# csukuangfj/kaldi-hmm-gmm

Measured on AMD Instinct MI355X. Metric: frames/sec (whole node) per EM iter (align+acc-stats), 5k-pdf x 64-Gauss, higher is better.
Workload: dtype f32 via f16x2s

## Files before the change

include/khg_hip.h:

```cpp
#ifndef KHG_HIP_H_
#define KHG_HIP_H_
#include <stdint.h>

#ifdef __cplusplus
extern "C" {
#endif

#define KHG_OK 0
#define KHG_E_ARG (-1)
#define KHG_E_HIP (-2)
#define KHG_E_RUNTIME (-3)
#define KHG_E_UNSUPPORTED (-4)
#define KHG_MAX_DIM 512

typedef struct khg_ctx khg_ctx;
typedef struct khg_model khg_model;
typedef struct khg_tm khg_tm;
typedef struct khg_utts khg_utts;
typedef struct khg_accs khg_accs;

const char *khg_last_error(void);
int khg_version(void);

int khg_ctx_create(int device, void *stream, khg_ctx **out);
int khg_ctx_destroy(khg_ctx *ctx);
int khg_ctx_sync(khg_ctx *ctx);
int khg_ctx_set_timing(khg_ctx *ctx, int on);
int khg_ctx_get_timings(khg_ctx *ctx, char *names, int64_t names_cap, float *ms, int32_t cap,
                        int32_t *n_out);

#define KHG_K1_AUTO 0
#define KHG_K1_FP32_PDF 2
#define KHG_K1_FP32_UTT 3
#define KHG_K1_F16X2 4
#define KHG_K1_F16X2S 5
int khg_ctx_set_k1_form(khg_ctx *ctx, int form);

#define KHG_OPT_K1_FORM 0
#define KHG_OPT_K1_ORDER 1
#define KHG_OPT_K1_NF 2
#define KHG_OPT_K1P_TS 3
#define KHG_OPT_K1_INTERLEAVE 4
#define KHG_OPT_K1_DBG 5
#define KHG_OPT_K2_INORDER 6
#define KHG_OPT_K2_KS 7
#define KHG_OPT_K2_SERIAL 8
#define KHG_OPT_K2_PROF 9
#define KHG_OPT_K3_BUCKET 10
#define KHG_OPT_K3_FORM 11
#define KHG_OPT_K3_PHASE_B 12
#define KHG_OPT_K3_NY 13
#define KHG_OPT_DEBUG 14
#define KHG_OPT_K3_PHASE_A 15
#define KHG_OPT_K2_SPLIT 16
#define KHG_OPT_K2S_HUB 17
#define KHG_OPT_LAT_OPS_LDS 18
#define KHG_OPT_K1_LAUNCH 19
#define KHG_OPT_K1_PGRID 20
#define KHG_OPT_K1_PROF 21
#define KHG_OPT_K2_LADDER 22
#define KHG_OPT_COUNT 23
#define KHG_INFO_SCRATCH_BYTES 100
#define KHG_INFO_SCRATCH_BLOCKS 101
int khg_ctx_set_option(khg_ctx *ctx, int option, int value);
int khg_ctx_get_option(const khg_ctx *ctx, int option, int *value);
int khg_option_check(int option, int value);
int khg_option_from_env(const char *name, const char *text, int *option, int *value);

int khg_model_create(khg_ctx *ctx, int32_t num_pdfs, int32_t dim, const int32_t *gauss_off_h,
                     const float *gconsts_h, const float *means_invvars_h,
                     const float *inv_vars_h, khg_model **out);
int khg_model_destroy(khg_model *m);
int khg_model_invalidate(khg_model *m);

int khg_tm_create(khg_ctx *ctx, int32_t num_tids, const int32_t *id2pdf_h, khg_tm **out);
int khg_tm_set_trans_cost(khg_tm *tm, const float *trans_cost_h);
int khg_tm_destroy(khg_tm *tm);

int khg_utts_create(khg_ctx *ctx, const khg_tm *tm, int32_t n_utt, int32_t dim,
                    const int64_t *frame_off_h, const float *feats_h, const float *feats_d,
                    const int64_t *state_off_h, const int32_t *start_h, const int64_t *arc_off_h,
                    const int32_t *ilabel_h, const int32_t *olabel_h, const float *weight_h,
                    const int32_t *nextstate_h, const float *final_h, khg_utts **out);
int khg_utts_destroy(khg_utts *u);
typedef struct khg_graph khg_graph;
int khg_graph_create(khg_ctx *ctx, const khg_tm *tm, int32_t num_states, int32_t start, const int64_t *arc_off_h,
                     const int32_t *ilabel_h, const int32_t *olabel_h, const float *weight_h,
                     const int32_t *nextstate_h, const float *final_h, khg_graph **out);
int khg_graph_destroy(khg_graph *g);
int khg_graph_info(const khg_graph *g, int64_t *num_states, int64_t *num_arcs, int32_t *num_pdfs,
                   int32_t *max_in_degree, int64_t *device_bytes);
int khg_utts_create_on_graph(khg_ctx *ctx, const khg_tm *tm, khg_graph *g, int32_t n_utt, int32_t dim,
                             const int64_t *frame_off_h, const float *feats_h, const float *feats_d, khg_utts **out);
int khg_utts_graph_bytes(const khg_utts *u, int64_t *bytes);
int khg_utts_num_pdfs(const khg_utts *u, int64_t *pdf_off_h );
int khg_utts_pdfs(const khg_utts *u, int32_t *pdfs_h );
int khg_utts_k2_plan(khg_ctx *ctx, const khg_utts *u, int32_t out[8]);
int khg_utts_k2_ladder(khg_ctx *ctx, const khg_utts *u, int32_t *out);
int khg_utts_pdf_first(const khg_utts *u, int32_t *first_h );

int khg_loglikes(khg_ctx *ctx, const khg_model *m, khg_utts *u);
int khg_loglikes_reachable(khg_ctx *ctx, const khg_model *m, khg_utts *u);
int khg_loglikes_band(khg_ctx *ctx, const khg_model *m, khg_utts *u);
int khg_utts_pdf_last(const khg_utts *u, int32_t *last_h );
int khg_loglikes_layout(const khg_utts *u, int64_t *ll_off_h, int64_t *total);
int khg_loglikes_download(khg_ctx *ctx, const khg_utts *u, float *ll_h);
int khg_loglikes_upload(khg_ctx *ctx, khg_utts *u, const float *ll_h);
int khg_utts_set_pdf_list(khg_utts *u, int32_t n, const int32_t *pdfs_h);
int khg_utts_features_changed(khg_utts *u);

typedef struct {
  float beam;
  float retry_beam;
  int32_t careful;
  float acoustic_scale;
  int32_t max_active;
  int32_t min_active;
  float beam_delta;
  float hash_ratio;
  float like_scale;
} khg_align_config;
void khg_align_config_default(khg_align_config *c);

#define KHG_ALIGN_DONE 0
#define KHG_ALIGN_ERROR 1
#define KHG_ALIGN_RETRIED 2
#define KHG_ALIGN_EXACT_DP 4
#define KHG_ALIGN_FALLBACK 8

int khg_careful_graph(int32_t num_states, int32_t start, const int64_t *arc_off_h, const int32_t *ilabel_h,
                      const int32_t *olabel_h, const float *weight_h, const int32_t *nextstate_h, const float *final_h,
                      int32_t *out_num_states, int32_t *out_start, int64_t *out_arc_off_h, int32_t *out_ilabel_h,
                      int32_t *out_olabel_h, float *out_weight_h, int32_t *out_nextstate_h, float *out_final_h);

int khg_align(khg_ctx *ctx, const khg_tm *tm, khg_utts *u, const khg_align_config *cfg,
              int32_t *ali_h, int32_t *words_h, int64_t *words_off_h, int64_t words_cap,
              float *like_h, int32_t *status_h);
int khg_ali_upload(khg_ctx *ctx, khg_utts *u, const int32_t *ali_h);
int khg_ali_download(khg_ctx *ctx, khg_utts *u, int32_t *ali_h);

typedef struct {
  float beam;
  int32_t max_active;
  int32_t min_active;
  float lattice_beam;
  int32_t prune_interval;
  float beam_delta;
  float hash_ratio;
  float prune_scale;
  float acoustic_scale;
  int32_t allow_partial;
  int32_t scratch_per_frame;
} khg_lattice_faster_config;
void khg_lattice_faster_config_default(khg_lattice_faster_config *c);

#define KHG_LAT_SUCCEEDED 1
#define KHG_LAT_PARTIAL 2
#define KHG_LAT_SCRATCH 4
#define KHG_LAT_NO_PATH 8
#define KHG_LAT_EPS_LOOP 16
#define KHG_LAT_WORDS 32
#define KHG_LAT_NO_TRACEBACK 64

int khg_decode_lattice_faster(khg_ctx *ctx, const khg_tm *tm, khg_utts *u, const khg_lattice_faster_config *cfg,
                              int32_t *ali_h, int32_t *words_h, int64_t *words_off_h, int64_t words_cap,
                              double *like_h, int32_t *status_h);

typedef struct {
  float beam;
  float lattice_beam;
  int32_t prune_interval;
  float prune_scale;
  float acoustic_scale;
  int32_t allow_partial;
  int32_t scratch_per_frame;
} khg_lattice_simple_config;
void khg_lattice_simple_config_default(khg_lattice_simple_config *c);

#define KHG_LAT_NO_EPS_TOKEN 128
#define KHG_LAT_NAN 256

// ... 381 lines not shown
```

kaldi_hmm_gmm_amd/_lib.py:

```python
import ctypes as C
import os

import numpy as np

_HERE = os.path.dirname(os.path.abspath(__file__))
LIB_PATH = os.environ.get("KHG_LIBRARY") or os.path.join(_HERE, "libkhg_hip.so")


class KhgError(RuntimeError):
    """Mirror of the reference's std::runtime_error -> Python RuntimeError (csrc/log.h:46-53)."""


def _load():
    if not os.path.exists(LIB_PATH):
        raise ImportError(
            f"{LIB_PATH} not found: build it with `python -c 'import __graft_entry__ as g; g.build()'` "
            "(hipcc --offload-arch=gfx950). kaldi_hmm_gmm_amd has no CPU fallback."
        )
    try:
        import torch
    except ImportError:
        pass
    return C.CDLL(LIB_PATH)

# ... 54 lines not shown
    _fields_ = [
        ("min_gaussian_weight", C.c_float),
        ("min_gaussian_occupancy", C.c_float),
        ("min_variance", C.c_double),
        ("remove_low_count_gaussians", C.c_int32),
        ("variance_floor_vector", C.POINTER(C.c_double)),
    ]


class EbwOptionsC(C.Structure):
    _fields_ = [("E", C.c_double), ("tau", C.c_double)]


class EbwWeightOptionsC(C.Structure):
    _fields_ = [("min_num_count_weight_update", C.c_double), ("min_gaussian_weight", C.c_double), ("tau", C.c_double)]


class EbwResultsC(C.Structure):
    _fields_ = [("auxf_impr_gauss", C.c_double), ("count", C.c_double), ("auxf_impr_weights", C.c_double), ("floored", C.c_int32),
                ("failed", C.c_int32), ("skipped", C.c_int32), ("weights_skipped", C.c_int32)]


class FmllrOptionsC(C.Structure):
    _fields_ = [("min_count", C.c_double), ("num_iters", C.c_int32)]


class MlltOptionsC(C.Structure):
    _fields_ = [("num_iters", C.c_int32)]


class LdaOptionsC(C.Structure):
    _fields_ = [("target_dim", C.c_int32), ("remove_offset", C.c_int32), ("within_class_factor", C.c_double)]


class FrontendOptsC(C.Structure):
    _fields_ = [("kind", C.c_int32), ("samp_freq", C.c_float), ("frame_length_ms", C.c_float), ("frame_shift_ms", C.c_float), ("preemph_coeff", C.c_float),
                ("remove_dc_offset", C.c_int32), ("window_type", C.c_int32), ("blackman_coeff", C.c_float), ("snip_edges", C.c_int32),
                ("round_to_power_of_two", C.c_int32), ("dither", C.c_float), ("num_mel_bins", C.c_int32), ("low_freq", C.c_float), ("high_freq", C.c_float),
                ("vtln_warp", C.c_float), ("htk_compat", C.c_int32), ("num_ceps", C.c_int32), ("cepstral_lifter", C.c_float), ("use_energy", C.c_int32),
                ("raw_energy", C.c_int32), ("energy_floor", C.c_float), ("use_log_fbank", C.c_int32), ("use_power", C.c_int32)]


class RescoreStatsC(C.Structure):
    _fields_ = [("arcs", C.c_int64), ("emitting_arcs", C.c_int64), ("cells", C.c_int64)]


class LmRescoreStatsC(C.Structure):
    _fields_ = [("in_states", C.c_int64), ("in_arcs", C.c_int64), ("out_states", C.c_int64), ("out_arcs", C.c_int64), ("max_hist", C.c_int64)]


SIGNATURES = {
    "khg_last_error": (C.c_char_p, []),
    "khg_version": (C.c_int, []),
    "khg_ctx_create": (C.c_int, [C.c_int, vp, C.POINTER(vp)]),
    "khg_ctx_destroy": (C.c_int, [vp]),
    "khg_ctx_sync": (C.c_int, [vp]),
    "khg_ctx_set_timing": (C.c_int, [vp, C.c_int]),
    "khg_ctx_set_k1_form": (C.c_int, [vp, C.c_int]),
    "khg_ctx_set_option": (C.c_int, [vp, C.c_int, C.c_int]),
    "khg_ctx_get_option": (C.c_int, [vp, C.c_int, C.POINTER(C.c_int)]),
    "khg_option_check": (C.c_int, [C.c_int, C.c_int]),
    "khg_option_from_env": (C.c_int, [C.c_char_p, C.c_char_p, C.POINTER(C.c_int), C.POINTER(C.c_int)]),
    "khg_ctx_get_timings": (C.c_int, [vp, C.c_char_p, C.c_int64, c_f32p, C.c_int32, c_i32p]),
    "khg_model_create": (C.c_int, [vp, C.c_int32, C.c_int32, c_i32p, c_f32p, c_f32p, c_f32p, C.POINTER(vp)]),
    "khg_model_destroy": (C.c_int, [vp]),
    "khg_tm_create": (C.c_int, [vp, C.c_int32, c_i32p, C.POINTER(vp)]),
    "khg_tm_set_trans_cost": (C.c_int, [vp, c_f32p]),
    "khg_tm_destroy": (C.c_int, [vp]),
    "khg_utts_create": (
        C.c_int,
        [vp, vp, C.c_int32, C.c_int32, c_i64p, c_f32p, vp, c_i64p, c_i32p, c_i64p, c_i32p, c_i32p, c_f32p, c_i32p,
         c_f32p, C.POINTER(vp)],
    ),
    "khg_utts_destroy": (C.c_int, [vp]),
    "khg_graph_create": (C.c_int, [vp, vp, C.c_int32, C.c_int32, c_i64p, c_i32p, c_i32p, c_f32p, c_i32p, c_f32p, C.POINTER(vp)]),
    "khg_graph_destroy": (C.c_int, [vp]),
    "khg_graph_info": (C.c_int, [vp, c_i64p, c_i64p, c_i32p, c_i32p, c_i64p]),
    "khg_utts_create_on_graph": (C.c_int, [vp, vp, vp, C.c_int32, C.c_int32, c_i64p, c_f32p, vp, C.POINTER(vp)]),
    "khg_utts_graph_bytes": (C.c_int, [vp, c_i64p]),
    "khg_utts_num_pdfs": (C.c_int, [vp, c_i64p]),
    "khg_utts_pdfs": (C.c_int, [vp, c_i32p]),
    "khg_utts_k2_plan": (C.c_int, [vp, vp, c_i32p]),
    "khg_utts_k2_ladder": (C.c_int, [vp, vp, c_i32p]),
    "khg_utts_pdf_first": (C.c_int, [vp, c_i32p]),
    "khg_loglikes": (C.c_int, [vp, vp, vp]),
    "khg_loglikes_reachable": (C.c_int, [vp, vp, vp]),
    "khg_loglikes_band": (C.c_int, [vp, vp, vp]),
    "khg_utts_pdf_last": (C.c_int, [vp, c_i32p]),
    "khg_loglikes_layout": (C.c_int, [vp, c_i64p, c_i64p]),
    "khg_loglikes_download": (C.c_int, [vp, vp, c_f32p]),
    "khg_loglikes_upload": (C.c_int, [vp, vp, c_f32p]),
    "khg_utts_set_pdf_list": (C.c_int, [vp, C.c_int32, c_i32p]),
    "khg_utts_features_changed": (C.c_int, [vp]),
    "khg_comm_info": (C.c_int, [vp, c_i32p, c_i32p, c_i32p]),
    "khg_align_config_default": (None, [C.POINTER(AlignConfigC)]),
    "khg_align": (C.c_int, [vp, vp, vp, C.POINTER(AlignConfigC), c_i32p, c_i32p, c_i64p, C.c_int64, c_f32p, c_i32p]),
    "khg_ali_upload": (C.c_int, [vp, vp, c_i32p]),
    "khg_lattice_faster_config_default": (None, [C.POINTER(LatticeFasterConfigC)]),
    "khg_decode_lattice_faster": (C.c_int, [vp, vp, vp, C.POINTER(LatticeFasterConfigC), c_i32p, c_i32p, c_i64p, C.c_int64, c_f64p,
                                            c_i32p]),
    "khg_lattice_simple_config_default": (None, [C.POINTER(LatticeSimpleConfigC)]),
    "khg_decode_lattice_simple": (C.c_int, [vp, vp, vp, C.POINTER(LatticeSimpleConfigC), c_i32p, c_i32p, c_i64p, C.c_int64, c_f64p,
                                            c_i32p, c_i32p]),
    "khg_decode_lattice_simple_raw": (C.c_int, [vp, vp, vp, C.POINTER(LatticeSimpleConfigC), c_i32p, c_i32p, c_i64p, C.c_int64, c_f64p,
                                                c_i32p, c_i32p, C.POINTER(vp)]),
    "khg_decode_lattice_faster_raw": (C.c_int, [vp, vp, vp, C.POINTER(LatticeFasterConfigC), c_i32p, c_i32p, c_i64p, C.c_int64, c_f64p,
                                                c_i32p, C.POINTER(vp)]),
    "khg_lattices_sizes": (C.c_int, [vp, c_i64p, c_i64p]),
    "khg_lattices_download": (C.c_int, [vp, vp, c_i32p, c_i32p, c_f32p, c_f32p, c_f32p, c_i32p, c_i32p, c_i32p, c_f32p, c_f32p, c_i32p,
                                        c_i32p]),
    "khg_lattices_device_bytes": (C.c_int, [vp, c_i64p]),
    "khg_lattices_destroy": (C.c_int, [vp]),
    "khg_lattices_validate": (C.c_int, [C.c_int32, c_i64p, c_i64p, c_i32p, c_i32p, c_f32p, c_f32p, c_f32p, c_i32p, c_i32p, c_i32p, c_f32p,
                                        c_f32p, c_i32p, c_i32p]),
    "khg_lattices_upload": (C.c_int, [vp, C.c_int32, c_i64p, c_i64p, c_i32p, c_i32p, c_f32p, c_f32p, c_f32p, c_i32p, c_i32p, c_i32p, c_f32p,
                                      c_f32p, c_i32p, c_i32p, C.POINTER(vp)]),
    "khg_lattices_num_utts": (C.c_int, [vp, c_i32p]),
    "khg_lattices_ali_layout": (C.c_int, [vp, vp, c_i64p]),
    "khg_lattices_num_chunks": (C.c_int, [vp, c_i32p]),
    "khg_lattices_chunk_utts": (C.c_int, [vp, c_i32p]),
    "khg_lattices_best_path": (C.c_int, [vp, vp, C.c_int32, c_f32p, c_f32p, c_i32p, c_i32p, c_i64p, C.c_int64, c_f32p, c_i32p]),
    "khg_lattices_prune": (C.c_int, [vp, vp, C.c_float, C.c_float, C.c_float, c_i32p, C.POINTER(vp)]),
    "khg_lattices_posteriors": (C.c_int, [vp, vp, C.c_float, C.c_float, c_i32p, c_f64p, C.POINTER(vp)]),
    "khg_lattices_rescore": (C.c_int, [vp, vp, vp, vp, vp, C.c_float, C.c_int, C.POINTER(RescoreStatsC), C.POINTER(vp)]),
    "khg_lattices_op_status": (C.c_int, [vp, c_i32p]),
    "khg_lattices_boost": (C.c_int, [vp, vp, C.c_int32, c_i32p, C.c_int32, c_i32p, c_i64p, c_i32p, vp, C.c_float, C.c_float, c_i32p,
                                     C.POINTER(vp)]),
    "khg_lm_validate": (C.c_int, [C.c_int32, c_i32p, c_f32p, c_i32p, c_i32p, c_f32p, c_i32p, c_f32p, C.c_int32]),
    "khg_lm_create": (C.c_int, [vp, C.c_int32, c_i32p, c_f32p, c_i32p, c_i32p, c_f32p, c_i32p, c_f32p, C.c_int32, C.POINTER(vp)]),
    "khg_lm_destroy": (C.c_int, [vp]),
    "khg_lm_num_states": (C.c_int, [vp, c_i32p]),
    "khg_lm_device_bytes": (C.c_int, [vp, c_i64p]),
    "khg_lm_score": (C.c_int, [C.c_int32, c_i32p, c_f32p, c_i32p, c_i32p, c_f32p, c_i32p, c_f32p, C.c_int32, C.c_int32, c_i32p, c_f32p]),
    "khg_lattices_lm_rescore": (C.c_int, [vp, vp, vp, C.c_float, C.c_int32, c_i32p, C.POINTER(LmRescoreStatsC), C.POINTER(vp)]),
    "khg_lattices_mpe_posteriors": (C.c_int, [vp, vp, C.c_int32, c_i32p, c_i32p, C.c_int32, c_i32p, c_i64p, c_i32p, vp, C.c_int32, C.c_int32,
                                              C.c_float, C.c_float, c_i32p, c_f64p, c_f64p, C.POINTER(vp)]),
    "khg_posteriors_sizes": (C.c_int, [vp, c_i64p, c_i64p]),
    "khg_posteriors_download": (C.c_int, [vp, vp, c_i64p, c_i32p, c_f64p, c_f64p]),
    "khg_posteriors_device_bytes": (C.c_int, [vp, c_i64p]),
    "khg_posteriors_destroy": (C.c_int, [vp]),
    "khg_posteriors_validate": (C.c_int, [C.c_int32, c_i64p, c_i64p, C.c_int64, c_i32p, c_f64p]),
    "khg_posteriors_upload": (C.c_int, [vp, C.c_int32, c_i64p, c_i64p, c_i32p, c_f64p, C.POINTER(vp)]),
    "khg_ali_download": (C.c_int, [vp, vp, c_i32p]),
    "khg_accs_create": (C.c_int, [vp, vp, vp, C.POINTER(vp)]),
    "khg_accs_destroy": (C.c_int, [vp]),
    "khg_accs_zero": (C.c_int, [vp, vp]),
    "khg_accs_size": (C.c_int, [vp, c_i64p]),
    "khg_accs_device_ptr": (C.c_int, [vp, C.POINTER(vp)]),
    "khg_accs_download": (C.c_int, [vp, vp, c_f64p]),
    "khg_accs_upload": (C.c_int, [vp, vp, c_f64p]),
    "khg_acc_stats": (C.c_int, [vp, vp, vp, vp, C.c_float, vp]),
    "khg_acc_stats_post": (C.c_int, [vp, vp, vp, vp, vp, C.c_float, vp]),
    "khg_acc_stats_post2": (C.c_int, [vp, vp, vp, vp, vp, C.c_float, vp, vp]),
    "khg_accs_add": (C.c_int, [vp, vp, C.c_float, vp]),
    "khg_accs_scale": (C.c_int, [vp, vp, C.c_float]),
    "khg_accs_smooth_with_accum": (C.c_int, [vp, vp, C.c_float, vp, vp, c_i32p]),
    "khg_accs_allreduce": (C.c_int, [vp, vp, vp]),
    "khg_accs_allreduce_range": (C.c_int, [vp, vp, vp, C.c_int32, C.c_int32, vp]),
    "khg_acc_stats_reduce": (C.c_int, [vp, vp, vp, vp, C.c_float, vp, vp, C.c_int32]),
    "khg_accs_allreduce_f32": (C.c_int, [vp, vp, vp]),
    "khg_comm_unique_id": (C.c_int, [vp]),
    "khg_comm_create": (C.c_int, [vp, C.c_int32, C.c_int32, vp, C.POINTER(vp)]),
    "khg_comm_destroy": (C.c_int, [vp]),
    "khg_compute_gconsts": (C.c_int, [C.c_int32, C.c_int32, c_i32p, c_f32p, c_f32p, c_f32p, c_f32p, c_i32p]),
    "khg_mle_options_default": (None, [C.POINTER(MleOptionsC)]),
    "khg_mle_am_diag_gmm_update": (
# ... 131 lines not shown
```

kaldi_hmm_gmm_amd/csrc/khg_ctx_model.hip:

```cpp
#include "khg_internal.hpp"

#include <mutex>
#include "khg_k1_loglikes.hip.inc"

static thread_local std::string g_err;
extern "C" const char* khg_last_error(void) { return g_err.c_str(); }
int khg_set_error(int code, const std::string& msg) { g_err = msg; return code; }
extern "C" int khg_version(void) { return 100; }

static std::mutex g_ctx_mu;
static std::vector<khg_ctx*> g_ctxs;
static constexpr size_t KHG_ARENA_BYTES = size_t(24) << 20;
void* arena_alloc(khg_ctx* ctx, size_t bytes) {
  KhgArena& a = ctx->arena;
  if (!a.dev) {
    if (a.cap == SIZE_MAX) return nullptr;
    void *d = nullptr, *h = nullptr;
    if (hipMalloc(&d, KHG_ARENA_BYTES) != hipSuccess || hipHostMalloc(&h, KHG_ARENA_BYTES, hipHostMallocDefault) != hipSuccess) {
      if (d) (void)hipFree(d);
      (void)hipGetLastError();
      a.cap = SIZE_MAX;
      return nullptr;
    }
    a.dev = static_cast<char*>(d); a.host = static_cast<char*>(h); a.cap = KHG_ARENA_BYTES; a.top = a.base = 256;
// ... 51 lines not shown
  return false;
}
void khg_dev_free(void* p) {
  if (p && !khg_arena_release(p)) (void)hipFree(p);
}

static void ctx_defaults_from_env(khg_ctx* c);
extern "C" int khg_ctx_create(int device, void* stream, khg_ctx** out) {
  if (!out) return khg_set_error(KHG_E_ARG, "khg_ctx_create: out is NULL");
  int n = 0;
  hipError_t e = hipGetDeviceCount(&n);
  if (e != hipSuccess || n <= 0)
    return khg_set_error(KHG_E_HIP, "khg_ctx_create: no HIP device available (this library has no CPU fallback)");
  if (device < 0 || device >= n) return khg_set_error(KHG_E_ARG, "khg_ctx_create: bad device index");
  HIPCHK(hipSetDevice(device));
  hipDeviceProp_t prop;
  HIPCHK(hipGetDeviceProperties(&prop, device));
  if (std::string(prop.gcnArchName).rfind("gfx950", 0) != 0)
    return khg_set_error(KHG_E_UNSUPPORTED, std::string("khg_ctx_create: built for gfx950, device is ") + prop.gcnArchName);
  khg_ctx* c = new khg_ctx();
  c->device = device;
  if (stream) { c->stream = (hipStream_t)stream; c->own_stream = false; }
  else { HIPCHK(hipStreamCreateWithFlags(&c->stream, hipStreamNonBlocking)); c->own_stream = true; }
  for (auto& s : c->sides) HIPCHK(hipStreamCreateWithFlags(&s, hipStreamNonBlocking));
  ctx_defaults_from_env(c);
  int rc = dev_alloc(&c->err_flag_d, 1);
  if (!rc) rc = dev_alloc(&c->dump_d, 256);
  if (!rc && hipHostMalloc(reinterpret_cast<void**>(&c->err_host), 256, hipHostMallocDefault) != hipSuccess) rc = khg_set_error(KHG_E_HIP, "khg_ctx_create: hipHostMalloc failed");
  if (rc) { delete c; return rc; }
  HIPCHK(hipMemsetAsync(c->err_flag_d, 0, sizeof(int32_t), c->stream));
  { std::lock_guard<std::mutex> lk(g_ctx_mu); g_ctxs.push_back(c); }
  *out = c;
  return KHG_OK;
}
extern "C" int khg_ctx_destroy(khg_ctx* c) {
  if (!c) return KHG_OK;
  (void)hipStreamSynchronize(c->stream);
  for (auto& s : c->sides) (void)hipStreamSynchronize(s);
  {
    std::lock_guard<std::mutex> lk(g_ctx_mu);
    g_ctxs.erase(std::remove(g_ctxs.begin(), g_ctxs.end(), c), g_ctxs.end());
    if (c->arena.dev && !c->arena.blocks.empty()) {
      c->arena.dirty.clear();
      g_orphans.push_back(std::move(c->arena));
      c->arena = KhgArena();
    }
  }
  DEVFREE(c->err_flag_d); DEVFREE(c->dump_d); DEVFREE(c->k1_next_d);
  if (c->err_host) (void)hipHostFree(c->err_host);
  if (c->arena.dev) (void)hipFree(c->arena.dev);
  if (c->arena.host) (void)hipHostFree(c->arena.host);
  if (c->own_stream) (void)hipStreamDestroy(c->stream);
  for (auto& s : c->sides) (void)hipStreamDestroy(s);
  if (c->comm_stream) { (void)hipStreamSynchronize(c->comm_stream); (void)hipStreamDestroy(c->comm_stream); }
  if (c->ev_k3) (void)hipEventDestroy(c->ev_k3);
  if (c->ev_c1) (void)hipEventDestroy(c->ev_c1);
  delete c;
  return KHG_OK;
}
extern "C" int khg_ctx_set_timing(khg_ctx* c, int on) {
  if (!c) return khg_set_error(KHG_E_ARG, "ctx is NULL");
  c->timing = on != 0;
  return KHG_OK;
}
extern "C" int khg_ctx_get_timings(khg_ctx* c, char* names, int64_t names_cap, float* ms, int32_t cap, int32_t* n_out) {
  if (!c || !n_out) return khg_set_error(KHG_E_ARG, "bad arguments");
  HIPCHK(hipStreamSynchronize(c->stream));
  for (auto& s : c->sides) HIPCHK(hipStreamSynchronize(s));
  int n = 0; std::string all;
  for (auto& t : c->timings) {
    float v = 0.0f;
    (void)hipEventElapsedTime(&v, t.e0, t.e1);
    if (n < cap && ms) ms[n] = v;
    all += t.name; all += '\n';
    (void)hipEventDestroy(t.e0); (void)hipEventDestroy(t.e1);
    ++n;
  }
  c->timings.clear();
  if (names && names_cap > 0) { size_t k = std::min<size_t>(all.size(), (size_t)names_cap - 1); memcpy(names, all.data(), k); names[k] = 0; }
  *n_out = n;
  return KHG_OK;
}
static const struct { int lo, hi; } k_opt_range[KHG_OPT_COUNT] = {
  {KHG_K1_AUTO, KHG_K1_F16X2S}, {0, 4}, {0, 6}, {0, 1 << 20}, {-1, 1}, {0, 255}, {0, 1}, {0, 4}, {0, 3}, {0, 1}, {0, 2}, {0, 2}, {0, 2}, {0, 64}, {0, 1}, {0, 1}, {0, 1}, {0, 1 << 20}, {0, 1}, {0, 2}, {0, 1 << 16}, {0, 1}, {0, 1}};
extern "C" int khg_option_check(int opt, int value) {
  if (opt < 0 || opt >= KHG_OPT_COUNT) return khg_set_error(KHG_E_ARG, "khg_option_check: no such option");
  if (value < k_opt_range[opt].lo || value > k_opt_range[opt].hi || (opt == KHG_OPT_K1_FORM && value == 1))
    return khg_set_error(KHG_E_ARG, "khg_ctx_set_option: option " + std::to_string(opt) + " takes values " + std::to_string(k_opt_range[opt].lo) + " .. " + std::to_string(k_opt_range[opt].hi));
  return KHG_OK;
}
extern "C" int khg_ctx_set_option(khg_ctx* c, int opt, int value) {
  if (!c || opt < 0 || opt >= KHG_OPT_COUNT) return khg_set_error(KHG_E_ARG, "khg_ctx_set_option: bad arguments");
  int rc = khg_option_check(opt, value);
  if (rc) return rc;
  c->opt[opt] = value;
  return KHG_OK;
}
extern "C" int khg_ctx_get_option(const khg_ctx* c, int opt, int* value) {
  if (c && value && (opt == KHG_INFO_SCRATCH_BYTES || opt == KHG_INFO_SCRATCH_BLOCKS)) {
    *value = opt == KHG_INFO_SCRATCH_BYTES ? (c->arena.dev ? (int)c->arena.top : 0) : (int)c->arena.blocks.size();
    return KHG_OK;
  }
  if (!c || !value || opt < 0 || opt >= KHG_OPT_COUNT) return khg_set_error(KHG_E_ARG, "khg_ctx_get_option: bad arguments");
  *value = c->opt[opt];
  return KHG_OK;
}
extern "C" int khg_ctx_set_k1_form(khg_ctx* c, int form) { return khg_ctx_set_option(c, KHG_OPT_K1_FORM, form); }
static const struct { const char* name; int opt; const char* words; } k_env_tab[] = {
  {"KHG_K1", KHG_OPT_K1_FORM, "auto=0,pdf=2,fp32=2,utt=3,f16x2=4,f16x2s=5"},
  {"KHG_K1_ORDER", KHG_OPT_K1_ORDER, "desc=0,none=1,asc=2,tiles=3,xcd=4"},
  {"KHG_K1_NF", KHG_OPT_K1_NF, ""}, {"KHG_K1P_TS", KHG_OPT_K1P_TS, ""}, {"KHG_K1_INTERLEAVE", KHG_OPT_K1_INTERLEAVE, ""},
  {"KHG_K1B_DBG", KHG_OPT_K1_DBG, ""}, {"KHG_K2_INORDER", KHG_OPT_K2_INORDER, ""}, {"KHG_K2_KS", KHG_OPT_K2_KS, ""},
  {"KHG_K2_SERIAL", KHG_OPT_K2_SERIAL, ""}, {"KHG_K2_PROF", KHG_OPT_K2_PROF, ""},
  {"KHG_K3_BUCKET", KHG_OPT_K3_BUCKET, "sort=0,atomic=1,count=2"}, {"KHG_K3_FORM", KHG_OPT_K3_FORM, "auto=0,block=1,valu=2"},
  {"KHG_K3_VALU", KHG_OPT_K3_FORM, "1=2"}, {"KHG_K3_PHASEB", KHG_OPT_K3_PHASE_B, "f64=0,f32=1,f16=2"},
  {"KHG_K3_NY", KHG_OPT_K3_NY, ""}, {"KHG_DEBUG", KHG_OPT_DEBUG, ""}, {"KHG_K3_PHASEA", KHG_OPT_K3_PHASE_A, "auto=0,f16=0,f32=1"},
  {"KHG_K2_SPLIT", KHG_OPT_K2_SPLIT, "on=0,off=1"}, {"KHG_K2S_HUB", KHG_OPT_K2S_HUB, ""},
  {"KHG_LAT_OPS_LDS", KHG_OPT_LAT_OPS_LDS, "on=0,off=1"},
  {"KHG_K1_LAUNCH", KHG_OPT_K1_LAUNCH, "auto=0,chunk=1,persistent=2"}, {"KHG_K1_PGRID", KHG_OPT_K1_PGRID, ""},
  {"KHG_K1_PROF", KHG_OPT_K1_PROF, ""}, {"KHG_K2_LADDER", KHG_OPT_K2_LADDER, "on=0,off=1"}};
extern "C" int khg_option_from_env(const char* name, const char* text, int* option, int* value) {
  if (!name || !text || !*text || !option || !value) return khg_set_error(KHG_E_ARG, "khg_option_from_env: bad arguments");
  for (const auto& t : k_env_tab) {
    if (strcmp(t.name, name) != 0) continue;
    const char* e = text;
    int v = atoi(e);
    bool word = false;
    for (const char* w = t.words; *w;) {
      const char* eq = strchr(w, '=');
      const size_t n = (size_t)(eq - w);
      if (strlen(e) == n && strncmp(e, w, n) == 0) { v = atoi(eq + 1); word = true; break; }
      const char* comma = strchr(eq, ',');
      if (!comma) break;
      w = comma + 1;
    }
    if (!word && *t.words && !(e[0] >= '0' && e[0] <= '9') && e[0] != '-')
      return khg_set_error(KHG_E_ARG, std::string(name) + ": unknown word '" + text + "'");
    if (v < k_opt_range[t.opt].lo || v > k_opt_range[t.opt].hi)
      return khg_set_error(KHG_E_ARG, std::string(name) + " takes values " + std::to_string(k_opt_range[t.opt].lo) + " .. " + std::to_string(k_opt_range[t.opt].hi));
    *option = t.opt; *value = v;
    return KHG_OK;
  }
  return khg_set_error(KHG_E_ARG, std::string("khg_option_from_env: no such variable: ") + name);
}
static void ctx_defaults_from_env(khg_ctx* c) {
  c->opt[KHG_OPT_K1_INTERLEAVE] = -1;
  c->opt[KHG_OPT_K1P_TS] = 1024;
  c->opt[KHG_OPT_K2S_HUB] = 32;
  c->opt[KHG_OPT_K3_PHASE_B] = 2;
  for (const auto& t : k_env_tab) {
    const char* e = getenv(t.name);
    if (!e || !*e) continue;
    int opt = 0, v = 0;
    if (khg_option_from_env(t.name, e, &opt, &v) == KHG_OK) c->opt[opt] = v;
  }
}
extern "C" int khg_ctx_sync(khg_ctx* c) {
  if (!c) return khg_set_error(KHG_E_ARG, "ctx is NULL");
  return check_err_flag(c, "khg_ctx_sync");
}
int check_err_flag(khg_ctx* c, const char* where) {
  { int rf = arena_flush(c); if (rf) return rf; }
  for (int i = 0; i < khg_ctx::NSIDE; ++i)
    if (c->side_dirty[i]) { HIPCHK(hipStreamSynchronize(c->sides[i])); c->side_dirty[i] = false; }
  HIPCHK(hipMemcpyAsync(c->err_host, c->err_flag_d, sizeof(int32_t), hipMemcpyDeviceToHost, c->stream));
  HIPCHK(hipStreamSynchronize(c->stream));
  c->pageable_pending = false;
  const int32_t f = *c->err_host;
  if (f) {
    HIPCHK(hipMemsetAsync(c->err_flag_d, 0, sizeof(int32_t), c->stream));
    if (f & 1) return khg_set_error(KHG_E_RUNTIME, std::string(where) + ": Invalid answer (overflow or invalid variances/features?)");
    if (f & 2) return khg_set_error(KHG_E_RUNTIME, std::string(where) + ": internal queue overflow in the faithful decoder");
    if (f & 8) return khg_set_error(KHG_E_RUNTIME, std::string(where) + ": internal error: K3 work items exceed their bound");
    return khg_set_error(KHG_E_RUNTIME, std::string(where) + ": pdf-id out of range (graph/model mismatch)");
  }
  return KHG_OK;
}

template <int KQ>
__global__ __launch_bounds__(256) void k0_pack_tiles(const float* __restrict__ gconsts, const float* __restrict__ miv,
                                                      const float* __restrict__ iv, const int32_t* __restrict__ gauss_off,
                                                      const int32_t* __restrict__ pdf_tile_off, const int32_t* __restrict__ tile_pdf,
                                                      int D, float* __restrict__ wimg, float* __restrict__ nhiv) {
  constexpr int ROW = khg_row_floats(KQ), TILE = khg_tile_floats(KQ);
  const int t = blockIdx.x, p = tile_pdf[t];
  const int g_first = gauss_off[p] + 32 * (t - pdf_tile_off[p]);
  const int nrow = min(32, gauss_off[p + 1] - g_first);
  float* img = wimg + (size_t)t * TILE;
  for (int i = threadIdx.x; i < TILE; i += 256) {
    float v = 0.0f;
    if (i < 4 * 32 * ROW) {
      const int q = i / (32 * ROW), r = (i / ROW) & 31, s = i % ROW;
      const int d = 2 * s + (q & 1);
      if (r < nrow && d < D) {
        const size_t src = (size_t)(g_first + r) * D + d;
        v = (q & 2) ? -0.5f * iv[src] : miv[src];
      }
    } else if (i < 4 * 32 * ROW + 32) {
      const int r = i - 4 * 32 * ROW;
      v = r < nrow ? gconsts[g_first + r] : -INFINITY;
    }
    img[i] = v;
  }
// ... 271 lines not shown
```

kaldi_hmm_gmm_amd/csrc/khg_internal.hpp:

```cpp
#pragma once
#include <hip/hip_runtime.h>

#include <algorithm>
#include <climits>
#include <cmath>
#include <cstdint>
#include <cstdio>
#include <cstdlib>
#include <cstring>
#include <deque>
#include <limits>
#include <string>
#include <type_traits>
#include <utility>
#include <vector>

#include "../../include/khg_hip.h"
#include "khg_dev_types.hip.inc"

int khg_set_error(int code, const std::string& msg);

#define HIPCHK(expr)                                                                         \
  do {                                                                                       \
    hipError_t e_ = (expr);                                                                  \
// ... 159 lines not shown
  float* trans_cost_d = nullptr;
  bool has_trans_cost = false;
};

struct khg_graph {
  khg_ctx* ctx = nullptr;
  int32_t refs = 1;
  int64_t S = 0, A = 0, nwords = 0, device_bytes = 0;
  int32_t start = -1, max_indeg = 0, max_outdeg = 0;
  bool same_col = true, has_eps = false, ladder = true;
  std::vector<int32_t> pdfs, pdf_first, pdf_dfin;
  int64_t *state_off_d = nullptr, *in_off_d = nullptr, *out_off_d = nullptr;
  int32_t *start_d = nullptr, *in_src_d = nullptr, *in_col_d = nullptr, *in_tid_d = nullptr, *in_olabel_d = nullptr, *out_inidx_d = nullptr;
  float *in_w_d = nullptr, *final_d = nullptr;
};
void khg_graph_release(khg_graph* g);

struct khg_utts {
  khg_ctx* ctx = nullptr;
  khg_graph* graph = nullptr;
  int32_t* gidx_d = nullptr;
  int64_t graph_bytes = 0;
  bool small = false;
  int32_t n_utt = 0, D = 0;
  int64_t N = 0;
  bool has_graphs = false;
  std::vector<int64_t> frame_off, state_off, pdf_off, ll_off, bp_off, path_off, words_off;
  std::vector<int32_t> pdfs;
  int32_t max_states = 0, max_inarcs = 0, max_indeg = 0, max_outdeg = 0;
  bool same_col = true;
  bool ladder = true;
  int32_t pdfs_checked_P = -1;
  bool has_eps = false;
  const float* feats_d = nullptr; bool own_feats = false;
  int64_t *frame_off_d = nullptr, *state_off_d = nullptr, *pdf_off_d = nullptr, *ll_off_d = nullptr;
  int32_t *pdfs_d = nullptr, *start_d = nullptr;
  KwChunk* wchunks_d = nullptr;
  int32_t n_wchunks = 0;
  int64_t *in_off_d = nullptr, *out_off_d = nullptr;
  int32_t *in_src_d = nullptr, *in_col_d = nullptr, *in_tid_d = nullptr, *in_olabel_d = nullptr, *out_inidx_d = nullptr;
  float *in_w_d = nullptr, *final_d = nullptr;
  K1Chunk* chunks_d = nullptr; int32_t n_chunks = 0; int32_t chunk_kq = 0;
  int64_t* tile_off_d = nullptr; int32_t* tiles_d = nullptr;
  std::vector<int32_t> pdf_first;
  std::vector<int32_t> pdf_last;
  int ll_mode = 0;
  void* band_args = nullptr;
  khg_model* band_model = nullptr; int band_ks = 0; size_t band_lds = 0; uint64_t band_serial = 0, band_version = 0; std::vector<int32_t> band_key;
  int tiles_reach = -1;
  std::vector<int32_t> tiles_pto;
  float* ll_d = nullptr; int64_t ll_total = 0; bool ll_valid = false;
  float* xpl_d = nullptr; int64_t* utt_xtile_off_d = nullptr; int32_t xpl_kq = 0;
  K1pEntry* p_ents_d = nullptr; K1pSlice* p_slices_d = nullptr; int32_t p_nslices = 0; int p_reach = -1; int32_t p_P = -1;
  int32_t p_grp[10] = {0, 0, 0, 0, 0, 0, 0, 0, 0, 0};
  std::vector<int32_t> p_goff;
  int64_t* utt_x32_off_d = nullptr;
  K1bChunk* bchunks_d = nullptr; int32_t n_bchunks = 0, bchunk_nt = 0;
  int32_t* x32_utt_d = nullptr; int64_t n_x32 = 0;
  k1b_u32x4* xh_d = nullptr; int32_t xh_ks = 0; std::vector<int32_t> xh_ex; int32_t* xh_ex_d = nullptr;
  std::vector<float> xmax;
  k1b_u32x4* xs_d = nullptr; int32_t xs_ks = 0; std::vector<int32_t> xs_ex; int32_t* xs_ex_d = nullptr;
  K1sChunk* schunks_d = nullptr; int32_t n_schunks = 0, schunk_nmax = 0;
  K1sUnit* sunits_d = nullptr; std::vector<int32_t> sunits_pto; int sunits_reach = -1;
  uint8_t* bp_d = nullptr; int64_t *bp_off_d = nullptr, *path_off_d = nullptr, *words_off_d = nullptr;
  double* layer_best_d = nullptr; int32_t* layer_cnt_d = nullptr; int32_t* path_d = nullptr;
  unsigned char* k2_gscratch_d = nullptr; size_t k2_gscratch_bytes = 0;
  int32_t* k2_order_d = nullptr;
  int32_t *ali_d = nullptr, *words_d = nullptr, *num_words_d = nullptr, *status_d = nullptr;
  float* like_d = nullptr;
  bool ali_valid = false;
  char* out_blk_d = nullptr; size_t out_blk_bytes = 0;
  hipEvent_t ev_dp = nullptr, ev_ali = nullptr;
  bool ali_pending = false;
  int32_t *ali2_d = nullptr, *unc_d = nullptr, *unc_cnt_h = nullptr, *unc_cnt_dev = nullptr;
  int64_t* sub_off_d = nullptr;
  bool ali_split = false;
  int32_t *pdf_count_d = nullptr, *pdf_cursor_d = nullptr, *frame_ids_d = nullptr;
  uint32_t *sort_keys_d = nullptr, *sort_keys_out_d = nullptr, *sort_vals_d = nullptr; void* sort_tmp_d = nullptr; size_t sort_tmp_bytes = 0;
  int32_t* cs_hist_d = nullptr; size_t cs_hist_n = 0; int64_t* cs_tot_d = nullptr; size_t cs_tot_n = 0;
  double *k3_part_d = nullptr, *k3_llpart_d = nullptr; size_t k3_part_n = 0, k3_llpart_n = 0;
  void* k3_items_d = nullptr; int32_t* k3_item_off_d = nullptr; size_t k3_items_n = 0, k3_item_off_n = 0;
  int64_t* pdf_start_d = nullptr; unsigned long long* tid_count_d = nullptr;
  int32_t k3_P = 0, k3_tids = 0;
  int32_t *pe_row_d = nullptr, *pe_tid_d = nullptr, *pe_ids_d = nullptr; float* pe_w_d = nullptr; size_t pe_cap = 0;
  uint32_t *pe_keys_d = nullptr, *pe_keys_out_d = nullptr, *pe_vals_d = nullptr; void* pe_tmp_d = nullptr; size_t pe_tmp_bytes = 0;
  int64_t* pe_start_d = nullptr; int32_t pe_P = 0;
  uint64_t *rc_keys_d = nullptr, *rc_keys_out_d = nullptr; uint32_t *rc_vals_d = nullptr, *rc_vals_out_d = nullptr;
  int32_t *rc_flag_d = nullptr, *rc_inc_d = nullptr, *rc_row_d = nullptr; float* rc_cell_d = nullptr; size_t rc_cap = 0;
  void* rc_tmp_d = nullptr; size_t rc_tmp_bytes = 0;
  int32_t *rc_cell_start_d = nullptr, *rc_item_off_d = nullptr; int64_t* rc_stats_d = nullptr; int32_t rc_P = -1;
};

static inline int64_t utt_states(const khg_utts* u, int i) { return u->graph ? u->state_off[1] : u->state_off[(size_t)i + 1] - u->state_off[(size_t)i]; }

struct khg_accs {
  khg_ctx* ctx = nullptr;
  int64_t sumG = 0; int32_t D = 0, num_tids = 0;
  int64_t n = 0, cap = 0;
  double* buf_d = nullptr;
  float* wire_d = nullptr; int64_t wire_cap = 0;
  double* occ() const { return buf_d; }
  double* mean() const { return buf_d + sumG; }
  double* var() const { return buf_d + sumG + sumG * D; }
  double* trans() const { return buf_d + sumG + 2 * sumG * D; }
  double* scalars() const { return trans() + num_tids + 1; }
};

constexpr size_t KHG_ARENA_MAX_REQ = size_t(4) << 20;
template <class T>
inline int u_alloc(khg_utts* u, T** p, size_t n) {
  if (n == 0) n = 1;
  if (u->small && n * sizeof(T) <= KHG_ARENA_MAX_REQ) {
    *p = static_cast<T*>(arena_alloc(u->ctx, n * sizeof(T)));
    if (*p) return KHG_OK;
  }
  return dev_alloc(p, n);
}
template <class T>
inline int u_upload(khg_ctx* ctx, khg_utts* u, T** p, const std::vector<T>& v) {
  if (u->small && v.size() * sizeof(T) <= KHG_ARENA_MAX_REQ) {
    *p = static_cast<T*>(arena_alloc(u->ctx, std::max<size_t>(v.size(), 1) * sizeof(T)));
    if (*p) {
      if (!v.empty()) { memcpy(u->ctx->arena.mirror(*p), v.data(), v.size() * sizeof(T)); arena_mark_dirty(u->ctx, *p, v.size() * sizeof(T)); }
      return KHG_OK;
    }
  }
  return dev_upload(ctx, p, v);
}

int check_err_flag(khg_ctx* c, const char* where);
int model_pack(khg_ctx* ctx, khg_model* m);
int model_stats(khg_ctx* ctx, khg_model* m);
int wait_ali(khg_ctx* ctx, khg_utts* u);
void k1_free_band(khg_utts* u);
int k1_maxima(khg_ctx* ctx, khg_model* m, khg_utts* u, std::vector<float>* xk);
khg_model* khg_model_lookup(uint64_t serial);
int k1_band_check(khg_ctx* ctx, khg_utts* u);
int k1_band_repair(khg_ctx* ctx, khg_utts* u, int32_t* status_d, int repair_bit, hipStream_t side);
int accs_allreduce_pieces(khg_ctx* ctx, khg_accs* a, const khg_model* m, int first_pdf, int n_pdf, void* comm, hipStream_t st);
int ctx_comm_stream(khg_ctx* ctx);
int k3_post_check(khg_ctx* ctx, const khg_model* m, const std::string& who);
__attribute__((visibility("hidden"))) int k3_acc_stats_post_one_block(khg_ctx* ctx, const khg_model* m, const khg_tm* tm, khg_utts* u, const khg_posteriors* p, float scale, khg_accs* acc);
struct PostInfo { const khg_ctx* ctx; int32_t U, max_tid; const int64_t *frame_off, *entry_off; };
void posteriors_info(const khg_posteriors* p, PostInfo* out);
int posteriors_flatten(khg_ctx* ctx, const khg_posteriors* p, const int64_t* set_frame_off_d, double scale, int32_t num_tids,
                       int32_t* e_row, int32_t* e_tid, float* e_w, int sign = 0);
int posteriors_make_unit(khg_ctx* ctx, int32_t n_utt, const int64_t* frame_off_h, int64_t** entry_begin_d, double** weight_d, int32_t** tid_d,
                         const int64_t** frame_off_d, khg_posteriors** out);
inline int utts_grow_pe(khg_utts* u, size_t E) {
  if (E <= u->pe_cap) return KHG_OK;
  DEVFREE(u->pe_row_d); DEVFREE(u->pe_tid_d); DEVFREE(u->pe_ids_d); DEVFREE(u->pe_w_d); DEVFREE(u->pe_keys_d); DEVFREE(u->pe_keys_out_d); DEVFREE(u->pe_vals_d);
  u->pe_cap = 0;
  int rc = u_alloc(u, &u->pe_row_d, E);
  if (!rc) rc = u_alloc(u, &u->pe_tid_d, E);
  if (!rc) rc = u_alloc(u, &u->pe_ids_d, E);
  if (!rc) rc = u_alloc(u, &u->pe_w_d, E);
  if (!rc) rc = u_alloc(u, &u->pe_keys_d, E);
  if (!rc) rc = u_alloc(u, &u->pe_keys_out_d, E);
  if (!rc) rc = u_alloc(u, &u->pe_vals_d, E);
  if (rc) return rc;
  u->pe_cap = E;
  return KHG_OK;
}
```

kaldi_hmm_gmm_amd/csrc/khg_k3.hip:

```cpp
#include "khg_internal.hpp"

#include <hipcub/hipcub.hpp>

#include "khg_k3_accstats.hip.inc"
#include "khg_k3_post.hip.inc"
#include "khg_k3_accops.hip.inc"

extern "C" int khg_accs_create(khg_ctx* ctx, const khg_model* m, const khg_tm* tm, khg_accs** out) {
  if (ctx_dead(ctx) || !m || !tm || !out) return khg_set_error(KHG_E_ARG, "khg_accs_create: bad arguments");
  khg_accs* a = new khg_accs();
  a->ctx = ctx; a->sumG = m->sumG; a->D = m->D; a->num_tids = tm->num_tids;
  a->n = a->sumG * (1 + 2 * (int64_t)a->D) + a->num_tids + 1 + 8;
  int rc = dev_alloc(&a->buf_d, (size_t)a->n);
  if (rc) { delete a; return rc; }
  a->cap = a->n;
  *out = a;
  return khg_accs_zero(ctx, a);
}
extern "C" int khg_accs_destroy(khg_accs* a) { if (a) { DEVFREE(a->buf_d); DEVFREE(a->wire_d); delete a; } return KHG_OK; }
extern "C" int khg_accs_zero(khg_ctx* ctx, khg_accs* a) {
  if (ctx_dead(ctx) || !a) return khg_set_error(KHG_E_ARG, "bad arguments");
  HIPCHK(hipMemsetAsync(a->buf_d, 0, sizeof(double) * (size_t)a->n, ctx->stream));
  return KHG_OK;
}
// ... 54 lines not shown
  if (dst->sumG > 0) {
    KernelTimer kt(ctx, "k3_accs_smooth");
    KHG_LAUNCH(ctx, k3_accs_smooth, dim3((unsigned)((dst->sumG + 3) / 4)), dim3(256), 0, ctx->stream, dst->occ(), dst->mean(), dst->var(), src->occ(),
               src->mean(), src->var(), (double)tau, dst->sumG, (int)dst->D, cnt_d);
    e = hipGetLastError();
  }
  if (untouched_out) {
    int32_t cnt = 0;
    if (e == hipSuccess) e = hipMemcpyAsync(&cnt, cnt_d, sizeof(int32_t), hipMemcpyDeviceToHost, ctx->stream);
    if (e == hipSuccess) e = hipStreamSynchronize(ctx->stream);
    DEVFREE(cnt_d);
    if (e == hipSuccess) *untouched_out = cnt;
  }
  if (e != hipSuccess) return khg_set_error(KHG_E_HIP, hipGetErrorString(e));
  return KHG_OK;
}

static int k3_phase_a_scales(khg_ctx* ctx, khg_model* m, khg_utts* u, bool* use) {
  *use = false;
  const int D = m->D, K = 8 * m->KQ;
  if (m->KQ == 0) return KHG_OK;
  std::vector<float> xk;
  int rc = k1_maxima(ctx, m, u, &xk);
  if (rc) return rc;
  if (m->k3_xb.empty()) {
    if (m->wmax.empty() || (int)m->k3_xb_raw.size() != D) { m->wmax.clear(); rc = model_stats(ctx, m); if (rc) return rc; }
    m->k3_xb = m->k3_xb_raw;
    m->k3_ex.assign((size_t)K, 0);
    bool ok = true;
    for (int d = 0; d < D; ++d) {
      const float xb = m->k3_xb[(size_t)d];
      if (!(xb > 0.0f) || !(xb < 1.0e18f)) { ok = false; break; }
      m->k3_ex[(size_t)2 * d] = 12 - std::ilogb(xb);
      m->k3_ex[(size_t)2 * d + 1] = 9 - std::ilogb(xb * xb);
    }
    int S = INT_MAX;
    if (ok) {
      for (int k = 0; k < 2 * D; ++k) if (m->wmax[(size_t)k] > 0.0f) S = std::min(S, 14 - std::ilogb(m->wmax[(size_t)k]) + m->k3_ex[(size_t)k]);
      if (S == INT_MAX) S = 0;
      if (S < -40 || S > 40) ok = false;
    }
    if (ok) {
      double floor_sum = 0.0, bound = (double)m->gcmax;
      for (int k = 0; k < 2 * D; ++k) {
        const double xbk = (k & 1) ? (double)m->k3_xb[(size_t)(k >> 1)] * (double)m->k3_xb[(size_t)(k >> 1)] : (double)m->k3_xb[(size_t)(k >> 1)];
        floor_sum += std::ldexp((double)m->wmax[(size_t)k], S - m->k3_ex[(size_t)k]) + std::ldexp(xbk, m->k3_ex[(size_t)k]);
        bound += (double)m->wmax[(size_t)k] * xbk * ((k & 1) ? 128.0 : 16.0);
      }
      if (!(std::ldexp(floor_sum, -25 - S) <= 4.0e-6) || !(bound <= 268435456.0)) ok = false;
      if (ctx->opt[KHG_OPT_DEBUG]) fprintf(stderr, "[khg] K3 fp16 phase A: S %d, floor %.3g, bound %.3g -> %s\n", S, std::ldexp(floor_sum, -25 - S), bound, ok ? "on" : "off");
    }
    m->k3_S = ok ? S : 0;
    m->k3_f16_ok = ok;
    if (ok) {
      if (!m->k3_ex_d) { rc = dev_alloc(&m->k3_ex_d, (size_t)K); if (rc) return rc; }
      HIPCHK(hipMemcpyAsync(m->k3_ex_d, m->k3_ex.data(), sizeof(int32_t) * (size_t)K, hipMemcpyHostToDevice, ctx->stream));
      HIPCHK(hipStreamSynchronize(ctx->stream));
    }
  }
  if (!m->k3_f16_ok) return KHG_OK;
  for (int k = 0; k < 2 * D; ++k)
    if (!(std::ldexp((double)xk[(size_t)k], m->k3_ex[(size_t)k]) < 65504.0)) return KHG_OK;
  *use = true;
  return KHG_OK;
}

static size_t k3_valu_lds(const khg_model* m, int maxG, bool post) {
  return sizeof(float) * (size_t)K3_CHUNK * ((size_t)(m->KQ ? 4 * m->KQ : (m->D | 1)) + (maxG | 1) + (post ? 5 : 4));
}
#define K3_VALU_LDS_MAX (160 * 1024)
enum K3Form { K3F_WAVE, K3F_MFMA, K3F_VALU };
struct K3Run {
  int form = K3F_VALU;
  int cls_lo = 0, cls_hi = INT_MAX;
  int maxG = 0, n_cls = 0;
  bool second = false;
  int NB = 0, NB16 = 0, nwv16 = 4;
  int ny = 1;
  bool parked = false;
  size_t nsum1 = 0;
  int target = 0;
  int64_t extra_blocks = 0, max_items = 0, max_slots = 0;
  bool may_f16a = false, may_f16b = false;
  size_t lds[3] = {0, 0, 0};
  bool too_wide = false;
};
struct K3Plan { int nruns = 0; K3Run run[2]; };

static K3Plan k3_plan(const khg_ctx* ctx, const khg_model* m, bool post, int64_t Neff, bool one_block) {
  const int P = m->P, KQ = m->KQ;
  const int k3form = ctx->opt[KHG_OPT_K3_FORM];
  const int pha = ctx->opt[KHG_OPT_K3_PHASE_A], phb = ctx->opt[KHG_OPT_K3_PHASE_B], ny_opt = ctx->opt[KHG_OPT_K3_NY];
  const int64_t avg = Neff / std::max(1, P);
  auto items = [&](K3Run& r) {
    r.target = one_block ? INT_MAX : (int)std::min<int64_t>(1 << 30, std::max<int64_t>(512, 2 * avg / r.ny));
    const int64_t per_t = Neff / r.target;
    r.extra_blocks = std::min<int64_t>(per_t + P, 2 * per_t) + 1;
    r.max_items = (int64_t)P * r.ny + r.extra_blocks;
    r.max_slots = !r.parked ? INT_MAX : r.ny > 1 ? r.max_items : 2 * per_t + 1;
  };
  auto wave = [&](int cls_lo, int cls_hi, int maxG) {
    K3Run r;
    r.form = K3F_WAVE; r.cls_lo = cls_lo; r.cls_hi = cls_hi; r.maxG = maxG; r.n_cls = P;
    const size_t nb = (size_t)(r.NB = (maxG + 15) / 16);
    r.may_f16a = nb >= 3 && pha == 0 && phb != 1; r.may_f16b = phb == 2;
    const size_t fold = sizeof(double) * (nb * 16 * 80 + nb * 16);
    r.lds[0] = std::max<size_t>(sizeof(float) * (nb * 20 * 64 + 4 * 4 * 16 * 20), fold);
    r.lds[1] = std::max<size_t>(sizeof(float) * (4 * 4 * 16 * 20) + 2 * (size_t)(4 * 2 * 16 * K3_XH_ROW), fold);
    r.lds[2] = std::max<size_t>(2 * (size_t)4 * (2 * (2 * 16 * K3_XH_ROW) + 2 * 2 * 40 * 36) + nb * 3 * 2 * 64 * 16, fold);
    const int64_t avg_tiles = (avg + 15) / 16;
    r.ny = (int)std::max<int64_t>(1, std::min<int64_t>(std::min<int64_t>(32, (avg_tiles + 15) / 16), (4096 + P - 1) / P));
    if (ny_opt > 0) r.ny = ny_opt;
    r.parked = true; r.nsum1 = nb * 16 * 80 + nb * 16 + 1;
    items(r);
    return r;
  };
  auto block = [&](int form, int cls_lo, int cls_hi, int maxG, int n_cls, bool second) {
    K3Run r;
    r.form = form; r.cls_lo = cls_lo; r.cls_hi = cls_hi; r.maxG = maxG; r.n_cls = n_cls; r.second = second;
    const int64_t avg_chunks = (avg + K3_CHUNK - 1) / K3_CHUNK;
    if (form == K3F_MFMA) {
      r.NB = std::max(1, (maxG + 63) / 64);
      r.lds[0] = sizeof(float) * ((size_t)4 * K3_CHUNK * 2 * KQ + (post ? 6 : 5) * K3_CHUNK);
      r.ny = (int)std::max<int64_t>(1, std::min<int64_t>(std::min<int64_t>(32, avg_chunks), (4096 + n_cls - 1) / std::max(1, n_cls)));
      if (ny_opt > 0) r.ny = ny_opt;
      r.may_f16a = r.may_f16b = !post && pha == 0 && phb == 2 && ((KQ == 20 && maxG <= 128) || (KQ == 10 && maxG <= 192));
      r.NB16 = maxG <= 128 ? 1 : 3; r.nwv16 = maxG > 64 && maxG <= 128 ? 8 : 4;
      const size_t kpad = ((size_t)8 * KQ + 31) / 32 * 32, gp_b16 = maxG <= 64 ? 64 : (maxG <= 128 ? 128 : 192);
      r.lds[2] = std::max<size_t>(2 * (2 * (size_t)K3_CHUNK * (kpad + 8) + 2 * (size_t)8 * KQ * (K3_CHUNK + 8)) + sizeof(float) * 9 * K3_CHUNK,
                                  sizeof(float) * (2 * gp_b16 * (size_t)(m->D | 1) + 8 * (size_t)KQ));
    } else {
      r.lds[0] = k3_valu_lds(m, maxG, post); r.too_wide = r.lds[0] > K3_VALU_LDS_MAX;
      r.ny = (int)std::max<int64_t>(1, std::min<int64_t>(64, (avg_chunks + 3) / 4));
    }
    if (one_block) r.ny = 1;
    items(r);
    return r;
  };
  int maxG = 0, maxG_lo = 0, n_hi = 0;
  for (int p = 0; p < P; ++p) {
    const int Gp = m->gauss_off[(size_t)p + 1] - m->gauss_off[(size_t)p];
    maxG = std::max(maxG, Gp);
    if (Gp <= 64) maxG_lo = std::max(maxG_lo, Gp); else ++n_hi;
  }
  const bool mfma_ok = (maxG <= 128 || (maxG <= 256 && KQ == 10)) && k3form != 2 && KQ != 0;
  const bool wave_ok = !post && KQ == 10 && k3form == 0 && maxG_lo > 0;
  const int rest = mfma_ok ? K3F_MFMA : K3F_VALU;
  K3Plan pl;
  if (wave_ok && n_hi == 0) pl.run[pl.nruns++] = wave(0, INT_MAX, maxG);
  else if (wave_ok) {
    pl.run[pl.nruns++] = wave(0, 64, maxG_lo);
    pl.run[pl.nruns++] = block(rest, 64, INT_MAX, maxG, n_hi, true);
  } else pl.run[pl.nruns++] = block(rest, 0, INT_MAX, maxG, P, false);
  return pl;
}

int k3_post_check(khg_ctx* ctx, const khg_model* m, const std::string& who) {
  const K3Run r = k3_plan(ctx, m, true, 0, false).run[0];
  if (r.too_wide) return khg_set_error(KHG_E_UNSUPPORTED, who + "a pdf of " + std::to_string(r.maxG) + " Gaussians is too large for the LDS chunk buffers of the statistics pass");
  return KHG_OK;
}

typedef void (*K3Kernel)(K3Args);
enum K3Variant { K3V_WAVE, K3V_WAVE16, K3V_FINALIZE, K3V_MFMA, K3V_BLOCK16, K3V_VALU };
struct K3Inst { int variant, KQ, NB, nwv; bool post, f16a; K3Kernel fn; };
#define K3_WAVE_ROWS(NB)                                                                                                           \
  {K3V_WAVE, 10, NB, 4, false, false, k3_accumulate_wave<NB>}, {K3V_WAVE, 10, NB, 4, false, true, k3_accumulate_wave<NB, true>}, \
  {K3V_WAVE16, 10, NB, 4, false, true, k3_accumulate_wave16<NB>}, {K3V_FINALIZE, 10, NB, 4, false, false, k3_wave_finalize<NB>}
#define K3_MFMA_ROWS(KQ, NBW) {K3V_MFMA, KQ, NBW, 4, false, false, k3_accumulate_mfma<KQ, NBW>}, {K3V_MFMA, KQ, NBW, 4, true, false, k3_accumulate_mfma<KQ, NBW, true>}
#define K3_VALU_ROWS(KQ) {K3V_VALU, KQ, 0, 4, false, false, k3_accumulate<KQ>}, {K3V_VALU, KQ, 0, 4, true, false, k3_accumulate<KQ, true>}
static const K3Inst k3_insts[] = {
  K3_WAVE_ROWS(1), K3_WAVE_ROWS(2), K3_WAVE_ROWS(3), K3_WAVE_ROWS(4),
  K3_MFMA_ROWS(10, 1), K3_MFMA_ROWS(10, 2), K3_MFMA_ROWS(10, 3), K3_MFMA_ROWS(10, 4), K3_MFMA_ROWS(20, 1), K3_MFMA_ROWS(20, 2),
  {K3V_BLOCK16, 20, 1, 4, false, true, k3_accumulate_block16<20, 1, 4>}, {K3V_BLOCK16, 10, 1, 4, false, true, k3_accumulate_block16<10, 1, 4>},
  {K3V_BLOCK16, 20, 1, 8, false, true, k3_accumulate_block16<20, 1, 8>}, {K3V_BLOCK16, 10, 1, 8, false, true, k3_accumulate_block16<10, 1, 8>},
  {K3V_BLOCK16, 10, 3, 4, false, true, k3_accumulate_block16<10, 3, 4>},
  K3_VALU_ROWS(10), K3_VALU_ROWS(20), K3_VALU_ROWS(0),
};
static K3Kernel k3_kernel(int variant, int KQ, int NB, int nwv, bool post, bool f16a) {
  for (const K3Inst& i : k3_insts)
    if (i.variant == variant && i.KQ == KQ && i.NB == NB && i.nwv == nwv && i.post == post && i.f16a == f16a) return i.fn;
  return nullptr;
}
static int k3_launch(khg_ctx* ctx, K3Kernel fn, unsigned grid, int nthr, size_t lds, const K3Args& a) {
  if (lds > 48 * 1024) HIPCHK(hipFuncSetAttribute((const void*)fn, hipFuncAttributeMaxDynamicSharedMemorySize, (int)lds));
  KHG_LAUNCH(ctx, fn, dim3(grid), dim3(nthr), lds, ctx->stream, a);
  return KHG_OK;
}

template <class Launch>
static int k3_for_ranges(khg_ctx* ctx, const khg_model* m, khg_accs* acc, void* comm, int nparts, Launch&& launch) {
  const int n = comm ? nparts : 1;
  for (int part = 0; part < n; ++part) {
    const int p0 = (int)((int64_t)m->P * part / n), np = (int)((int64_t)m->P * (part + 1) / n) - p0;
    int rc = launch(p0, np);
    if (!rc && comm && n > 1) rc = accs_allreduce_pieces(ctx, acc, m, p0, np, comm, nullptr);
    if (rc) return rc;
  }
  return KHG_OK;
}

static K3Args k3_args(khg_ctx* ctx, const khg_model* m, const khg_tm* tm, const khg_utts* u, khg_accs* acc, float weight, bool post, int64_t Neff) {
  K3Args a;
  a.feats = u->feats_d; a.ali = post ? u->pe_tid_d : u->ali_d; a.id2pdf = tm->id2pdf_d; a.num_tids = tm->num_tids;
  a.N = Neff; a.P = m->P; a.D = m->D;
  a.gauss_off = m->gauss_off_d; a.gconsts = m->gconsts_d; a.means_invvars = m->miv_d; a.inv_vars = m->iv_d; a.nhalf_inv_vars = m->nhiv_d;
  a.pdf_count = u->pdf_count_d; a.pdf_start = post ? u->pe_start_d : u->pdf_start_d; a.pdf_cursor = u->pdf_cursor_d;
  a.frame_ids = post ? u->pe_ids_d : u->frame_ids_d; a.tid_count = u->tid_count_d;
  a.e_row = post ? u->pe_row_d : nullptr; a.e_w = post ? u->pe_w_d : nullptr;
  a.occ = acc->occ(); a.mean_acc = acc->mean(); a.var_acc = acc->var(); a.trans_acc = acc->trans(); a.scalars = acc->scalars();
  a.weight = weight; a.err_flag = ctx->err_flag_d; a.part = nullptr; a.ll_part = nullptr; a.pdf0 = 0; a.npdf = m->P; a.items = nullptr; a.item_off = nullptr;
  a.pa_ex = nullptr; a.pa_S = 0; a.pa_scale = 1.0f; a.pa_inv = 1.0f; a.pa_c1 = 1.44269504088896340736f; a.pb_gscale = 1.0f; a.pb_SG = 0;
  return a;
}
static bool k3_weight_ordinary(float weight) { return std::isfinite(weight) && std::fabs(weight) > 1.0e-30f && std::fabs(weight) < 1.0e30f; }
static void k3_set_scales(K3Args& a, const khg_model* m, bool f16a, bool f16b) {
  if (f16a) {
    a.pa_ex = m->k3_ex_d; a.pa_S = m->k3_S;
    a.pa_scale = std::ldexp(1.0f, m->k3_S); a.pa_inv = std::ldexp(1.0f, -m->k3_S); a.pa_c1 = std::ldexp(1.44269504088896340736f, -m->k3_S);
  }
  if (f16b) { a.pb_SG = 13 - std::ilogb(std::fabs(a.weight)); a.pb_gscale = std::ldexp(1.0f, a.pb_SG); }
}

template int u_alloc<uint32_t>(khg_utts*, uint32_t**, size_t);
static int k3_bucket(khg_ctx* ctx, const khg_model* m, const khg_tm* tm, khg_utts* u, const K3Args& a, bool post, int64_t nsub, int64_t Neff) {
  int rc = KHG_OK;
  uint32_t *&sort_keys = post ? u->pe_keys_d : u->sort_keys_d, *&sort_keys_out = post ? u->pe_keys_out_d : u->sort_keys_out_d;
  uint32_t*& sort_vals = post ? u->pe_vals_d : u->sort_vals_d;
  void*& sort_tmp = post ? u->pe_tmp_d : u->sort_tmp_d;
  size_t& sort_tmp_bytes = post ? u->pe_tmp_bytes : u->sort_tmp_bytes;
  const int gb = (int)std::min<int64_t>(4096, (Neff + 255) / 256);
  {
    KernelTimer kt(ctx, nsub < 0 ? "k3_bucket" : "k3_bucket_pass2");
    if (!post && nsub < 0 && (ctx->opt[KHG_OPT_K3_BUCKET] == 1 || u->N >= (int64_t)INT_MAX)) {
      KHG_LAUNCH(ctx, k3_count, dim3(gb), dim3(256), 0, ctx->stream, a);
      KHG_LAUNCH(ctx, k3_scan, dim3(1), dim3(1024), 0, ctx->stream, a);
      KHG_LAUNCH(ctx, k3_scatter, dim3(gb), dim3(256), 0, ctx->stream, a);
    } else if (!post && nsub < 0 && ctx->opt[KHG_OPT_K3_BUCKET] == 2 && m->P <= K3_CS_MAXP) {
      const int nw = m->P + 1 <= 7168 ? 4 : 2;
      int64_t CB = 32768;
      while (CB > 64 * nw * 4 && (u->N + CB - 1) / CB < 1024) CB /= 2;
      const int nblk = (int)((u->N + CB - 1) / CB);
      const size_t hist_n = (size_t)nblk * ((size_t)m->P + 1);
      if (u->cs_hist_n < hist_n) { DEVFREE(u->cs_hist_d); rc = u_alloc(u, &u->cs_hist_d, hist_n); if (rc) return rc; u->cs_hist_n = hist_n; }
      if (u->cs_tot_n < (size_t)m->P + 1) { DEVFREE(u->cs_tot_d); rc = u_alloc(u, &u->cs_tot_d, (size_t)m->P + 1); if (rc) return rc; u->cs_tot_n = (size_t)m->P + 1; }
      K3CsArgs c{u->cs_hist_d, u->cs_tot_d, (int32_t)CB, nblk};
      const bool ldst = tm->num_tids <= K3_LDS_TIDS;
      const size_t lds_h = sizeof(unsigned int) * ((size_t)m->P + 1 + (ldst ? (size_t)tm->num_tids + 1 : 0));
      const size_t lds_p = sizeof(unsigned int) * (size_t)nw * ((size_t)m->P + 1 + 1024);
      if (lds_h > 48 * 1024) {
        HIPCHK(hipFuncSetAttribute((const void*)k3_cs_hist<true>, hipFuncAttributeMaxDynamicSharedMemorySize, (int)lds_h));
        HIPCHK(hipFuncSetAttribute((const void*)k3_cs_hist<false>, hipFuncAttributeMaxDynamicSharedMemorySize, (int)lds_h));
      }
      if (lds_p > 48 * 1024) HIPCHK(hipFuncSetAttribute((const void*)k3_cs_place, hipFuncAttributeMaxDynamicSharedMemorySize, (int)lds_p));
      if (ldst) KHG_LAUNCH(ctx, k3_cs_hist<true>, dim3(nblk), dim3(256), lds_h, ctx->stream, a, c);
      else KHG_LAUNCH(ctx, k3_cs_hist<false>, dim3(nblk), dim3(256), lds_h, ctx->stream, a, c);
      KHG_LAUNCH(ctx, k3_cs_scan, dim3((m->P + 256) / 256), dim3(256), 0, ctx->stream, a, c);
      KHG_LAUNCH(ctx, k3_cs_starts, dim3(1), dim3(1024), 0, ctx->stream, a, c);
      KHG_LAUNCH(ctx, k3_cs_place, dim3(nblk), dim3(64 * nw), lds_p, ctx->stream, a, c);
    } else {
      int bits = 1;
      while ((1 << bits) <= m->P) ++bits;
      if (!sort_keys) {
        rc = u_alloc(u, &sort_keys, (size_t)u->N);
        if (!rc) rc = u_alloc(u, &sort_keys_out, (size_t)u->N);
        if (!rc) rc = u_alloc(u, &sort_vals, (size_t)u->N);
        if (rc) return rc;
      }
      size_t need = 0;
      HIPCHK(hipcub::DeviceRadixSort::SortPairs(nullptr, need, sort_keys, sort_keys_out, sort_vals,
                                                reinterpret_cast<uint32_t*>(a.frame_ids), (int)Neff, 0, bits, ctx->stream));
      if (need > sort_tmp_bytes) {
        DEVFREE(sort_tmp);
        { int rt = u_alloc(u, reinterpret_cast<char**>(&sort_tmp), need); if (rt) return rt; }
        sort_tmp_bytes = need;
      }
      if (post) {
        const bool ldst = tm->num_tids <= K3_LDS_TIDS;
        if (ldst) KHG_LAUNCH(ctx, k3_post_keys<true>, dim3(std::min(gb, 1024)), dim3(256), sizeof(double) * ((size_t)tm->num_tids + 1), ctx->stream, a, sort_keys, sort_vals);
        else KHG_LAUNCH(ctx, k3_post_keys<false>, dim3(std::min(gb, 1024)), dim3(256), 0, ctx->stream, a, sort_keys, sort_vals);
      } else if (nsub >= 0) {
        if (!u->sub_off_d) { rc = u_alloc(u, &u->sub_off_d, (size_t)u->n_utt + 1); if (rc) return rc; }
        KHG_LAUNCH(ctx, k3_sub_scan, dim3(1), dim3(1024), 0, ctx->stream, u->unc_d, u->frame_off_d, u->n_utt, u->sub_off_d);
        KHG_LAUNCH(ctx, k3_sub_keys, dim3((unsigned)std::min(u->n_utt, 8192)), dim3(64), 0, ctx->stream, a, u->unc_d, u->frame_off_d, u->sub_off_d, u->n_utt, sort_keys, sort_vals);
      } else if (tm->num_tids <= K3_LDS_TIDS) KHG_LAUNCH(ctx, k3_sort_keys<true>, dim3(std::min(gb, 1024)), dim3(256), 0, ctx->stream, a, sort_keys, sort_vals);
      else KHG_LAUNCH(ctx, k3_sort_keys<false>, dim3(std::min(gb, 1024)), dim3(256), 0, ctx->stream, a, sort_keys, sort_vals);
      HIPCHK(hipcub::DeviceRadixSort::SortPairs(sort_tmp, need, sort_keys, sort_keys_out, sort_vals,
                                                reinterpret_cast<uint32_t*>(a.frame_ids), (int)Neff, 0, bits, ctx->stream));
      if (post) {
        K3Args b = a;
        b.num_tids = -1;
        KHG_LAUNCH(ctx, k3_bounds, dim3((m->P + 256) / 256), dim3(256), 0, ctx->stream, b, sort_keys_out);
      } else KHG_LAUNCH(ctx, k3_bounds, dim3((m->P + 256) / 256), dim3(256), 0, ctx->stream, a, sort_keys_out);
    }
  }
  return KHG_OK;
}
static int k3_make_work_items(khg_ctx* ctx, const khg_model* m, khg_utts* u, const K3Args& a, const K3Run& r, K3Item** items, int32_t** item_off) {
  if (r.max_items >= INT_MAX / 2) return khg_set_error(KHG_E_UNSUPPORTED, "khg_acc_stats: too many work items");
  const size_t n_items = (size_t)r.max_items, n_off = (size_t)m->P + 1, n_part = r.parked ? (size_t)r.max_slots * r.nsum1 : 0;
  int rc = KHG_OK;
  if (u->k3_items_n < n_items) { DEVFREE(u->k3_items_d); rc = u_alloc(u, reinterpret_cast<K3Item**>(&u->k3_items_d), 2 * n_items); if (rc) return rc; u->k3_items_n = n_items; }
  if (u->k3_item_off_n < n_off) { DEVFREE(u->k3_item_off_d); rc = u_alloc(u, &u->k3_item_off_d, 2 * n_off); if (rc) return rc; u->k3_item_off_n = n_off; }
  if (u->k3_part_n < n_part) { DEVFREE(u->k3_part_d); rc = u_alloc(u, &u->k3_part_d, n_part); if (rc) return rc; u->k3_part_n = n_part; }
  *items = reinterpret_cast<K3Item*>(u->k3_items_d) + (r.second ? u->k3_items_n : 0);
  *item_off = u->k3_item_off_d + (r.second ? u->k3_item_off_n : 0);
  KHG_LAUNCH(ctx, k3_make_items, dim3(1), dim3(1024), 0, ctx->stream, a, r.ny, r.target, (int)r.max_items, (int)std::min<int64_t>(r.max_slots, INT_MAX),
             *items, *item_off, r.cls_lo, r.cls_hi);
  return KHG_OK;
}
static int k3_run(khg_ctx* ctx, const khg_model* m, khg_utts* u, khg_accs* acc, K3Args& a, const K3Run& r, bool post, const char* timer, void* comm, int nparts) {
  if (r.too_wide) return khg_set_error(KHG_E_UNSUPPORTED, "khg_acc_stats: pdf too large for the LDS chunk buffers");
  const bool wave = r.form == K3F_WAVE;
  const bool wt = k3_weight_ordinary(a.weight);
  bool f16a = false;
  if (r.may_f16a && (wave || wt)) { int rs = k3_phase_a_scales(ctx, const_cast<khg_model*>(m), u, &f16a); if (rs) return rs; }
  const bool f16b = f16a && r.may_f16b && wt;
  k3_set_scales(a, m, f16a, f16b);
  const int variant = wave ? (f16b ? K3V_WAVE16 : K3V_WAVE) : r.form == K3F_VALU ? K3V_VALU : f16b ? K3V_BLOCK16 : K3V_MFMA;
  const int nwv = variant == K3V_BLOCK16 ? r.nwv16 : 4;
  const K3Kernel fn = k3_kernel(variant, m->KQ, variant == K3V_BLOCK16 ? r.NB16 : r.NB, nwv, post, f16a);
  const K3Kernel fin = wave ? k3_kernel(K3V_FINALIZE, m->KQ, r.NB, 4, false, false) : nullptr;
  if (!fn || (wave && !fin)) return khg_set_error(KHG_E_RUNTIME, "khg_acc_stats: no kernel for the planned form");
  const size_t lds = r.lds[f16b ? 2 : f16a ? 1 : 0];
  int rc = KHG_OK;
  if (wave && u->k3_llpart_n < (size_t)m->P) { DEVFREE(u->k3_llpart_d); rc = u_alloc(u, &u->k3_llpart_d, (size_t)m->P); if (rc) return rc; u->k3_llpart_n = (size_t)m->P; }
  K3Item* items = nullptr; int32_t* item_off = nullptr;
  rc = k3_make_work_items(ctx, m, u, a, r, &items, &item_off); if (rc) return rc;
  a.items = items; a.item_off = item_off;
  if (wave) {
    HIPCHK(hipMemsetAsync(u->k3_llpart_d, 0, sizeof(double) * (size_t)m->P, ctx->stream));
    a.ll_part = u->k3_llpart_d; a.part = u->k3_part_d;
  }
  rc = k3_for_ranges(ctx, m, acc, comm, nparts, [&](int p0, int np) -> int {
    a.pdf0 = p0; a.npdf = np;
    const unsigned nblk = (unsigned)((int64_t)std::min(np, r.n_cls) * r.ny + r.extra_blocks);
    KernelTimer kt(ctx, timer);
    int rl = k3_launch(ctx, fn, nblk, 64 * nwv, lds, a);
    if (!rl && wave) rl = k3_launch(ctx, fin, (unsigned)np, 256, 0, a);
    return rl;
  });
  if (rc) return rc;
  a.pdf0 = 0; a.npdf = m->P;
  if (wave) KHG_LAUNCH(ctx, k3_wave_scalars, dim3(1), dim3(1024), 0, ctx->stream, a, r.cls_lo, r.cls_hi);
  return KHG_OK;
}
static int acc_stats_pass(khg_ctx* ctx, const khg_model* m, const khg_tm* tm, khg_utts* u, float weight, khg_accs* acc, void* comm, int nparts, int64_t nsub,
                          int64_t npost = -1, bool one_block = false) {
  int rc = KHG_OK;
  const bool post = npost >= 0;
  const int64_t Neff = post ? npost : nsub < 0 ? u->N : nsub;
  if (!post) {
    HIPCHK(hipMemsetAsync(u->pdf_count_d, 0, sizeof(int32_t) * (size_t)m->P, ctx->stream));
    HIPCHK(hipMemsetAsync(u->tid_count_d, 0, sizeof(unsigned long long) * ((size_t)tm->num_tids + 1), ctx->stream));
  }
  K3Args a = k3_args(ctx, m, tm, u, acc, weight, post, Neff);
  nparts = std::max(1, std::min(nparts, m->P));
  if (comm && nparts > 1) { rc = ctx_comm_stream(ctx); if (rc) return rc; }
  if (Neff > 0) {
    rc = k3_bucket(ctx, m, tm, u, a, post, nsub, Neff); if (rc) return rc;
    const K3Plan pl = k3_plan(ctx, m, post, Neff, one_block);
    for (int i = 0; i < pl.nruns && !rc; ++i)
      rc = k3_run(ctx, m, u, acc, a, pl.run[i], post, nsub < 0 ? "k3_accumulate" : "k3_accumulate_pass2", i + 1 == pl.nruns ? comm : nullptr, nparts);
    if (rc) return rc;
    HIPCHK(hipGetLastError());
  } else {
    rc = k3_for_ranges(ctx, m, acc, nparts > 1 ? comm : nullptr, nparts, [](int, int) { return (int)KHG_OK; }); if (rc) return rc;
  }
  if (comm) {
    if (nparts > 1) rc = accs_allreduce_pieces(ctx, acc, m, -1, 0, comm, nullptr);
    else rc = khg_accs_allreduce(ctx, acc, comm);
    if (rc) return rc;
  }
  return KHG_OK;
}
static int acc_stats_impl(khg_ctx* ctx, const khg_model* m, const khg_tm* tm, khg_utts* u, float weight, khg_accs* acc, void* comm, int nparts) {
  if (ctx_dead(ctx) || !m || !tm || !u || !acc) return khg_set_error(KHG_E_ARG, "khg_acc_stats: bad arguments");
  { int rf = utts_foreign_ctx(ctx, u, "khg_acc_stats"); if (rf) return rf; }
  if (!u->ali_valid) return khg_set_error(KHG_E_ARG, "khg_acc_stats: no resident alignment (khg_align or khg_ali_upload first)");
  if (m->D != u->D || acc->D != m->D || acc->sumG != m->sumG || acc->num_tids != tm->num_tids)
    return khg_set_error(KHG_E_RUNTIME, "khg_acc_stats: accumulator / model / feature dimensions do not match");
  if (tm->max_pdf >= m->P) return khg_set_error(KHG_E_RUNTIME, "khg_acc_stats: transition model refers to pdf-ids the model does not have");
  int64_t nsub = -1;
  if (u->ali_pending && u->ali_split && u->N > 0) {
    HIPCHK(hipEventSynchronize(u->ev_dp));
    if (u->unc_cnt_h[0] == 0) u->ali_split = false;
    else nsub = u->unc_cnt_h[1];
  }
  int rc = nsub < 0 ? wait_ali(ctx, u) : KHG_OK;
  if (!rc) rc = arena_flush(ctx);
  if (rc) return rc;
  if (!u->frame_ids_d || u->k3_P != m->P || u->k3_tids != tm->num_tids) {
    DEVFREE(u->pdf_count_d); DEVFREE(u->pdf_cursor_d); DEVFREE(u->pdf_start_d); DEVFREE(u->tid_count_d); DEVFREE(u->frame_ids_d);
    rc = u_alloc(u, &u->pdf_count_d, (size_t)m->P);
    if (!rc) rc = u_alloc(u, &u->pdf_cursor_d, (size_t)m->P);
    if (!rc) rc = u_alloc(u, &u->pdf_start_d, (size_t)m->P + 1);
    if (!rc) rc = u_alloc(u, &u->tid_count_d, (size_t)tm->num_tids + 1);
    if (!rc) rc = u_alloc(u, &u->frame_ids_d, (size_t)u->N);
    if (rc) return rc;
    u->k3_P = m->P; u->k3_tids = tm->num_tids;
  }
  if (nsub < 0) return acc_stats_pass(ctx, m, tm, u, weight, acc, comm, nparts, -1);
  rc = acc_stats_pass(ctx, m, tm, u, weight, acc, nullptr, 1, -1);
  if (!rc) rc = wait_ali(ctx, u);
  if (!rc) rc = acc_stats_pass(ctx, m, tm, u, weight, acc, comm, nparts, nsub);
  return rc;
}
extern "C" int khg_acc_stats(khg_ctx* ctx, const khg_model* m, const khg_tm* tm, khg_utts* u, float weight, khg_accs* acc) {
  return acc_stats_impl(ctx, m, tm, u, weight, acc, nullptr, 1);
}
extern "C" int khg_acc_stats_reduce(khg_ctx* ctx, const khg_model* m, const khg_tm* tm, khg_utts* u, float weight, khg_accs* acc, void* comm, int32_t nparts) {
  return acc_stats_impl(ctx, m, tm, u, weight, acc, comm, nparts <= 0 ? 4 : nparts);
}

static int acc_stats_post_impl(const std::string& name, khg_ctx* ctx, const khg_model* m, const khg_tm* tm, khg_utts* u, const khg_posteriors* p, float scale,
                               khg_accs* acc, khg_accs* acc2, bool two, bool one_block = false) {
  const std::string who = name + ": ";
  if (ctx_dead(ctx) || !m || !tm || !u || !p || !acc || (two && !acc2)) return khg_set_error(KHG_E_ARG, who + "bad arguments");
  if (two && acc == acc2) return khg_set_error(KHG_E_ARG, who + "num_accs and den_accs are the same block");
  { int rf = utts_foreign_ctx(ctx, u, name.c_str()); if (rf) return rf; }
  PostInfo pi;
  posteriors_info(p, &pi);
  if (pi.ctx != ctx || m->ctx != ctx || tm->ctx != ctx || acc->ctx != ctx || u->ctx != ctx || (two && acc2->ctx != ctx))
    return khg_set_error(KHG_E_ARG, who + "a handle of another context");
  if (pi.U != u->n_utt)
    return khg_set_error(KHG_E_ARG, who + "the posteriors hold " + std::to_string(pi.U) + " utterances, the set " + std::to_string(u->n_utt));
  for (int i = 0; i < pi.U; ++i) {
    const int64_t tp = pi.frame_off[i + 1] - pi.frame_off[i], ts = u->frame_off[(size_t)i + 1] - u->frame_off[(size_t)i];
    if (tp != 0 && tp != ts)
      return khg_set_error(KHG_E_ARG, who + "utterance " + std::to_string(i) + " has " + std::to_string(tp) + " frames of posteriors and " + std::to_string(ts) + " frames of features");
  }
  if (m->D != u->D || acc->D != m->D || acc->sumG != m->sumG || acc->num_tids != tm->num_tids ||
      (two && (acc2->D != m->D || acc2->sumG != m->sumG || acc2->num_tids != tm->num_tids)))
    return khg_set_error(KHG_E_ARG, who + "accumulator / model / feature dimensions do not match");
  if (tm->max_pdf >= m->P) return khg_set_error(KHG_E_ARG, who + "transition model refers to pdf-ids the model does not have");
  if (!std::isfinite(scale)) return khg_set_error(KHG_E_ARG, who + "scale must be finite");
  if (pi.max_tid > tm->num_tids)
    return khg_set_error(KHG_E_ARG, who + "the posteriors hold transition-id " + std::to_string(pi.max_tid) + ", the transition model has " + std::to_string(tm->num_tids));
  const int64_t E = pi.entry_off[pi.U];
// ... 30 lines not shown
```

kaldi_hmm_gmm_amd/csrc/khg_k3_accstats.hip.inc:

```

struct K3Args {
  const float* feats;
  const int32_t* ali;
  const int32_t* id2pdf;
  int32_t num_tids;
  int64_t N;
  int32_t P, D;
  const int32_t* gauss_off;
  const float* gconsts;
  const float* means_invvars;
  const float* inv_vars;
  const float* nhalf_inv_vars;
  int32_t* pdf_count;
  int64_t* pdf_start;
  int32_t* pdf_cursor;
  int32_t* frame_ids;
  unsigned long long* tid_count;
  double* occ; double* mean_acc; double* var_acc; double* trans_acc; double* scalars;
  float weight;
  int32_t* err_flag;
  double* part;
  double* ll_part;
  int32_t pdf0, npdf;
  const struct K3Item* items;
  const int32_t* item_off;
  const int32_t* pa_ex;
  int32_t pa_S;
  float pa_scale, pa_inv, pa_c1;
  float pb_gscale;
  int32_t pb_SG;
  const int32_t* e_row;
  const float* e_w;
};

struct K3Item { int32_t pdf, y, ny, slot; };

__device__ __forceinline__ bool k3_take_item(const K3Args& a, K3Item& it) {
  const int i = a.item_off[a.pdf0] + (int)blockIdx.x;
  if (i >= a.item_off[a.pdf0 + a.npdf]) return false;
  it = a.items[i];
  return true;
}

#define K3_NYCAP 4096
__global__ __launch_bounds__(1024) void k3_make_items(K3Args a, int ny_base, int target_frames, int max_items, int max_slots, K3Item* items, int32_t* item_off,
                                                      int cls_lo, int cls_hi) {
  __shared__ int s_n[1024], s_s[1024];
  __shared__ int s_run[2];
  const int tid = threadIdx.x;
  if (tid == 0) { s_run[0] = 0; s_run[1] = 0; }
  __syncthreads();
  for (int base = 0; base < a.P; base += 1024) {
    const int p = base + tid;
    int n = 0;
    if (p < a.P) {
      const int64_t nfr = a.pdf_start[p + 1] - a.pdf_start[p];
      const int64_t c = (nfr + target_frames - 1) / target_frames;
      n = (int)(c > ny_base ? (c > K3_NYCAP ? K3_NYCAP : c) : ny_base);
      const int Gp = a.gauss_off[p + 1] - a.gauss_off[p];
      if (Gp <= cls_lo || Gp > cls_hi || nfr == 0) n = 0;
    }
    const int sl = n > 1 ? n : 0;
    s_n[tid] = n; s_s[tid] = sl;
    __syncthreads();
    for (int o = 1; o < 1024; o <<= 1) {
      const int vn = tid >= o ? s_n[tid - o] : 0, vs = tid >= o ? s_s[tid - o] : 0;
      __syncthreads();
      s_n[tid] += vn; s_s[tid] += vs;
      __syncthreads();
    }
    const int i0 = s_run[0] + s_n[tid] - n, sl0 = s_run[1] + s_s[tid] - sl;
    if (p < a.P) {
      item_off[p] = i0 < max_items ? i0 : max_items;
      if (i0 + n > max_items || sl0 + sl > max_slots) atomicOr(a.err_flag, 8);
      else for (int y = 0; y < n; ++y) items[i0 + y] = K3Item{p, y, n, sl ? sl0 + y : -1};
    }
    __syncthreads();
    if (tid == 1023) { s_run[0] += s_n[1023]; s_run[1] += s_s[1023]; }
    __syncthreads();
  }
  if (tid == 0) item_off[a.P] = s_run[0] < max_items ? s_run[0] : max_items;
}

#define K3_SEG 8
__global__ void k3_count(K3Args a) {
  const int64_t nseg = (a.N + K3_SEG - 1) / K3_SEG;
  int64_t sgi = (int64_t)blockIdx.x * blockDim.x + threadIdx.x;
  const int64_t stride = (int64_t)gridDim.x * blockDim.x;
  for (; sgi < nseg; sgi += stride) {
    const int64_t i0 = sgi * K3_SEG;
    const int n = (int)min((int64_t)K3_SEG, a.N - i0);
    int ctid = -1, ntid = 0, cpdf = -1, npdf = 0;
    for (int k = 0; k < n; ++k) {
      const int tid = a.ali[i0 + k];
      if (tid < 1 || tid > a.num_tids) continue;
      const int pdf = a.id2pdf[tid];
      if (pdf < 0 || pdf >= a.P) { atomicOr(a.err_flag, 4); continue; }
      if (tid != ctid) {
        if (ntid) atomicAdd(&a.tid_count[ctid], (unsigned long long)ntid);
        ctid = tid; ntid = 0;
      }
      ++ntid;
      if (pdf != cpdf) {
        if (npdf) atomicAdd(&a.pdf_count[cpdf], npdf);
        cpdf = pdf; npdf = 0;
      }
      ++npdf;
    }
    if (ntid) atomicAdd(&a.tid_count[ctid], (unsigned long long)ntid);
    if (npdf) atomicAdd(&a.pdf_count[cpdf], npdf);
  }
}

// ... 688 lines not shown
          ll[k][ft][r] = e;
          s += e;
        }
        s = k3_row_sum(s);
        if (j16 == 0) red[wave * K3_CHUNK + 16 * ft + 4 * q + r] = s;
      }
    k3_block_sync();
    if (tid < K3_CHUNK)
      fin[tid] = (red[tid] + red[K3_CHUNK + tid]) + (red[2 * K3_CHUNK + tid] + red[3 * K3_CHUNK + tid]);
    k3_block_sync();
#pragma unroll
    for (int ft = 0; ft < 4; ++ft)
#pragma unroll
      for (int r = 0; r < 4; ++r) {
        const int f = 16 * ft + 4 * q + r;
        const float ssum = fin[f];
        float wf = a.weight;
        if constexpr (POST) wf = wts[f];
        if (wave == 0 && j16 == 0 && f < cf) {
          const float llf = __logf(ssum) + mx[ft][r];
          if (!(fabsf(llf) <= 3.0e38f)) atomicOr(a.err_flag, 1);
          tot_ll += (double)(llf * wf);
          if constexpr (POST) tot_w += (double)wf;
        }
        const float scale = f < cf ? wf / ssum : 0.0f;
#pragma unroll
        for (int k = 0; k < NBW; ++k) ll[k][ft][r] = ll[k][ft][r] * scale;
      }
#pragma unroll
    for (int ft = 0; ft < 4; ++ft) {
#pragma unroll
      for (int s = 0; s < 4; ++s) {
        const int fr = 16 * ft + 4 * q + s;
        double ga[NBW];
#pragma unroll
        for (int k = 0; k < NBW; ++k) { ga[k] = (double)ll[k][ft][s]; occ[k] += ga[k]; }
#pragma unroll
        for (int db = 0; db < NDB; ++db) {
          const int col = 16 * db + j16;
          const int d = col < XP ? col : col - XP;
          const double bv = (double)xq[(((col < XP ? 0 : 2) + (d & 1)) * K3_CHUNK + fr) * KH + (d >> 1)];
#pragma unroll
          for (int k = 0; k < NBW; ++k)
            acc[k][db] = __builtin_amdgcn_mfma_f64_16x16x4f64(ga[k], bv, acc[k][db], 0, 0, 0);
        }
      }
    }
  }
#pragma unroll
  for (int k = 0; k < NBW; ++k) {
    const int gb = 16 * (wave + 4 * k);
#pragma unroll
    for (int db = 0; db < NDB; ++db) {
      const int col = 16 * db + j16;
#pragma unroll
      for (int r = 0; r < 4; ++r) {
        const int g = gb + q + 4 * r;
        if (g < G) {
          if (col < D) atomicAdd(a.mean_acc + (int64_t)(g0 + g) * D + col, acc[k][db][r]);
          else if (col >= XP && col - XP < D) atomicAdd(a.var_acc + (int64_t)(g0 + g) * D + (col - XP), acc[k][db][r]);
        }
      }
    }
    double o = occ[k];
    o += __shfl_xor(o, 16);
    o += __shfl_xor(o, 32);
    if (q == 0 && gb + j16 < G) atomicAdd(a.occ + g0 + gb + j16, o);
  }
  if (wave == 0) {
    for (int o2 = 32; o2 > 0; o2 >>= 1) tot_ll += __shfl_xor(tot_ll, o2);
    if (lane == 0 && tot_ll != 0.0) atomicAdd(&a.scalars[1], tot_ll);
  }
  if constexpr (POST) {
    if (wave == 0) {
      for (int o2 = 32; o2 > 0; o2 >>= 1) tot_w += __shfl_xor(tot_w, o2);
      if (lane == 0 && tot_w != 0.0) atomicAdd(&a.scalars[0], tot_w);
    }
  } else {
    if (tid == 0 && it.y == 0) atomicAdd(&a.scalars[0], (double)nfr * (double)a.weight);
  }
}

typedef _Float16 k3_f16x8 __attribute__((ext_vector_type(8)));
#define K3_XH_ROW 104

template <int NB>
__device__ __forceinline__ void k3_wave_flush(const K3Args& a, const double* sum, int g0, int G, int D, int tid) {
  constexpr int XP = 40;
  for (int i = tid; i < NB * 16 * 2 * XP; i += 256) {
    const int g = i / (2 * XP), col = i - g * (2 * XP);
    if (g < G) {
      if (col < D) atomicAdd(a.mean_acc + (int64_t)(g0 + g) * D + col, sum[i]);
      else if (col >= XP && col - XP < D) atomicAdd(a.var_acc + (int64_t)(g0 + g) * D + (col - XP), sum[i]);
    }
  }
  if (tid < NB * 16 && tid < G) atomicAdd(a.occ + g0 + tid, sum[NB * 16 * 2 * XP + tid]);
}

__device__ __forceinline__ void k3_lds_sync() {
  asm volatile("s_waitcnt lgkmcnt(0)" ::: "memory");
  __builtin_amdgcn_wave_barrier();
}

template <int NB, bool F16A = false>
__global__ __launch_bounds__(256, NB <= 2 ? 2 : 1) void k3_accumulate_wave(K3Args a) {
  extern __shared__ __attribute__((aligned(16))) float k3s[];
  constexpr int KQ = 10, XP = 4 * KQ, KH = 2 * KQ, NDB = KQ / 2, TF = 16;
  K3Item it;
  if (!k3_take_item(a, it)) return;
  const int pdf = it.pdf;
  const int64_t beg = a.pdf_start[pdf];
  const int nfr = (int)(a.pdf_start[pdf + 1] - beg);
  if (nfr == 0) return;
  const int D = a.D;
  const int g0 = a.gauss_off[pdf], G = a.gauss_off[pdf + 1] - g0;
  const int tid = threadIdx.x, lane = tid & 63;
  const int wave = __builtin_amdgcn_readfirstlane(tid >> 6);
  const int j16 = lane & 15, q = lane >> 4;
  float* Wl = k3s;
  float* xw = (F16A ? k3s : Wl + NB * KH * 64) + wave * (4 * TF * KH);
  _Float16* xh = reinterpret_cast<_Float16*>(k3s + 4 * (4 * TF * KH)) + wave * (2 * TF * K3_XH_ROW);
  float gcv[NB];
#pragma unroll
  for (int k = 0; k < NB; ++k) gcv[k] = (16 * k + j16 < G) ? a.gconsts[g0 + 16 * k + j16] : -INFINITY;
  float wq[F16A ? 1 : NB][F16A ? 1 : KH];
  k3_f16x8 w1[F16A ? NB : 1][3], w2[F16A ? NB : 1][3];
  if constexpr (!F16A) {
    for (int idx = tid; idx < NB * KH * 64; idx += 256) {
      const int l = idx & 63, s = (idx >> 6) % KH, k = idx / (64 * KH);
      const int g = 16 * k + (l & 15), qq = l >> 4, d = 2 * s + (qq & 1);
      float v = 0.0f;
      if (g < G && d < D) v = (qq & 2) ? a.nhalf_inv_vars[(int64_t)(g0 + g) * D + d] : a.means_invvars[(int64_t)(g0 + g) * D + d];
      Wl[idx] = v;
    }
    __syncthreads();
#pragma unroll
    for (int k = 0; k < NB; ++k)
#pragma unroll
      for (int s = 0; s < KH; ++s) wq[k][s] = Wl[(k * KH + s) * 64 + lane];
  } else {
#pragma unroll
    for (int k = 0; k < NB; ++k)
#pragma unroll
      for (int st = 0; st < 3; ++st) {
        k3_f16x8 p1, p2;
#pragma unroll
        for (int e = 0; e < 8; ++e) {
          const int kp = 32 * st + 8 * q + e, var = kp >= XP, d = var ? kp - XP : kp, g = 16 * k + j16;
          float v = 0.0f;
          if (kp < 2 * XP && g < G && d < D) {
            const float w = var ? a.nhalf_inv_vars[(int64_t)(g0 + g) * D + d] : a.means_invvars[(int64_t)(g0 + g) * D + d];
            v = ldexpf(w, a.pa_S - a.pa_ex[2 * d + var]);
          }
          const _Float16 h1 = (_Float16)v;
          p1[e] = h1; p2[e] = (_Float16)(v - (float)h1);
        }
        w1[k][st] = p1; w2[k][st] = p2;
      }
#pragma unroll
    for (int k = 0; k < NB; ++k) gcv[k] = gcv[k] * a.pa_scale;
    for (int i = lane; i < 2 * TF * K3_XH_ROW; i += 64) xh[i] = (_Float16)0.0f;
    k3_lds_sync();
  }
  (void)Wl; (void)wq; (void)w1; (void)w2;

  f64x4 acc[NB][NDB];
// ... 90 lines not shown
      }
    }
#pragma unroll
    for (int r = 0; r < 4; ++r) {
      float m = ll[0][r];
#pragma unroll
      for (int k = 1; k < NB; ++k) m = fmaxf(m, ll[k][r]);
      m = k3_row_max(m);
      float ssum = 0.0f;
#pragma unroll
      for (int k = 0; k < NB; ++k) {
        const float e = __builtin_amdgcn_exp2f((ll[k][r] - m) * (F16A ? a.pa_c1 : 1.44269504088896340736f));
        ll[k][r] = e;
        ssum += e;
      }
      ssum = k3_row_sum(ssum);
      const int f = 4 * q + r;
      if (j16 == 0 && f < cf) {
        const float llf = __logf(ssum) + (F16A ? m * a.pa_inv : m);
        if (!(fabsf(llf) <= 3.0e38f)) atomicOr(a.err_flag, 1);
        tot_ll += (double)(llf * a.weight);
      }
      const float scale = f < cf ? a.weight / ssum : 0.0f;
#pragma unroll
      for (int k = 0; k < NB; ++k) ll[k][r] = ll[k][r] * scale;
    }
#pragma unroll
    for (int s = 0; s < 4; ++s) {
      const int fr = 4 * q + s;
      double ga[NB];
#pragma unroll
      for (int k = 0; k < NB; ++k) { ga[k] = (double)ll[k][s]; occ[k] += ga[k]; }
#pragma unroll
      for (int db = 0; db < NDB; ++db) {
        const int col = 16 * db + j16;
        const int d = col < XP ? col : col - XP;
        const double bv = (double)xw[(((col < XP ? 0 : 2) + (d & 1)) * TF + fr) * KH + (d >> 1)];
#pragma unroll
        for (int k = 0; k < NB; ++k)
          acc[k][db] = __builtin_amdgcn_mfma_f64_16x16x4f64(ga[k], bv, acc[k][db], 0, 0, 0);
      }
    }
    k3_lds_sync();
  }
  __syncthreads();
  double* sum = reinterpret_cast<double*>(k3s);
  constexpr int NSUM = NB * 16 * 2 * XP + NB * 16;
  for (int i = tid; i < NSUM; i += 256) sum[i] = 0.0;
  __syncthreads();
#pragma unroll 1
  for (int w = 0; w < 4; ++w) {
    if (wave == w) {
#pragma unroll
      for (int k = 0; k < NB; ++k) {
#pragma unroll
        for (int db = 0; db < NDB; ++db) {
          const int col = 16 * db + j16;
#pragma unroll
          for (int r = 0; r < 4; ++r) atomicAdd(&sum[(16 * k + q + 4 * r) * (2 * XP) + col], acc[k][db][r]);
        }
        double o = occ[k];
        o += __shfl_xor(o, 16);
        o += __shfl_xor(o, 32);
        if (q == 0) atomicAdd(&sum[NB * 16 * 2 * XP + 16 * k + j16], o);
      }
    }
    __syncthreads();
  }
  __shared__ double s_ll[4];
  for (int o2 = 32; o2 > 0; o2 >>= 1) tot_ll += __shfl_xor(tot_ll, o2);
  if (lane == 0) s_ll[wave] = tot_ll;
  __syncthreads();
  const double block_ll = ((s_ll[0] + s_ll[1]) + s_ll[2]) + s_ll[3];
  if (it.ny == 1) {
    k3_wave_flush<NB>(a, sum, g0, G, D, tid);
    if (tid == 0) a.ll_part[pdf] = block_ll;
  } else {
    double* dst = a.part + (int64_t)it.slot * (NSUM + 1);
    for (int i = tid; i < NSUM; i += 256) dst[i] = sum[i];
    if (tid == 0) dst[NSUM] = block_ll;
  }
}

template <int NB>
__global__ __launch_bounds__(256, 1) void k3_accumulate_wave16(K3Args a) {
  extern __shared__ __attribute__((aligned(16))) float k3s[];
  constexpr int KQ = 10, XP = 4 * KQ, NDB = KQ / 2, TF = 16;
  constexpr int XHH = 2 * TF * K3_XH_ROW;
  constexpr int XTR = 36, XTH = 2 * 2 * XP * XTR;
  K3Item it;
  if (!k3_take_item(a, it)) return;
  const int pdf = it.pdf;
  const int64_t beg = a.pdf_start[pdf];
  const int nfr = (int)(a.pdf_start[pdf + 1] - beg);
  if (nfr == 0) return;
  const int D = a.D;
  const int g0 = a.gauss_off[pdf], G = a.gauss_off[pdf + 1] - g0;
  const int tid = threadIdx.x, lane = tid & 63;
  const int wave = __builtin_amdgcn_readfirstlane(tid >> 6);
  const int j16 = lane & 15, q = lane >> 4;
  _Float16* xh = reinterpret_cast<_Float16*>(k3s) + wave * (2 * XHH + XTH);
  _Float16* xt = xh + 2 * XHH;
  float gcv[NB];
#pragma unroll
  for (int k = 0; k < NB; ++k) gcv[k] = ((16 * k + j16 < G) ? a.gconsts[g0 + 16 * k + j16] : -INFINITY) * a.pa_scale;
  char* wl16 = reinterpret_cast<char*>(reinterpret_cast<_Float16*>(k3s) + 4 * (2 * XHH + XTH));
  for (int e0 = tid; e0 < NB * 3 * 64; e0 += 256) {
    const int l = e0 & 63, st = (e0 >> 6) % 3, k = e0 / (3 * 64), jl = l & 15, ql = l >> 4;
    k3_f16x8 p1, p2;
#pragma unroll
    for (int e = 0; e < 8; ++e) {
      const int kp = 32 * st + 8 * ql + e, var = kp >= XP, d = var ? kp - XP : kp, g = 16 * k + jl;
      float v = 0.0f;
      if (kp < 2 * XP && g < G && d < D) {
        const float w = var ? a.nhalf_inv_vars[(int64_t)(g0 + g) * D + d] : a.means_invvars[(int64_t)(g0 + g) * D + d];
        v = ldexpf(w, a.pa_S - a.pa_ex[2 * d + var]);
      }
      const _Float16 h1 = (_Float16)v;
      p1[e] = h1; p2[e] = (_Float16)(v - (float)h1);
    }
    *reinterpret_cast<k3_f16x8*>(wl16 + (((k * 3 + st) * 2 + 0) * 64 + l) * 16) = p1;
    *reinterpret_cast<k3_f16x8*>(wl16 + (((k * 3 + st) * 2 + 1) * 64 + l) * 16) = p2;
  }
  {
    static_assert((2 * XHH + XTH) % 8 == 0, "the wave's planes are whole 16-byte words");
    const k3_f16x8 z = {0, 0, 0, 0, 0, 0, 0, 0};
    for (int i = lane; i < (2 * XHH + XTH) / 8; i += 64) reinterpret_cast<k3_f16x8*>(xh)[i] = z;
  }
  __syncthreads();

  f64x4 acc[NB][NDB];
  double occ[NB];
#pragma unroll
  for (int k = 0; k < NB; ++k) {
    occ[k] = 0.0;
#pragma unroll
    for (int db = 0; db < NDB; ++db) acc[k][db] = f64x4{0, 0, 0, 0};
  }
  double tot_ll = 0.0;
  unsigned bad = 0;
  const int ntile = (nfr + TF - 1) / TF, npair = (ntile + 1) / 2;
  constexpr int NM = 2 * TF * XP / (4 * 64);
  static_assert(NM * 4 * 64 == 2 * TF * XP, "micro-tiles cover the pair exactly");
  const int pstride = 4 * it.ny;
  float pre[NM][4];
  float sx[NM][2], sx2[NM][2];
  const bool even_d = (D & 1) == 0;
#pragma unroll
  for (int j = 0; j < NM; ++j)
#pragma unroll
    for (int c = 0; c < 2; ++c) {
      const int d = min(2 * ((lane + 64 * j) % 20) + c, D - 1);
      sx[j][c] = ldexpf(1.0f, a.pa_ex[2 * d]); sx2[j][c] = ldexpf(1.0f, a.pa_ex[2 * d + 1]);
    }
  const float gs = a.pb_gscale;
  const int rot = (int)(((unsigned)pdf * 2654435761u) % (unsigned)npair);
  auto pair_of = [&](int p) { const int x = p + rot; return x >= npair ? x - npair : x; };
  auto cf_of = [&](int pl, int tau) { if (pl >= npair) return 0; const int t = 2 * pair_of(pl) + tau; return t < ntile ? min(TF, nfr - t * TF) : 0; };
  auto fid_of = [&](int pl, int tau) -> int {
    const int n = cf_of(pl, tau);
    const int t = pl < npair ? 2 * pair_of(pl) + tau : 0;
    return lane < n ? a.frame_ids[beg + t * TF + lane] : 0;
  };
  auto request = [&](int fid0, int fid1) {
    int fa[NM], fb[NM];
#pragma unroll
    for (int j = 0; j < NM; ++j) {
      const int i = lane + 64 * j, tau = i / 160, fp = (i % 160) / 20;
      if (j < 2) { fa[j] = __shfl(fid0, 2 * fp); fb[j] = __shfl(fid0, 2 * fp + 1); }
      else if (j > 2) { fa[j] = __shfl(fid1, 2 * fp); fb[j] = __shfl(fid1, 2 * fp + 1); }
      else {
        const int a0 = __shfl(fid0, 2 * fp), a1 = __shfl(fid1, 2 * fp), b0 = __shfl(fid0, 2 * fp + 1), b1 = __shfl(fid1, 2 * fp + 1);
        fa[j] = tau ? a1 : a0; fb[j] = tau ? b1 : b0;
      }
    }
#pragma unroll
    for (int j = 0; j < NM; ++j) {
      const int d0 = 2 * ((lane + 64 * j) % 20);
      if (even_d) {
        typedef float f2 __attribute__((ext_vector_type(2)));
        const int dd = min(d0, D - 2);
        const f2 va = *reinterpret_cast<const f2*>(a.feats + (int64_t)fa[j] * D + dd), vb = *reinterpret_cast<const f2*>(a.feats + (int64_t)fb[j] * D + dd);
        pre[j][0] = va[0]; pre[j][1] = va[1]; pre[j][2] = vb[0]; pre[j][3] = vb[1];
      } else {
        const int da = min(d0, D - 1), db = min(d0 + 1, D - 1);
        pre[j][0] = a.feats[(int64_t)fa[j] * D + da]; pre[j][1] = a.feats[(int64_t)fa[j] * D + db];
        pre[j][2] = a.feats[(int64_t)fb[j] * D + da]; pre[j][3] = a.feats[(int64_t)fb[j] * D + db];
      }
    }
  };
  int p = it.y * 4 + wave;
  int fidn0 = 0, fidn1 = 0;
  if (p < npair) { request(fid_of(p, 0), fid_of(p, 1)); fidn0 = fid_of(p + pstride, 0); fidn1 = fid_of(p + pstride, 1); }
  for (; p < npair; p += pstride) {
    const int cf[2] = {cf_of(p, 0), cf_of(p, 1)};
#pragma unroll
    for (int j = 0; j < NM; ++j) {
      typedef _Float16 h2v __attribute__((ext_vector_type(2)));
      const int i = lane + 64 * j, tau = i / 160, r = i % 160, f0 = 2 * (r / 20), d0 = 2 * (r % 20);
      const int cft = tau ? cf[1] : cf[0];
      _Float16 h1[4], h2[4], g1[4], g2[4];
#pragma unroll
      for (int e = 0; e < 4; ++e) {
        const int f = f0 + (e >> 1), d = d0 + (e & 1);
        const float v = (f < cft && d < D) ? pre[j][e] : 0.0f;
        const float s1 = v * sx[j][e & 1], s2 = (v * v) * sx2[j][e & 1];
        h1[e] = (_Float16)s1; g1[e] = (_Float16)s2;
        h2[e] = (_Float16)(s1 - (float)h1[e]); g2[e] = (_Float16)(s2 - (float)g1[e]);
      }
#pragma unroll
      for (int ff = 0; ff < 2; ++ff) {
        _Float16* r1 = xh + tau * XHH + (f0 + ff) * K3_XH_ROW + d0;
        *reinterpret_cast<h2v*>(r1) = h2v{h1[2 * ff], h1[2 * ff + 1]};
        *reinterpret_cast<h2v*>(r1 + TF * K3_XH_ROW) = h2v{h2[2 * ff], h2[2 * ff + 1]};
        *reinterpret_cast<h2v*>(r1 + XP) = h2v{g1[2 * ff], g1[2 * ff + 1]};
        *reinterpret_cast<h2v*>(r1 + TF * K3_XH_ROW + XP) = h2v{g2[2 * ff], g2[2 * ff + 1]};
      }
#pragma unroll
      for (int dd = 0; dd < 2; ++dd) {
        _Float16* c1 = xt + (d0 + dd) * XTR + tau * TF + f0;
        *reinterpret_cast<h2v*>(c1) = h2v{h1[dd], h1[2 + dd]};
        *reinterpret_cast<h2v*>(c1 + 2 * XP * XTR) = h2v{h2[dd], h2[2 + dd]};
        *reinterpret_cast<h2v*>(c1 + XP * XTR) = h2v{g1[dd], g1[2 + dd]};
        *reinterpret_cast<h2v*>(c1 + 2 * XP * XTR + XP * XTR) = h2v{g2[dd], g2[2 + dd]};
      }
    }
    if (p + pstride < npair) { request(fidn0, fidn1); fidn0 = fid_of(p + 2 * pstride, 0); fidn1 = fid_of(p + 2 * pstride, 1); }
    k3_lds_sync();
    f32x4 ll[2][NB];
#pragma unroll
    for (int tau = 0; tau < 2; ++tau)
#pragma unroll
      for (int k = 0; k < NB; ++k) ll[tau][k] = f32x4{gcv[k], gcv[k], gcv[k], gcv[k]};
#pragma unroll
    for (int st = 0; st < 3; ++st) {
      k3_f16x8 x1[2], x2[2];
#pragma unroll
      for (int tau = 0; tau < 2; ++tau) {
        x1[tau] = *reinterpret_cast<const k3_f16x8*>(xh + tau * XHH + j16 * K3_XH_ROW + 32 * st + 8 * q);
        x2[tau] = *reinterpret_cast<const k3_f16x8*>(xh + tau * XHH + (TF + j16) * K3_XH_ROW + 32 * st + 8 * q);
      }
#pragma unroll
      for (int k = 0; k < NB; ++k) {
        const k3_f16x8 wa = *reinterpret_cast<const k3_f16x8*>(wl16 + (((k * 3 + st) * 2 + 0) * 64 + lane) * 16);
        const k3_f16x8 wb = *reinterpret_cast<const k3_f16x8*>(wl16 + (((k * 3 + st) * 2 + 1) * 64 + lane) * 16);
#pragma unroll
        for (int tau = 0; tau < 2; ++tau) {
          ll[tau][k] = __builtin_amdgcn_mfma_f32_16x16x32_f16(x2[tau], wa, ll[tau][k], 0, 0, 0);
          ll[tau][k] = __builtin_amdgcn_mfma_f32_16x16x32_f16(x1[tau], wb, ll[tau][k], 0, 0, 0);
          ll[tau][k] = __builtin_amdgcn_mfma_f32_16x16x32_f16(x1[tau], wa, ll[tau][k], 0, 0, 0);
        }
      }
    }
#pragma unroll
    for (int tau = 0; tau < 2; ++tau) {
#pragma unroll
      for (int r = 0; r < 4; ++r) {
        float m = ll[tau][0][r];
#pragma unroll
        for (int k = 1; k < NB; ++k) m = fmaxf(m, ll[tau][k][r]);
        m = k3_row_max(m);
        float ssum = 0.0f;
#pragma unroll
        for (int k = 0; k < NB; ++k) {
          const float e = __builtin_amdgcn_exp2f((ll[tau][k][r] - m) * a.pa_c1);
          ll[tau][k][r] = e;
          ssum += e;
        }
        ssum = k3_row_sum(ssum);
        const int f = 4 * q + r;
        const bool counts = (j16 == 0) & (f < cf[tau]);
        const float llf = __logf(ssum) + m * a.pa_inv;
        bad |= (counts & !(fabsf(llf) <= 3.0e38f)) ? 1u : 0u;
        tot_ll += counts ? (double)(llf * a.weight) : 0.0;
        const float scale = f < cf[tau] ? a.weight / ssum : 0.0f;
#pragma unroll
        for (int k = 0; k < NB; ++k) ll[tau][k][r] = ll[tau][k][r] * scale;
      }
    }
    k3_f16x8 ga1[NB], ga2[NB];
    f32x4 prev[NB];
#pragma unroll
    for (int k = 0; k < NB; ++k) {
#pragma unroll
      for (int e = 0; e < 8; ++e) {
        const float g = e < 4 ? ll[0][k][e] : ll[1][k][e - 4];
        occ[k] += (double)g;
        const float gsc = g * gs;
        const _Float16 h1 = (_Float16)gsc;
        ga1[k][e] = h1; ga2[k][e] = (_Float16)(gsc - (float)h1);
      }
    }
#pragma unroll
    for (int db = 0; db < NDB; ++db) {
      const _Float16* cb = xt + (16 * db + j16) * XTR + 4 * q;
      k3_f16x8 xb1, xb2;
      {
        typedef _Float16 h4 __attribute__((ext_vector_type(4)));
        const h4 a0 = *reinterpret_cast<const h4*>(cb), a1 = *reinterpret_cast<const h4*>(cb + TF);
        const h4 b0 = *reinterpret_cast<const h4*>(cb + 2 * XP * XTR), b1 = *reinterpret_cast<const h4*>(cb + 2 * XP * XTR + TF);
#pragma unroll
        for (int e = 0; e < 4; ++e) { xb1[e] = a0[e]; xb1[4 + e] = a1[e]; xb2[e] = b0[e]; xb2[4 + e] = b1[e]; }
      }
      f32x4 cur[NB];
#pragma unroll
      for (int k = 0; k < NB; ++k) {
        f32x4 c = f32x4{0, 0, 0, 0};
        c = __builtin_amdgcn_mfma_f32_16x16x32_f16(ga1[k], xb2, c, 0, 0, 0);
        c = __builtin_amdgcn_mfma_f32_16x16x32_f16(ga2[k], xb1, c, 0, 0, 0);
        c = __builtin_amdgcn_mfma_f32_16x16x32_f16(ga1[k], xb1, c, 0, 0, 0);
        cur[k] = c;
      }
      if (db > 0) {
#pragma unroll
        for (int k = 0; k < NB; ++k)
#pragma unroll
          for (int r = 0; r < 4; ++r) acc[k][db - 1][r] += (double)prev[k][r];
      }
#pragma unroll
      for (int k = 0; k < NB; ++k) prev[k] = cur[k];
    }
#pragma unroll
    for (int k = 0; k < NB; ++k)
#pragma unroll
      for (int r = 0; r < 4; ++r) acc[k][NDB - 1][r] += (double)prev[k][r];
    k3_lds_sync();
  }
  __syncthreads();
  double* sum = reinterpret_cast<double*>(k3s);
  constexpr int NSUM = NB * 16 * 2 * XP + NB * 16;
  for (int i = tid; i < NSUM; i += 256) sum[i] = 0.0;
  __syncthreads();
  int unscale[NDB];
#pragma unroll
  for (int db = 0; db < NDB; ++db) {
    const int col = 16 * db + j16, var = col >= XP, d = min(var ? col - XP : col, D - 1);
    unscale[db] = -(a.pb_SG + a.pa_ex[2 * d + var]);
  }
#pragma unroll 1
  for (int ph = 0; ph < 4; ++ph) {
    const int kk = (wave + ph) & 3;
#pragma unroll
    for (int k = 0; k < NB; ++k) {
      if (k != kk) continue;
#pragma unroll
      for (int db = 0; db < NDB; ++db) {
        const int col = 16 * db + j16;
#pragma unroll
        for (int r = 0; r < 4; ++r) atomicAdd(&sum[(16 * k + 4 * q + r) * (2 * XP) + col], ldexp(acc[k][db][r], unscale[db]));
      }
      double o = occ[k];
      o += __shfl_xor(o, 16);
      o += __shfl_xor(o, 32);
      if (q == 0) atomicAdd(&sum[NB * 16 * 2 * XP + 16 * k + j16], o);
    }
    __syncthreads();
  }
  if (bad) atomicOr(a.err_flag, 1);
  __shared__ double s_ll[4];
  for (int o2 = 32; o2 > 0; o2 >>= 1) tot_ll += __shfl_xor(tot_ll, o2);
  if (lane == 0) s_ll[wave] = tot_ll;
  __syncthreads();
  const double block_ll = ((s_ll[0] + s_ll[1]) + s_ll[2]) + s_ll[3];
  if (it.ny == 1) {
    k3_wave_flush<NB>(a, sum, g0, G, D, tid);
    if (tid == 0) a.ll_part[pdf] = block_ll;
  } else {
    double* dst = a.part + (int64_t)it.slot * (NSUM + 1);
    for (int i = tid; i < NSUM; i += 256) dst[i] = sum[i];
    if (tid == 0) dst[NSUM] = block_ll;
  }
}

#ifndef K3B16_KO
#define K3B16_KO 0
#endif
template <int KQ, int NBW, int NWV>
__global__ __launch_bounds__(64 * NWV, 1) void k3_accumulate_block16(K3Args a) {
  constexpr int NT = 64 * NWV;
  extern __shared__ __attribute__((aligned(16))) float k3s[];
  constexpr int XP = 4 * KQ;
  constexpr int K2 = 2 * XP;
  constexpr int KPAD = (K2 + 31) / 32 * 32, KST = KPAD / 32;
// ... 358 lines not shown
```

kaldi_hmm_gmm_amd/csrc/khg_pybind.cpp:

```cpp
#include <chrono>

#include <pybind11/numpy.h>
#include <pybind11/pybind11.h>
#include <pybind11/stl.h>

#include <cstdint>
#include <cstring>
#include <limits>
#include <string>
#include <vector>

#include "../../include/khg_hip.h"
#include "khg_py_ebw.hpp"
#include "khg_py_lattices.hpp"

namespace py = pybind11;

namespace {

py::object g_khg_error;

void Check(int rc) {
  if (rc == KHG_OK) return;
  const char* msg = khg_last_error();
  if (g_khg_error && !g_khg_error.is_none()) {
    PyErr_SetString(g_khg_error.ptr(), msg ? msg : "khg error");
    throw py::error_already_set();
  }
  throw std::runtime_error(msg ? msg : "khg error");
}

template <class F>
int NoGil(F&& f) {
  py::gil_scoped_release release;
  return f();
}

template <class T>
using Arr = py::array_t<T, py::array::c_style | py::array::forcecast>;

template <class T>
Arr<T> Zeros(std::vector<py::ssize_t> shape) {
  Arr<T> a(shape);
  std::memset(a.mutable_data(), 0, sizeof(T) * (size_t)a.size());
  return a;
}

struct KContext {
  khg_ctx* h = nullptr;
  int device = 0;
  KContext(int dev, py::object stream) : device(dev) {
    void* st = stream.is_none() ? nullptr : reinterpret_cast<void*>(stream.cast<uintptr_t>());
    Check(khg_ctx_create(dev, st, &h));
  }
  ~KContext() { close(); }
  void close() { if (h) { khg_ctx_destroy(h); h = nullptr; } }
  void sync() { Check(NoGil([&] { return khg_ctx_sync(h); })); }
  void set_timing(bool on) { Check(khg_ctx_set_timing(h, on ? 1 : 0)); }
  void set_k1_form(const std::string& f) {
    int v = f == "auto" ? KHG_K1_AUTO : (f == "pdf" || f == "fp32") ? KHG_K1_FP32_PDF : f == "utt" ? KHG_K1_FP32_UTT : f == "f16x2" ? KHG_K1_F16X2 : f == "f16x2s" ? KHG_K1_F16X2S : -1;
    if (v < 0) throw py::key_error(f);
    Check(khg_ctx_set_k1_form(h, v));
  }
  static int opt_id(const py::object& o) {
    if (py::isinstance<py::int_>(o)) return o.cast<int>();
    static const char* names[KHG_OPT_COUNT] = {"k1_form", "k1_order", "k1_nf", "k1p_ts", "k1_interleave", "k1_dbg", "k2_inorder", "k2_ks", "k2_serial",
                                               "k2_prof", "k3_bucket", "k3_form", "k3_phase_b", "k3_ny", "debug", "k3_phase_a", "k2_split", "k2s_hub", "lat_ops_lds", "k1_launch", "k1_pgrid", "k1_prof", "k2_ladder"};
    const std::string n = o.cast<std::string>();
    for (int i = 0; i < KHG_OPT_COUNT; ++i) if (n == names[i]) return i;
    if (n == "scratch_bytes") return KHG_INFO_SCRATCH_BYTES;
    if (n == "scratch_blocks") return KHG_INFO_SCRATCH_BLOCKS;
    throw py::key_error(n);
  }
  int get_option(py::object name) { int v = 0; Check(khg_ctx_get_option(h, opt_id(name), &v)); return v; }
  int set_option(py::object name, int value) {
    const int id = opt_id(name);
    int old = 0;
    Check(khg_ctx_get_option(h, id, &old));
    Check(khg_ctx_set_option(h, id, value));
    return old;
  }
  py::list timings() {
    const int cap = 4096;
    std::vector<char> names(1 << 16);
    std::vector<float> ms(cap);
    int32_t n = 0;
    Check(khg_ctx_get_timings(h, names.data(), (int64_t)names.size(), ms.data(), cap, &n));
    py::list out;
    const char* p = names.data();
    for (int i = 0; i < n && i < cap; ++i) {
      const char* e = std::strchr(p, '\n');
      std::string nm = e ? std::string(p, e) : std::string(p);
      out.append(py::make_tuple(nm, ms[i]));
      if (!e) break;
      p = e + 1;
    }
    return out;
  }
};

struct KComm {
  void* h = nullptr;
  int nranks = 1, rank = 0;
  static py::bytes unique_id() {
    char id[KHG_COMM_ID_BYTES];
    Check(khg_comm_unique_id(id));
    return py::bytes(id, KHG_COMM_ID_BYTES);
  }
  KComm(KContext& ctx, int n, int r, py::bytes uid) : nranks(n), rank(r) {
    std::string s = uid;
    if (s.size() != KHG_COMM_ID_BYTES) throw py::value_error("Comm: the id is 128 bytes");
    Check(NoGil([&] { return khg_comm_create(ctx.h, n, r, s.data(), &h); }));
  }
  py::dict info() {
    int32_t n = 0, r = -1, v = 0;
    Check(khg_comm_info(h, &n, &r, &v));
    py::dict d;
    d["nranks"] = n; d["rank"] = r; d["version"] = v;
    return d;
  }
  ~KComm() { close(); }
  void close() { if (h) { khg_comm_destroy(h); h = nullptr; } }
};

struct KAccs;

struct KModel {
  khg_model* h = nullptr;
  py::object ctx_obj;
  KContext* ctx;
  int num_pdfs = 0, dim = 0;
  Arr<int32_t> gauss_off;
  KModel(py::object ctx_o, Arr<int32_t> go, Arr<float> gc, Arr<float> miv, Arr<float> iv, py::object weights)
      : ctx_obj(ctx_o), ctx(ctx_o.cast<KContext*>()), gauss_off(go) {
    num_pdfs = (int)go.shape(0) - 1;
    if (miv.ndim() != 2 || iv.ndim() != 2 || miv.shape(0) != iv.shape(0) || miv.shape(1) != iv.shape(1) || num_pdfs < 1 ||
        miv.shape(0) != go.at(num_pdfs) || gc.shape(0) != miv.shape(0))
      throw py::value_error("DeviceModel: inconsistent shapes");
    dim = (int)miv.shape(1);
    Check(khg_model_create(ctx->h, num_pdfs, dim, go.data(), gc.data(), miv.data(), iv.data(), &h));
    if (!weights.is_none()) set_weights(weights.cast<Arr<float>>());
  }
  ~KModel() { close(); }
  void close() { if (h) { khg_model_destroy(h); h = nullptr; } }
  int64_t sumG() const { return gauss_off.at(num_pdfs); }
  void set_weights(Arr<float> w) {
    if (w.shape(0) != sumG()) throw py::value_error("set_weights: one weight per Gaussian");
    Check(khg_model_set_weights(ctx->h, h, w.data()));
  }
  py::dict mle_update(KAccs& accs, py::object opts, int flags);
// ... 409 lines not shown
    Arr<int32_t> keys({K1, (py::ssize_t)N + 1});
    Arr<double> cnt({K1}), x({K1, (py::ssize_t)dim}), x2({K1, (py::ssize_t)dim});
    Check(NoGil([&] { return khg_tree_stats_download(ctx->h, h, keys.mutable_data(), cnt.mutable_data(), x.mutable_data(), x2.mutable_data()); }));
    py::dict d;
    const py::slice sl(0, K, 1);
    d["keys"] = py::array(keys)[sl]; d["count"] = py::array(cnt)[sl]; d["x"] = py::array(x)[sl]; d["x2"] = py::array(x2)[sl];
    return d;
  }
  void upload(Arr<int32_t> keys, Arr<double> cnt, Arr<double> x, Arr<double> x2) {
    const py::ssize_t K = cnt.size();
    if (keys.size() != K * (N + 1) || x.size() != K * dim || x2.size() != K * dim)
      throw py::value_error("DeviceTreeStats.upload: keys [num_keys, N + 1], count [num_keys], x and x2 [num_keys, dim]");
    Check(NoGil([&] { return khg_tree_stats_upload(ctx->h, h, (int64_t)K, keys.data(), cnt.data(), x.data(), x2.data()); }));
  }
  void add(float scale, KTreeStats& src) { Check(NoGil([&] { return khg_tree_stats_add(ctx->h, h, scale, src.h); })); }
};

struct KUtts {
  khg_utts* h = nullptr;
  py::object ctx_obj, keep, keep_model;
  KContext* ctx;
  Arr<int64_t> frame_off;
  int n_utt = 0, dim = 0;
  int64_t state_total = 0;
  KUtts(py::object ctx_o, py::object tm, Arr<int64_t> fo, py::object feats, py::object dim_o, py::object graphs, py::object graph)
      : ctx_obj(ctx_o), ctx(ctx_o.cast<KContext*>()), frame_off(fo) {
    if (!graphs.is_none() && !graph.is_none()) throw py::value_error("UtteranceSet: exactly one of graphs / graph");
    n_utt = (int)fo.shape(0) - 1;
    const float* feats_h = nullptr;
    const float* feats_d = nullptr;
    Arr<float> fh;
    if (py::isinstance<py::tuple>(feats)) {
      py::tuple t = feats;
      feats_d = reinterpret_cast<const float*>(t[0].cast<uintptr_t>());
      keep = t[1];
      if (dim_o.is_none()) throw py::value_error("UtteranceSet: dim is required with device features");
      dim = dim_o.cast<int>();
    } else {
      fh = feats.cast<Arr<float>>();
      if (fh.ndim() != 2 || fh.shape(0) != fo.at(n_utt)) throw py::value_error("UtteranceSet: feats must be [frames, dim]");
      dim = (int)fh.shape(1);
      feats_h = fh.data();
    }
    const khg_tm* tmh = tm.is_none() ? nullptr : tm.cast<KTransitions*>()->h;
    if (!graph.is_none()) {
      khg_graph* gh = reinterpret_cast<khg_graph*>(graph.attr("h").cast<uintptr_t>());
      if (!gh) throw py::value_error("UtteranceSet: the DecodingGraph is closed");
      Check(khg_utts_create_on_graph(ctx->h, tmh, gh, n_utt, dim, fo.data(), feats_h, feats_d, &h));
      state_total = graph.attr("num_states").cast<int64_t>() * n_utt;
    } else if (graphs.is_none()) {
      Check(khg_utts_create(ctx->h, tmh, n_utt, dim, fo.data(), feats_h, feats_d, nullptr, nullptr, nullptr, nullptr, nullptr, nullptr,
                            nullptr, nullptr, &h));
    } else {
      py::dict g = graphs;
      auto so = g["state_off"].cast<Arr<int64_t>>(); auto st = g["start"].cast<Arr<int32_t>>();
      auto ao = g["arc_off"].cast<Arr<int64_t>>(); auto il = g["ilabel"].cast<Arr<int32_t>>();
      auto ol = g["olabel"].cast<Arr<int32_t>>(); auto w = g["weight"].cast<Arr<float>>();
      auto ns = g["nextstate"].cast<Arr<int32_t>>(); auto fin = g["final"].cast<Arr<float>>();
      Check(khg_utts_create(ctx->h, tmh, n_utt, dim, fo.data(), feats_h, feats_d, so.data(), st.data(), ao.data(), il.data(), ol.data(),
                            w.data(), ns.data(), fin.data(), &h));
      state_total = so.at(n_utt);
    }
  }
  ~KUtts() { close(); }
  void close() { if (h) { khg_utts_destroy(h); h = nullptr; } }
  void set_pdf_list(Arr<int32_t> p) { Check(khg_utts_set_pdf_list(h, (int32_t)p.shape(0), p.data())); }
  void features_changed() { Check(khg_utts_features_changed(h)); }
  py::tuple pdf_lists() {
    Arr<int64_t> off({(py::ssize_t)n_utt + 1});
    Check(khg_utts_num_pdfs(h, off.mutable_data()));
    const py::ssize_t n = off.at(n_utt);
    Arr<int32_t> pdfs({n > 0 ? n : 1});
    Check(khg_utts_pdfs(h, pdfs.mutable_data()));
    return py::make_tuple(off, py::array(pdfs)[py::slice(0, n, 1)]);
  }
  py::dict k2_plan(py::object ctx_o) {
    int32_t o[8];
    Check(khg_utts_k2_plan(ctx_o.cast<KContext*>()->h, h, o));
    py::dict d;
    d["KS"] = o[0]; d["DEG"] = o[1]; d["FAST"] = o[2] != 0; d["GMEM"] = o[3] != 0; d["SC"] = o[4] != 0;
    d["nthr"] = o[5]; d["lds_bytes"] = o[6]; d["faithful_form"] = o[7];
    return d;
  }
  bool k2_ladder(py::object ctx_o) {
    int32_t o = 0;
    Check(khg_utts_k2_ladder(ctx_o.cast<KContext*>()->h, h, &o));
    return o != 0;
  }
  py::object pdf_first_frames() {
    Arr<int64_t> off({(py::ssize_t)n_utt + 1});
    Check(khg_utts_num_pdfs(h, off.mutable_data()));
    const py::ssize_t n = off.at(n_utt);
    Arr<int32_t> first({n > 0 ? n : 1});
    Check(khg_utts_pdf_first(h, first.mutable_data()));
    return py::array(first)[py::slice(0, n, 1)];
  }
  py::object pdf_last_frames() {
    Arr<int64_t> off({(py::ssize_t)n_utt + 1});
    Check(khg_utts_num_pdfs(h, off.mutable_data()));
    const py::ssize_t n = off.at(n_utt);
    Arr<int32_t> last({n > 0 ? n : 1});
    Check(khg_utts_pdf_last(h, last.mutable_data()));
    return py::array(last)[py::slice(0, n, 1)];
  }
  void loglikes(KModel& m, bool reachable_only, bool band) {
    keep_model = band ? py::cast(&m) : py::object();
    Check(NoGil([&] { return band ? khg_loglikes_band(ctx->h, m.h, h) : reachable_only ? khg_loglikes_reachable(ctx->h, m.h, h) : khg_loglikes(ctx->h, m.h, h); }));
  }
  py::tuple loglikes_layout() {
    Arr<int64_t> off({(py::ssize_t)n_utt + 1});
    int64_t tot = 0;
    Check(khg_loglikes_layout(h, off.mutable_data(), &tot));
    return py::make_tuple(off, tot);
  }
  py::list download_loglikes() {
    Arr<int64_t> off({(py::ssize_t)n_utt + 1}), poff({(py::ssize_t)n_utt + 1});
    int64_t tot = 0;
    Check(khg_loglikes_layout(h, off.mutable_data(), &tot));
    Check(khg_utts_num_pdfs(h, poff.mutable_data()));
    std::vector<float> buf((size_t)(tot > 0 ? tot : 1));
    Check(NoGil([&] { return khg_loglikes_download(ctx->h, h, buf.data()); }));
    py::list out;
    for (int u = 0; u < n_utt; ++u) {
      const int64_t T = frame_off.at(u + 1) - frame_off.at(u), tpad = (T + 31) / 32 * 32, n = poff.at(u + 1) - poff.at(u);
      Arr<float> m({(py::ssize_t)n, (py::ssize_t)T});
      for (int64_t j = 0; j < n; ++j) std::memcpy(m.mutable_data() + j * T, buf.data() + off.at(u) + j * tpad, sizeof(float) * (size_t)T);
      out.append(m);
    }
    return out;
  }
  void upload_loglikes(py::list mats) {
    Arr<int64_t> off({(py::ssize_t)n_utt + 1});
    int64_t tot = 0;
    Check(khg_loglikes_layout(h, off.mutable_data(), &tot));
    std::vector<float> buf((size_t)(tot > 0 ? tot : 1), 0.0f);
    for (int u = 0; u < n_utt && u < (int)mats.size(); ++u) {
      Arr<float> m = mats[u].cast<Arr<float>>();
      const int64_t T = frame_off.at(u + 1) - frame_off.at(u), tpad = (T + 31) / 32 * 32;
      for (py::ssize_t j = 0; j < m.shape(0); ++j) std::memcpy(buf.data() + off.at(u) + j * tpad, m.data() + j * m.shape(1), sizeof(float) * (size_t)T);
    }
    Check(NoGil([&] { return khg_loglikes_upload(ctx->h, h, buf.data()); }));
  }
  py::dict decode_lattice_faster(KTransitions& tm, float beam, int32_t max_active, int32_t min_active, float lattice_beam, int32_t prune_interval,
                                 float beam_delta, float hash_ratio, float prune_scale, float acoustic_scale, bool allow_partial, int32_t scratch_per_frame) {
    khg_lattice_faster_config c;
    khg_lattice_faster_config_default(&c);
    c.beam = beam; c.max_active = max_active; c.min_active = min_active; c.lattice_beam = lattice_beam; c.prune_interval = prune_interval;
    c.beam_delta = beam_delta; c.hash_ratio = hash_ratio; c.prune_scale = prune_scale; c.acoustic_scale = acoustic_scale;
    c.allow_partial = allow_partial ? 1 : 0; c.scratch_per_frame = scratch_per_frame;
    const int64_t N = frame_off.at(n_utt), wcap = 2 * N + 1024 * (int64_t)n_utt + 1024;
    Arr<int32_t> ali({(py::ssize_t)(N > 0 ? N : 1)}), words({(py::ssize_t)wcap}), status({(py::ssize_t)n_utt});
    Arr<int64_t> woff({(py::ssize_t)n_utt + 1});
    Arr<double> like({(py::ssize_t)n_utt});
    Check(NoGil([&] { return khg_decode_lattice_faster(ctx->h, tm.h, h, &c, ali.mutable_data(), words.mutable_data(), woff.mutable_data(), wcap,
                                                       like.mutable_data(), status.mutable_data()); }));
    py::dict d;
    d["ali"] = py::array(ali)[py::slice(0, N, 1)];
    d["like"] = like; d["status"] = status;
    d["words"] = py::array(words)[py::slice(0, woff.at(n_utt), 1)];
    d["words_off"] = woff;
    return d;
  }
  py::dict raw_lattice_faster_impl(KTransitions& tm, float beam, int32_t max_active, int32_t min_active, float lattice_beam, int32_t prune_interval,
                                   float beam_delta, float hash_ratio, float prune_scale, float acoustic_scale, bool allow_partial,
                                   int32_t scratch_per_frame, bool device) {
    khg_lattice_faster_config c;
// ... 264 lines not shown
    norm_args("add_deltas", na, ua, status, &st, &sp);
    Check(NoGil([&] { return khg_utts_add_deltas(ctx->h, h, order, window, (int32_t)na.shape(0), ua.data(), na.data(), sp, reinterpret_cast<float*>(out)); }));
  }
};

}

void BindHost(py::module_& m, py::object* error_class);

PYBIND11_MODULE(_kaldi_hmm_gmm_amd, m) {
  m.doc() = "pybind11 host surface of libkhg_hip.so (include/khg_hip.h): the accelerated EM hot path of kaldi-hmm-gmm on MI355X";
  m.def("_set_error_class", [](py::object cls) { g_khg_error = cls; });
  BindHost(m, &g_khg_error);
  m.def("version", [] { return khg_version(); });
  m.attr("ALIGN_DONE") = KHG_ALIGN_DONE; m.attr("ALIGN_ERROR") = KHG_ALIGN_ERROR; m.attr("ALIGN_RETRIED") = KHG_ALIGN_RETRIED;
  m.attr("ALIGN_EXACT_DP") = KHG_ALIGN_EXACT_DP; m.attr("ALIGN_FALLBACK") = KHG_ALIGN_FALLBACK;

  py::class_<KContext>(m, "Context")
      .def(py::init<int, py::object>(), py::arg("device") = 0, py::arg("stream") = py::none())
      .def_property_readonly("h", [](KContext& c) { return reinterpret_cast<uintptr_t>(c.h); })
      .def_readonly("device", &KContext::device)
      .def("sync", &KContext::sync).def("set_timing", &KContext::set_timing).def("timings", &KContext::timings)
      .def("set_k1_form", &KContext::set_k1_form).def("set_option", &KContext::set_option, py::arg("name"), py::arg("value"))
      .def("get_option", &KContext::get_option, py::arg("name")).def("close", &KContext::close);

  py::class_<KComm>(m, "Comm")
      .def_static("unique_id", &KComm::unique_id)
      .def(py::init<KContext&, int, int, py::bytes>(), py::arg("ctx"), py::arg("nranks"), py::arg("rank"), py::arg("uid"), py::keep_alive<1, 2>())
      .def_property_readonly("h", [](KComm& c) { return reinterpret_cast<uintptr_t>(c.h); })
      .def_readonly("nranks", &KComm::nranks).def_readonly("rank", &KComm::rank).def("close", &KComm::close).def("info", &KComm::info)
      .def_property_readonly_static("ID_BYTES", [](py::object) { return KHG_COMM_ID_BYTES; });

  py::class_<KModel>(m, "DeviceModel")
      .def(py::init<py::object, Arr<int32_t>, Arr<float>, Arr<float>, Arr<float>, py::object>(), py::arg("ctx"), py::arg("gauss_off"),
           py::arg("gconsts"), py::arg("means_invvars"), py::arg("inv_vars"), py::arg("weights") = py::none())
      .def_property_readonly("h", [](KModel& x) { return reinterpret_cast<uintptr_t>(x.h); })
      .def_readonly("ctx", &KModel::ctx_obj).def_readonly("num_pdfs", &KModel::num_pdfs).def_readonly("dim", &KModel::dim)
      .def_readonly("gauss_off", &KModel::gauss_off)
      .def("set_weights", &KModel::set_weights)
      .def("mle_update", &KModel::mle_update, py::arg("accs"), py::arg("opts") = py::none(), py::arg("flags") = 0x7)
      .def("mle_update_sharded", &KModel::mle_update_sharded, py::arg("accs"), py::arg("opts") = py::none(), py::arg("flags") = 0x7,
           py::arg("comm") = py::none())
      .def("mle_update_range", &KModel::mle_update_range, py::arg("accs"), py::arg("opts"), py::arg("flags"), py::arg("first_pdf"), py::arg("n_pdf"))
      .def("mle_rows_download", &KModel::mle_rows_download).def("mle_rows_upload", &KModel::mle_rows_upload)
      .def("mle_update_finish", &KModel::mle_update_finish)
      .def("ebw_update", &KModel::ebw_update, py::arg("num_accs"), py::arg("den_accs"), py::arg("opts") = py::none(),
           py::arg("weight_opts") = py::none(), py::arg("flags") = 0x7)
      .def("scale_weights", &KModel::scale_weights)
      .def("invalidate", &KModel::invalidate)
      .def("transform_means", &KModel::transform_means, py::arg("M"))
      .def("split", &KModel::split, py::arg("targets"), py::arg("perturb_factor"), py::arg("randn"))
      .def("merge", &KModel::merge, py::arg("targets"))
      .def("download", &KModel::download, py::arg("weights") = true)
      .def("close", &KModel::close);

  py::class_<KTransitions>(m, "DeviceTransitions")
      .def(py::init<py::object, Arr<int32_t>>(), py::arg("ctx"), py::arg("id2pdf"))
      .def_property_readonly("h", [](KTransitions& x) { return reinterpret_cast<uintptr_t>(x.h); })
      .def_readonly("ctx", &KTransitions::ctx_obj).def_readonly("id2pdf", &KTransitions::id2pdf).def_readonly("num_tids", &KTransitions::num_tids)
      .def("set_trans_cost", &KTransitions::set_trans_cost).def("close", &KTransitions::close);

  py::class_<KAccs>(m, "DeviceAccs")
      .def(py::init<py::object, KModel&, KTransitions&>(), py::arg("ctx"), py::arg("model"), py::arg("tm"))
      .def_property_readonly("h", [](KAccs& x) { return reinterpret_cast<uintptr_t>(x.h); })
      .def_readonly("ctx", &KAccs::ctx_obj).def_readonly("sumG", &KAccs::sumG).def_readonly("dim", &KAccs::dim)
      .def_readonly("num_tids", &KAccs::num_tids).def_readonly("size", &KAccs::size)
      .def("zero", &KAccs::zero).def("device_ptr", &KAccs::device_ptr)
      .def("allreduce", &KAccs::allreduce, py::arg("comm") = py::none(), py::arg("wire_fp32") = false)
      .def("allreduce_range", &KAccs::allreduce_range, py::arg("model"), py::arg("first_pdf"), py::arg("n_pdf"), py::arg("comm") = py::none())
      .def("split", &KAccs::split).def("relayout", &KAccs::relayout).def("download_range", &KAccs::download_range)
      .def("download_occ", [](KAccs& a) { return a.download_range(0, a.sumG); })
      .def("download_trans", &KAccs::download_trans).def("download", &KAccs::download).def("upload", &KAccs::upload)
      .def("add", &KAccs::add, py::arg("scale"), py::arg("src")).def("scale", &KAccs::scale, py::arg("f"))
      .def("smooth_with_accum", &KAccs::smooth_with_accum, py::arg("tau"), py::arg("src"), py::arg("model"), py::arg("count") = true)
      .def("close", &KAccs::close);

  py::class_<KUtts>(m, "UtteranceSet")
      .def(py::init<py::object, py::object, Arr<int64_t>, py::object, py::object, py::object, py::object>(), py::arg("ctx"), py::arg("tm"), py::arg("frame_off"),
           py::arg("feats"), py::arg("dim") = py::none(), py::arg("graphs") = py::none(), py::arg("graph") = py::none())
      .def_property_readonly("graph_bytes", [](KUtts& x) { int64_t b = 0; Check(khg_utts_graph_bytes(x.h, &b)); return b; })
      .def_property_readonly("h", [](KUtts& x) { return reinterpret_cast<uintptr_t>(x.h); })
      .def_readonly("ctx", &KUtts::ctx_obj).def_readonly("frame_off", &KUtts::frame_off).def_readonly("n_utt", &KUtts::n_utt)
      .def_readonly("dim", &KUtts::dim)
      .def("set_pdf_list", &KUtts::set_pdf_list).def("features_changed", &KUtts::features_changed).def("pdf_lists", &KUtts::pdf_lists).def("k2_plan", &KUtts::k2_plan, py::arg("ctx")).def("k2_ladder", &KUtts::k2_ladder, py::arg("ctx")).def("pdf_first_frames", &KUtts::pdf_first_frames)
      .def("pdf_last_frames", &KUtts::pdf_last_frames)
      .def("loglikes", &KUtts::loglikes, py::arg("model"), py::arg("reachable_only") = false, py::arg("band") = false)
      .def("loglikes_layout", &KUtts::loglikes_layout).def("download_loglikes", &KUtts::download_loglikes)
      .def("upload_loglikes", &KUtts::upload_loglikes)
      .def("align", &KUtts::align, py::arg("tm"), py::arg("beam") = 200.0f, py::arg("retry_beam") = 0.0f, py::arg("acoustic_scale") = 1.0f,
           py::arg("careful") = false, py::arg("max_active") = (int64_t)std::numeric_limits<int32_t>::max(), py::arg("min_active") = 20,
           py::arg("beam_delta") = 0.5f, py::arg("hash_ratio") = 2.0f, py::arg("download") = true)
      .def("decode_lattice_faster", &KUtts::decode_lattice_faster, py::arg("tm"), py::arg("beam") = 16.0f,
           py::arg("max_active") = std::numeric_limits<int32_t>::max(), py::arg("min_active") = 200, py::arg("lattice_beam") = 10.0f,
           py::arg("prune_interval") = 25, py::arg("beam_delta") = 0.5f, py::arg("hash_ratio") = 2.0f, py::arg("prune_scale") = 0.1f,
           py::arg("acoustic_scale") = 1.0f, py::arg("allow_partial") = true, py::arg("scratch_per_frame") = 0)
      .def("raw_lattice_faster", &KUtts::raw_lattice_faster, py::arg("tm"), py::arg("beam") = 16.0f,
           py::arg("max_active") = std::numeric_limits<int32_t>::max(), py::arg("min_active") = 200, py::arg("lattice_beam") = 10.0f,
           py::arg("prune_interval") = 25, py::arg("beam_delta") = 0.5f, py::arg("hash_ratio") = 2.0f, py::arg("prune_scale") = 0.1f,
           py::arg("acoustic_scale") = 1.0f, py::arg("allow_partial") = true, py::arg("scratch_per_frame") = 0)
      .def("raw_lattices_faster_device", &KUtts::raw_lattices_faster_device, py::arg("tm"), py::arg("beam") = 16.0f,
           py::arg("max_active") = std::numeric_limits<int32_t>::max(), py::arg("min_active") = 200, py::arg("lattice_beam") = 10.0f,
           py::arg("prune_interval") = 25, py::arg("beam_delta") = 0.5f, py::arg("hash_ratio") = 2.0f, py::arg("prune_scale") = 0.1f,
           py::arg("acoustic_scale") = 1.0f, py::arg("allow_partial") = true, py::arg("scratch_per_frame") = 0)
      .def("decode_lattice_simple", &KUtts::decode_lattice_simple, py::arg("tm"), py::arg("beam") = 16.0f, py::arg("lattice_beam") = 10.0f,
           py::arg("prune_interval") = 25, py::arg("prune_scale") = 0.1f, py::arg("acoustic_scale") = 1.0f, py::arg("allow_partial") = true,
           py::arg("scratch_per_frame") = 0)
      .def("raw_lattice_simple", &KUtts::raw_lattice_simple, py::arg("tm"), py::arg("beam") = 16.0f, py::arg("lattice_beam") = 10.0f,
           py::arg("prune_interval") = 25, py::arg("prune_scale") = 0.1f, py::arg("acoustic_scale") = 1.0f, py::arg("scratch_per_frame") = 0)
      .def("raw_lattices_simple_device", &KUtts::raw_lattices_simple_device, py::arg("tm"), py::arg("beam") = 16.0f, py::arg("lattice_beam") = 10.0f,
           py::arg("prune_interval") = 25, py::arg("prune_scale") = 0.1f, py::arg("acoustic_scale") = 1.0f, py::arg("scratch_per_frame") = 0)
      .def("upload_ali", &KUtts::upload_ali).def("download_ali", &KUtts::download_ali)
      .def("acc_stats", &KUtts::acc_stats, py::arg("model"), py::arg("tm"), py::arg("accs"), py::arg("weight") = 1.0f)
      .def("acc_stats_post", &KUtts::acc_stats_post, py::arg("model"), py::arg("tm"), py::arg("post"), py::arg("accs"), py::arg("scale") = 1.0f)
      .def("acc_stats_post2", &KUtts::acc_stats_post2, py::arg("model"), py::arg("tm"), py::arg("post"), py::arg("num_accs"), py::arg("den_accs"),
           py::arg("scale") = 1.0f)
      .def("acc_stats_reduce", &KUtts::acc_stats_reduce, py::arg("model"), py::arg("tm"), py::arg("accs"), py::arg("weight") = 1.0f,
           py::arg("comm") = py::none(), py::arg("nparts") = 4)
      .def("acc_fmllr_stats_post", &KUtts::acc_fmllr_stats_post, py::arg("model"), py::arg("tm"), py::arg("post"), py::arg("utt2spk"), py::arg("stats"),
           py::arg("scale") = 1.0f)
      .def("acc_mllt_stats_post", &KUtts::acc_mllt_stats_post, py::arg("model"), py::arg("tm"), py::arg("post"), py::arg("stats"), py::arg("scale") = 1.0f)
      .def("acc_lda_stats_post", &KUtts::acc_lda_stats_post, py::arg("tm"), py::arg("post"), py::arg("stats"), py::arg("scale") = 1.0f)
      .def("_acc_tree_stats", &KUtts::acc_tree_stats, py::arg("tid2phone"), py::arg("tid2pdf_class"), py::arg("tid_flags"), py::arg("ci_phones"), py::arg("stats"))
      .def("splice_transform_feats", &KUtts::splice_transform_feats, py::arg("left"), py::arg("right"), py::arg("M"), py::arg("out"))
      .def("transform_feats", &KUtts::transform_feats, py::arg("utt2spk"), py::arg("W"), py::arg("out") = py::none(), py::arg("n_spk") = 0)
      .def("acc_cmvn_stats", &KUtts::acc_cmvn_stats, py::arg("utt2spk"), py::arg("stats"))
      .def("apply_cmvn", &KUtts::apply_cmvn, py::arg("utt2spk"), py::arg("norm"), py::arg("status") = py::none(), py::arg("out") = py::none())
      .def("add_deltas", &KUtts::add_deltas, py::arg("order"), py::arg("window"), py::arg("out"), py::arg("norm") = py::none(), py::arg("utt2spk") = py::none(),
           py::arg("status") = py::none())
      .def("close", &KUtts::close);

  py::class_<KFmllrStats>(m, "DeviceFmllrStats")
      .def(py::init<py::object, int, int>(), py::arg("ctx"), py::arg("n_spk"), py::arg("dim"))
      .def_property_readonly("h", [](KFmllrStats& x) { return reinterpret_cast<uintptr_t>(x.h); })
      .def_readonly("ctx", &KFmllrStats::ctx_obj).def_readonly("n_spk", &KFmllrStats::n_spk).def_readonly("dim", &KFmllrStats::dim)
      .def("zero", &KFmllrStats::zero).def("download", &KFmllrStats::download)
      .def("upload", &KFmllrStats::upload, py::arg("beta"), py::arg("K"), py::arg("G"))
      .def("add", &KFmllrStats::add, py::arg("scale"), py::arg("src"))
      .def("estimate", &KFmllrStats::estimate, py::arg("min_count") = 500.0, py::arg("num_iters") = 40, py::arg("W_d") = py::none())
      .def("set_chunk_frames", &KFmllrStats::set_chunk_frames, py::arg("frames")).def("num_chunks", &KFmllrStats::num_chunks)
      .def("close", &KFmllrStats::close);

  py::class_<KMlltStats>(m, "DeviceMlltStats")
      .def(py::init<py::object, int>(), py::arg("ctx"), py::arg("dim"))
      .def_property_readonly("h", [](KMlltStats& x) { return reinterpret_cast<uintptr_t>(x.h); })
      .def_readonly("ctx", &KMlltStats::ctx_obj).def_readonly("dim", &KMlltStats::dim)
      .def("zero", &KMlltStats::zero).def("download", &KMlltStats::download)
      .def("upload", &KMlltStats::upload, py::arg("beta"), py::arg("G"))
      .def("add", &KMlltStats::add, py::arg("scale"), py::arg("src"))
      .def("set_chunk_frames", &KMlltStats::set_chunk_frames, py::arg("frames")).def("num_chunks", &KMlltStats::num_chunks)
      .def("close", &KMlltStats::close);

  py::class_<KLdaStats>(m, "DeviceLdaStats")
      .def(py::init<py::object, int, int, int, int>(), py::arg("ctx"), py::arg("num_classes"), py::arg("dim"), py::arg("left") = 4, py::arg("right") = 4)
      .def_property_readonly("h", [](KLdaStats& x) { return reinterpret_cast<uintptr_t>(x.h); })
      .def_readonly("ctx", &KLdaStats::ctx_obj).def_readonly("num_classes", &KLdaStats::num_classes).def_readonly("dim", &KLdaStats::dim)
      .def_readonly("left", &KLdaStats::left).def_readonly("right", &KLdaStats::right).def_readonly("dim_z", &KLdaStats::dim_z)
      .def("zero", &KLdaStats::zero).def("download", &KLdaStats::download)
      .def("upload", &KLdaStats::upload, py::arg("zero_acc"), py::arg("first_acc"), py::arg("total_second_acc"))
      .def("add", &KLdaStats::add, py::arg("scale"), py::arg("src"))
      .def("set_chunk_frames", &KLdaStats::set_chunk_frames, py::arg("frames")).def("num_chunks", &KLdaStats::num_chunks)
      .def("close", &KLdaStats::close);

  py::class_<KCmvnStats>(m, "DeviceCmvnStats")
      .def(py::init<py::object, int, int>(), py::arg("ctx"), py::arg("n_spk"), py::arg("dim"))
      .def_property_readonly("h", [](KCmvnStats& x) { return reinterpret_cast<uintptr_t>(x.h); })
      .def_readonly("ctx", &KCmvnStats::ctx_obj).def_readonly("n_spk", &KCmvnStats::n_spk).def_readonly("dim", &KCmvnStats::dim)
      .def("zero", &KCmvnStats::zero).def("download", &KCmvnStats::download)
// ... 213 lines not shown
```

kaldi_hmm_gmm_amd/csrc/khg_utts.hip:

```cpp
#include "khg_internal.hpp"

static void plan_ll(khg_utts* u) {
  u->ll_off.assign(u->n_utt + 1, 0);
  for (int i = 0; i < u->n_utt; ++i) {
    int64_t T = u->frame_off[i + 1] - u->frame_off[i];
    int64_t tpad = (T + 31) & ~int64_t(31);
    u->ll_off[i + 1] = u->ll_off[i] + (u->pdf_off[i + 1] - u->pdf_off[i]) * tpad;
  }
  u->ll_total = u->ll_off[u->n_utt];
}

struct GraphTables {
  std::vector<int64_t> in_off;
  std::vector<int32_t> in_src, in_col, in_tid, in_ol, out_inidx;
  std::vector<float> in_w;
  void size(int64_t NS, int64_t NA) {
    in_off.assign((size_t)NS + 1, 0);
    in_src.resize((size_t)NA); in_col.resize((size_t)NA); in_tid.resize((size_t)NA); in_ol.resize((size_t)NA); out_inidx.resize((size_t)NA);
    in_w.resize((size_t)NA);
  }
};
struct GraphFacts {
  int32_t max_indeg = 0, max_outdeg = 0;
  bool same_col = true, has_eps = false;
// ... 286 lines not shown
  if (rc) { khg_graph_release(g); return rc; }
  g->device_bytes = graph_table_bytes(1, S, A);
  *out = g;
  return KHG_OK;
}
void khg_graph_release(khg_graph* g) {
  if (!g || --g->refs > 0) return;
  DEVFREE(g->state_off_d); DEVFREE(g->start_d); DEVFREE(g->in_off_d); DEVFREE(g->out_off_d); DEVFREE(g->in_src_d); DEVFREE(g->in_col_d);
  DEVFREE(g->in_tid_d); DEVFREE(g->in_olabel_d); DEVFREE(g->out_inidx_d); DEVFREE(g->in_w_d); DEVFREE(g->final_d);
  delete g;
}
extern "C" int khg_graph_destroy(khg_graph* g) {
  khg_graph_release(g);
  return KHG_OK;
}
extern "C" int khg_graph_info(const khg_graph* g, int64_t* num_states, int64_t* num_arcs, int32_t* num_pdfs, int32_t* max_in_degree,
                              int64_t* device_bytes) {
  if (!g) return khg_set_error(KHG_E_ARG, "khg_graph_info: bad arguments");
  if (num_states) *num_states = g->S;
  if (num_arcs) *num_arcs = g->A;
  if (num_pdfs) *num_pdfs = (int32_t)g->pdfs.size();
  if (max_in_degree) *max_in_degree = g->max_indeg;
  if (device_bytes) *device_bytes = g->device_bytes;
  return KHG_OK;
}

extern "C" int khg_utts_create_on_graph(khg_ctx* ctx, const khg_tm* tm, khg_graph* g, int32_t n_utt, int32_t D, const int64_t* frame_off,
                                        const float* feats_h, const float* feats_dv, khg_utts** out) {
  (void)tm;
  if (ctx_dead(ctx) || !out || !g || n_utt <= 0 || D <= 0 || !frame_off || (!feats_h && !feats_dv))
    return khg_set_error(KHG_E_ARG, "khg_utts_create_on_graph: bad arguments");
  if (g->ctx != ctx)
    return khg_set_error(KHG_E_ARG, "khg_utts_create_on_graph: a decoding graph must be used with the context that created it");
  khg_utts* u = nullptr;
  int rc = utts_begin("khg_utts_create_on_graph", ctx, n_utt, D, frame_off, feats_h, feats_dv, g->S <= 32768 && g->A <= 65536, &u);
  if (rc) return rc;
  u->has_graphs = true;
  u->graph = g; ++g->refs;
  u->state_off.assign({0, g->S});
  u->max_states = (int32_t)g->S; u->max_inarcs = (int32_t)g->A; u->max_indeg = g->max_indeg; u->max_outdeg = g->max_outdeg;
  u->has_eps = g->has_eps; u->same_col = g->same_col; u->ladder = g->ladder;
  u->bp_off.assign(n_utt + 1, 0); u->path_off.assign(n_utt + 1, 0); u->words_off.assign(n_utt + 1, 0);
  GraphFacts gf;
  gf.pdfs = g->pdfs; gf.pdf_first = g->pdf_first; gf.pdf_dfin = g->pdf_dfin; gf.nwords = g->nwords;
  for (int i = 0; i < n_utt; ++i) plan_utt_on_graph(u, i, frame_off[i + 1] - frame_off[i], g->S, gf);
  u->state_off_d = g->state_off_d; u->start_d = g->start_d; u->in_off_d = g->in_off_d; u->out_off_d = g->out_off_d;
  u->in_src_d = g->in_src_d; u->in_col_d = g->in_col_d; u->in_tid_d = g->in_tid_d; u->in_olabel_d = g->in_olabel_d;
  u->out_inidx_d = g->out_inidx_d; u->in_w_d = g->in_w_d; u->final_d = g->final_d;
  std::vector<int32_t> gidx((size_t)n_utt, 0);
  rc = u_upload(ctx, u, &u->gidx_d, gidx);
  if (!rc) rc = u_upload(ctx, u, &u->bp_off_d, u->bp_off);
  if (!rc) rc = u_upload(ctx, u, &u->path_off_d, u->path_off);
  if (!rc) rc = u_upload(ctx, u, &u->words_off_d, u->words_off);
  if (rc) { khg_utts_destroy(u); return rc; }
  return utts_finish(ctx, u, out);
}
extern "C" int khg_utts_graph_bytes(const khg_utts* u, int64_t* bytes) {
  if (!u || !bytes) return khg_set_error(KHG_E_ARG, "khg_utts_graph_bytes: bad arguments");
  *bytes = u->graph_bytes;
  return KHG_OK;
}

extern "C" int khg_utts_set_pdf_list(khg_utts* u, int32_t n, const int32_t* pdfs) {
  if (!u || n <= 0 || !pdfs) return khg_set_error(KHG_E_ARG, "khg_utts_set_pdf_list: bad arguments");
  if (u->has_graphs) return khg_set_error(KHG_E_ARG, "khg_utts_set_pdf_list: set has graphs; its pdf lists come from them");
  u->pdfs.clear();
  u->pdf_first.clear(); u->pdf_last.clear();
  for (int i = 0; i < u->n_utt; ++i) { u->pdf_off[i + 1] = u->pdf_off[i] + n; u->pdfs.insert(u->pdfs.end(), pdfs, pdfs + n); }
  plan_ll(u);
  DEVFREE(u->pdf_off_d); DEVFREE(u->pdfs_d); DEVFREE(u->ll_off_d); DEVFREE(u->ll_d); DEVFREE(u->chunks_d); DEVFREE(u->wchunks_d);
  DEVFREE(u->tile_off_d); DEVFREE(u->tiles_d); u->tiles_pto.clear(); u->tiles_reach = -1;
  DEVFREE(u->p_ents_d); DEVFREE(u->p_slices_d); u->p_reach = -1;
  DEVFREE(u->sunits_d); u->sunits_pto.clear(); u->sunits_reach = -1;
  u->pdfs_checked_P = -1;
  u->ll_valid = false;
  return KHG_OK;
}

extern "C" int khg_utts_features_changed(khg_utts* u) {
  if (!u) return khg_set_error(KHG_E_ARG, "khg_utts_features_changed: bad arguments");
  u->xmax.clear();
  u->xs_ks = 0; u->xs_ex.clear();
  u->xh_ks = 0; u->xh_ex.clear();
  u->ll_valid = false;
  return KHG_OK;
}

int utts_foreign_ctx(const khg_ctx* ctx, const khg_utts* u, const char* where) {
  if (u && u->small && u->ctx != ctx)
    return khg_set_error(KHG_E_ARG, std::string(where) + ": a small utterance set (<= 16 utterances: scratch in its context's arena) must be used with the context that created it");
  return KHG_OK;
}

extern "C" int khg_utts_destroy(khg_utts* u) {
  if (!u) return KHG_OK;
  if (u->small && u->ctx && khg_ctx_alive(u->ctx)) {
    khg_ctx* c = u->ctx;
    for (int i = 0; i < khg_ctx::NSIDE; ++i)
      if (c->side_dirty[i]) { (void)hipStreamSynchronize(c->sides[i]); c->side_dirty[i] = false; }
    (void)hipStreamSynchronize(c->stream);
    c->pageable_pending = false;
  }
  if (u->out_blk_d) {
    u->ali_d = nullptr; u->words_d = nullptr; u->num_words_d = nullptr; u->status_d = nullptr; u->like_d = nullptr;
    DEVFREE(u->out_blk_d);
  }
  if (u->own_feats) DEVFREE(u->feats_d);
  if (u->graph) {
    u->state_off_d = nullptr; u->start_d = nullptr; u->in_off_d = nullptr; u->out_off_d = nullptr; u->in_src_d = nullptr; u->in_col_d = nullptr;
    u->in_tid_d = nullptr; u->in_olabel_d = nullptr; u->out_inidx_d = nullptr; u->in_w_d = nullptr; u->final_d = nullptr;
    khg_graph_release(u->graph); u->graph = nullptr;
  }
  DEVFREE(u->gidx_d);
  DEVFREE(u->frame_off_d); DEVFREE(u->state_off_d); DEVFREE(u->pdf_off_d); DEVFREE(u->ll_off_d);
  DEVFREE(u->pdfs_d); DEVFREE(u->wchunks_d); DEVFREE(u->start_d); DEVFREE(u->in_off_d); DEVFREE(u->out_off_d);
  DEVFREE(u->in_src_d); DEVFREE(u->in_col_d); DEVFREE(u->in_tid_d); DEVFREE(u->in_olabel_d); DEVFREE(u->out_inidx_d);
  DEVFREE(u->in_w_d); DEVFREE(u->final_d); DEVFREE(u->chunks_d); DEVFREE(u->ll_d); DEVFREE(u->tile_off_d); DEVFREE(u->tiles_d);
  DEVFREE(u->xpl_d); DEVFREE(u->utt_xtile_off_d); DEVFREE(u->p_ents_d); DEVFREE(u->p_slices_d);
  DEVFREE(u->utt_x32_off_d); DEVFREE(u->bchunks_d); DEVFREE(u->x32_utt_d); DEVFREE(u->xh_d); DEVFREE(u->xh_ex_d);
  DEVFREE(u->xs_d); DEVFREE(u->xs_ex_d); DEVFREE(u->schunks_d); DEVFREE(u->sunits_d);
  DEVFREE(u->bp_d); DEVFREE(u->bp_off_d); DEVFREE(u->path_off_d); DEVFREE(u->words_off_d);
  DEVFREE(u->ali2_d); DEVFREE(u->unc_d); DEVFREE(u->sub_off_d);
  if (u->unc_cnt_h) { (void)hipHostFree(u->unc_cnt_h); u->unc_cnt_h = nullptr; }
  DEVFREE(u->layer_best_d); DEVFREE(u->layer_cnt_d); DEVFREE(u->path_d); DEVFREE(u->k2_gscratch_d); DEVFREE(u->k2_order_d);
  DEVFREE(u->ali_d); DEVFREE(u->words_d); DEVFREE(u->num_words_d); DEVFREE(u->status_d); DEVFREE(u->like_d);
  DEVFREE(u->pdf_count_d); DEVFREE(u->pdf_cursor_d); DEVFREE(u->frame_ids_d); DEVFREE(u->pdf_start_d); DEVFREE(u->tid_count_d);
  DEVFREE(u->sort_keys_d); DEVFREE(u->sort_keys_out_d); DEVFREE(u->sort_vals_d); DEVFREE(u->sort_tmp_d); DEVFREE(u->cs_hist_d); DEVFREE(u->cs_tot_d);
  DEVFREE(u->k3_part_d); DEVFREE(u->k3_llpart_d); DEVFREE(u->k3_items_d); DEVFREE(u->k3_item_off_d);
  DEVFREE(u->pe_row_d); DEVFREE(u->pe_tid_d); DEVFREE(u->pe_ids_d); DEVFREE(u->pe_w_d); DEVFREE(u->pe_keys_d); DEVFREE(u->pe_keys_out_d);
  DEVFREE(u->pe_vals_d); DEVFREE(u->pe_tmp_d); DEVFREE(u->pe_start_d);
  DEVFREE(u->rc_keys_d); DEVFREE(u->rc_keys_out_d); DEVFREE(u->rc_vals_d); DEVFREE(u->rc_vals_out_d); DEVFREE(u->rc_flag_d); DEVFREE(u->rc_inc_d);
  DEVFREE(u->rc_row_d); DEVFREE(u->rc_cell_d); DEVFREE(u->rc_tmp_d); DEVFREE(u->rc_cell_start_d); DEVFREE(u->rc_item_off_d); DEVFREE(u->rc_stats_d);
  k1_free_band(u);
  if (u->ev_dp) (void)hipEventDestroy(u->ev_dp);
  if (u->ev_ali) (void)hipEventDestroy(u->ev_ali);
  delete u;
  return KHG_OK;
}
extern "C" int khg_utts_num_pdfs(const khg_utts* u, int64_t* pdf_off) {
  if (!u || !pdf_off) return khg_set_error(KHG_E_ARG, "bad arguments");
  std::copy(u->pdf_off.begin(), u->pdf_off.end(), pdf_off);
  return KHG_OK;
}
extern "C" int khg_utts_pdfs(const khg_utts* u, int32_t* pdfs) {
  if (!u || !pdfs) return khg_set_error(KHG_E_ARG, "bad arguments");
  std::copy(u->pdfs.begin(), u->pdfs.end(), pdfs);
  return KHG_OK;
}

__global__ void k2_merge_fallback(const int32_t* __restrict__ unc, const int64_t* __restrict__ frame_off, const int32_t* __restrict__ ali2,
                                  int32_t* __restrict__ ali, int n_utt) {
  for (int u = blockIdx.x; u < n_utt; u += gridDim.x) {
    if (!unc[u]) continue;
    const int64_t f0 = frame_off[u], f1 = frame_off[u + 1];
    for (int64_t f = f0 + threadIdx.x; f < f1; f += blockDim.x) ali[f] = ali2[f];
  }
}
int wait_ali(khg_ctx* ctx, khg_utts* u) {
  if (u->ali_pending) { HIPCHK(hipStreamWaitEvent(ctx->stream, u->ev_ali, 0)); u->ali_pending = false; }
  if (u->ali_split) {
    u->ali_split = false;
    KHG_LAUNCH(ctx, k2_merge_fallback, dim3((unsigned)std::min(u->n_utt, 16384)), dim3(64), 0, ctx->stream, u->unc_d, u->frame_off_d, u->ali2_d, u->ali_d, u->n_utt);
    HIPCHK(hipGetLastError());
  }
  return KHG_OK;
}
```

Before: 440.3 million.

## Prepack scaled f16 feature split planes per utterance set for wave16 acc-stats

Result: faster. 447.5 million, median of 6 (+1.7%).

```diff
diff --git a/include/khg_hip.h b/include/khg_hip.h
--- a/include/khg_hip.h
+++ b/include/khg_hip.h
@@ -59,7 +59,8 @@
 #define KHG_OPT_K1_PGRID 20
 #define KHG_OPT_K1_PROF 21
 #define KHG_OPT_K2_LADDER 22
-#define KHG_OPT_COUNT 23
+#define KHG_OPT_K3_PLANES 23
+#define KHG_OPT_COUNT 24
 #define KHG_INFO_SCRATCH_BYTES 100
 #define KHG_INFO_SCRATCH_BLOCKS 101
 int khg_ctx_set_option(khg_ctx *ctx, int option, int value);
@@ -97,6 +98,7 @@
 int khg_utts_pdfs(const khg_utts *u, int32_t *pdfs_h );
 int khg_utts_k2_plan(khg_ctx *ctx, const khg_utts *u, int32_t out[8]);
 int khg_utts_k2_ladder(khg_ctx *ctx, const khg_utts *u, int32_t *out);
+int khg_utts_k3_planes(const khg_utts *u, int64_t *bytes, int64_t *packs, int32_t *used);
 int khg_utts_pdf_first(const khg_utts *u, int32_t *first_h );
 
 int khg_loglikes(khg_ctx *ctx, const khg_model *m, khg_utts *u);
diff --git a/kaldi_hmm_gmm_amd/_lib.py b/kaldi_hmm_gmm_amd/_lib.py
--- a/kaldi_hmm_gmm_amd/_lib.py
+++ b/kaldi_hmm_gmm_amd/_lib.py
@@ -160,6 +160,7 @@
     "khg_utts_pdfs": (C.c_int, [vp, c_i32p]),
     "khg_utts_k2_plan": (C.c_int, [vp, vp, c_i32p]),
     "khg_utts_k2_ladder": (C.c_int, [vp, vp, c_i32p]),
+    "khg_utts_k3_planes": (C.c_int, [vp, c_i64p, c_i64p, c_i32p]),
     "khg_utts_pdf_first": (C.c_int, [vp, c_i32p]),
     "khg_loglikes": (C.c_int, [vp, vp, vp]),
     "khg_loglikes_reachable": (C.c_int, [vp, vp, vp]),
diff --git a/kaldi_hmm_gmm_amd/csrc/khg_ctx_model.hip b/kaldi_hmm_gmm_amd/csrc/khg_ctx_model.hip
--- a/kaldi_hmm_gmm_amd/csrc/khg_ctx_model.hip
+++ b/kaldi_hmm_gmm_amd/csrc/khg_ctx_model.hip
@@ -157,7 +157,7 @@
   return KHG_OK;
 }
 static const struct { int lo, hi; } k_opt_range[KHG_OPT_COUNT] = {
-  {KHG_K1_AUTO, KHG_K1_F16X2S}, {0, 4}, {0, 6}, {0, 1 << 20}, {-1, 1}, {0, 255}, {0, 1}, {0, 4}, {0, 3}, {0, 1}, {0, 2}, {0, 2}, {0, 2}, {0, 64}, {0, 1}, {0, 1}, {0, 1}, {0, 1 << 20}, {0, 1}, {0, 2}, {0, 1 << 16}, {0, 1}, {0, 1}};
+  {KHG_K1_AUTO, KHG_K1_F16X2S}, {0, 4}, {0, 6}, {0, 1 << 20}, {-1, 1}, {0, 255}, {0, 1}, {0, 4}, {0, 3}, {0, 1}, {0, 2}, {0, 2}, {0, 2}, {0, 64}, {0, 1}, {0, 1}, {0, 1}, {0, 1 << 20}, {0, 1}, {0, 2}, {0, 1 << 16}, {0, 1}, {0, 1}, {0, 2}};
 extern "C" int khg_option_check(int opt, int value) {
   if (opt < 0 || opt >= KHG_OPT_COUNT) return khg_set_error(KHG_E_ARG, "khg_option_check: no such option");
   if (value < k_opt_range[opt].lo || value > k_opt_range[opt].hi || (opt == KHG_OPT_K1_FORM && value == 1))
@@ -193,7 +193,8 @@
   {"KHG_K2_SPLIT", KHG_OPT_K2_SPLIT, "on=0,off=1"}, {"KHG_K2S_HUB", KHG_OPT_K2S_HUB, ""},
   {"KHG_LAT_OPS_LDS", KHG_OPT_LAT_OPS_LDS, "on=0,off=1"},
   {"KHG_K1_LAUNCH", KHG_OPT_K1_LAUNCH, "auto=0,chunk=1,persistent=2"}, {"KHG_K1_PGRID", KHG_OPT_K1_PGRID, ""},
-  {"KHG_K1_PROF", KHG_OPT_K1_PROF, ""}, {"KHG_K2_LADDER", KHG_OPT_K2_LADDER, "on=0,off=1"}};
+  {"KHG_K1_PROF", KHG_OPT_K1_PROF, ""}, {"KHG_K2_LADDER", KHG_OPT_K2_LADDER, "on=0,off=1"},
+  {"KHG_K3_PLANES", KHG_OPT_K3_PLANES, "auto=0,off=1,on=2"}};
 extern "C" int khg_option_from_env(const char* name, const char* text, int* option, int* value) {
   if (!name || !text || !*text || !option || !value) return khg_set_error(KHG_E_ARG, "khg_option_from_env: bad arguments");
   for (const auto& t : k_env_tab) {
diff --git a/kaldi_hmm_gmm_amd/csrc/khg_internal.hpp b/kaldi_hmm_gmm_amd/csrc/khg_internal.hpp
--- a/kaldi_hmm_gmm_amd/csrc/khg_internal.hpp
+++ b/kaldi_hmm_gmm_amd/csrc/khg_internal.hpp
@@ -265,6 +265,7 @@
   void* k3_items_d = nullptr; int32_t* k3_item_off_d = nullptr; size_t k3_items_n = 0, k3_item_off_n = 0;
   int64_t* pdf_start_d = nullptr; unsigned long long* tid_count_d = nullptr;
   int32_t k3_P = 0, k3_tids = 0;
+  void* k3x_d = nullptr; int64_t k3x_bytes = 0, k3x_packs = 0; std::vector<int32_t> k3x_key; bool k3x_used = false;
   int32_t *pe_row_d = nullptr, *pe_tid_d = nullptr, *pe_ids_d = nullptr; float* pe_w_d = nullptr; size_t pe_cap = 0;
   uint32_t *pe_keys_d = nullptr, *pe_keys_out_d = nullptr, *pe_vals_d = nullptr; void* pe_tmp_d = nullptr; size_t pe_tmp_bytes = 0;
   int64_t* pe_start_d = nullptr; int32_t pe_P = 0;
diff --git a/kaldi_hmm_gmm_amd/csrc/khg_k3.hip b/kaldi_hmm_gmm_amd/csrc/khg_k3.hip
--- a/kaldi_hmm_gmm_amd/csrc/khg_k3.hip
+++ b/kaldi_hmm_gmm_amd/csrc/khg_k3.hip
@@ -160,6 +160,7 @@
   int target = 0;
   int64_t extra_blocks = 0, max_items = 0, max_slots = 0;
   bool may_f16a = false, may_f16b = false;
+  bool may_planes = false;
   size_t lds[3] = {0, 0, 0};
   bool too_wide = false;
 };
@@ -185,7 +186,8 @@
     const size_t fold = sizeof(double) * (nb * 16 * 80 + nb * 16);
     r.lds[0] = std::max<size_t>(sizeof(float) * (nb * 20 * 64 + 4 * 4 * 16 * 20), fold);
     r.lds[1] = std::max<size_t>(sizeof(float) * (4 * 4 * 16 * 20) + 2 * (size_t)(4 * 2 * 16 * K3_XH_ROW), fold);
-    r.lds[2] = std::max<size_t>(2 * (size_t)4 * (2 * (2 * 16 * K3_XH_ROW) + 2 * 2 * 40 * 36) + nb * 3 * 2 * 64 * 16, fold);
+    r.lds[2] = std::max<size_t>(2 * (size_t)4 * (2 * (2 * 16 * K3_X16_ROW)) + nb * 3 * 2 * 64 * 16, fold);
+    r.may_planes = r.may_f16b && ctx->opt[KHG_OPT_K3_PLANES] != 1;
     const int64_t avg_tiles = (avg + 15) / 16;
     r.ny = (int)std::max<int64_t>(1, std::min<int64_t>(std::min<int64_t>(32, (avg_tiles + 15) / 16), (4096 + P - 1) / P));
     if (ny_opt > 0) r.ny = ny_opt;
@@ -240,11 +242,12 @@
 }
 
 typedef void (*K3Kernel)(K3Args);
-enum K3Variant { K3V_WAVE, K3V_WAVE16, K3V_FINALIZE, K3V_MFMA, K3V_BLOCK16, K3V_VALU };
+enum K3Variant { K3V_WAVE, K3V_WAVE16, K3V_WAVE16P, K3V_FINALIZE, K3V_MFMA, K3V_BLOCK16, K3V_VALU };
 struct K3Inst { int variant, KQ, NB, nwv; bool post, f16a; K3Kernel fn; };
 #define K3_WAVE_ROWS(NB)                                                                                                           \
   {K3V_WAVE, 10, NB, 4, false, false, k3_accumulate_wave<NB>}, {K3V_WAVE, 10, NB, 4, false, true, k3_accumulate_wave<NB, true>}, \
-  {K3V_WAVE16, 10, NB, 4, false, true, k3_accumulate_wave16<NB>}, {K3V_FINALIZE, 10, NB, 4, false, false, k3_wave_finalize<NB>}
+  {K3V_WAVE16, 10, NB, 4, false, true, k3_accumulate_wave16<NB>}, {K3V_WAVE16P, 10, NB, 4, false, true, k3_accumulate_wave16<NB, true>}, \
+  {K3V_FINALIZE, 10, NB, 4, false, false, k3_wave_finalize<NB>}
 #define K3_MFMA_ROWS(KQ, NBW) {K3V_MFMA, KQ, NBW, 4, false, false, k3_accumulate_mfma<KQ, NBW>}, {K3V_MFMA, KQ, NBW, 4, true, false, k3_accumulate_mfma<KQ, NBW, true>}
 #define K3_VALU_ROWS(KQ) {K3V_VALU, KQ, 0, 4, false, false, k3_accumulate<KQ>}, {K3V_VALU, KQ, 0, 4, true, false, k3_accumulate<KQ, true>}
 static const K3Inst k3_insts[] = {
@@ -289,6 +292,7 @@
   a.occ = acc->occ(); a.mean_acc = acc->mean(); a.var_acc = acc->var(); a.trans_acc = acc->trans(); a.scalars = acc->scalars();
   a.weight = weight; a.err_flag = ctx->err_flag_d; a.part = nullptr; a.ll_part = nullptr; a.pdf0 = 0; a.npdf = m->P; a.items = nullptr; a.item_off = nullptr;
   a.pa_ex = nullptr; a.pa_S = 0; a.pa_scale = 1.0f; a.pa_inv = 1.0f; a.pa_c1 = 1.44269504088896340736f; a.pb_gscale = 1.0f; a.pb_SG = 0;
+  a.xrec = nullptr; a.xrec_zero = 0;
   return a;
 }
 static bool k3_weight_ordinary(float weight) { return std::isfinite(weight) && std::fabs(weight) > 1.0e-30f && std::fabs(weight) < 1.0e30f; }
@@ -298,6 +302,39 @@
     a.pa_scale = std::ldexp(1.0f, m->k3_S); a.pa_inv = std::ldexp(1.0f, -m->k3_S); a.pa_c1 = std::ldexp(1.44269504088896340736f, -m->k3_S);
   }
   if (f16b) { a.pb_SG = 13 - std::ilogb(std::fabs(a.weight)); a.pb_gscale = std::ldexp(1.0f, a.pb_SG); }
+}
+
+static int k3_planes(khg_ctx* ctx, const khg_model* m, khg_utts* u, bool* use) {
+  *use = false;
+  const int mode = ctx->opt[KHG_OPT_K3_PLANES];
+  if (mode == 1 || u->N >= (int64_t)INT_MAX - 1 || (mode == 0 && u->small)) return KHG_OK;
+  const size_t bytes = sizeof(_Float16) * K3_XREC * ((size_t)u->N + 1);
+  if (u->k3x_d && u->k3x_key == m->k3_ex) { *use = true; return KHG_OK; }
+  if (!u->k3x_d) {
+    if (mode == 0) {
+      size_t free_b = 0, total_b = 0;
+      if (hipMemGetInfo(&free_b, &total_b) != hipSuccess) { (void)hipGetLastError(); return KHG_OK; }
+      if (bytes > free_b / 2) return KHG_OK;
+    }
+    void* p = nullptr;
+    if (hipMalloc(&p, bytes) != hipSuccess) { (void)hipGetLastError(); return KHG_OK; }
+    u->k3x_d = p; u->k3x_bytes = (int64_t)bytes;
+  }
+  {
+    KernelTimer kt(ctx, "k3_pack_x");
+    const int64_t nthr = ((int64_t)u->N + 1) * 5;
+    KHG_LAUNCH(ctx, k3_pack_x, dim3((unsigned)std::min<int64_t>(65536, (nthr + 255) / 256)), dim3(256), 0, ctx->stream, u->feats_d, u->N, (int)u->D, m->k3_ex_d,
+               reinterpret_cast<_Float16*>(u->k3x_d));
+  }
+  HIPCHK(hipGetLastError());
+  u->k3x_key = m->k3_ex; ++u->k3x_packs;
+  *use = true;
+  return KHG_OK;
+}
+extern "C" int khg_utts_k3_planes(const khg_utts* u, int64_t* bytes, int64_t* packs, int32_t* used) {
+  if (!u || !bytes || !packs || !used) return khg_set_error(KHG_E_ARG, "khg_utts_k3_planes: bad arguments");
+  *bytes = u->k3x_d ? u->k3x_bytes : 0; *packs = u->k3x_packs; *used = u->k3x_used ? 1 : 0;
+  return KHG_OK;
 }
 
 template int u_alloc<uint32_t>(khg_utts*, uint32_t**, size_t);
@@ -395,7 +432,12 @@
   if (r.may_f16a && (wave || wt)) { int rs = k3_phase_a_scales(ctx, const_cast<khg_model*>(m), u, &f16a); if (rs) return rs; }
   const bool f16b = f16a && r.may_f16b && wt;
   k3_set_scales(a, m, f16a, f16b);
-  const int variant = wave ? (f16b ? K3V_WAVE16 : K3V_WAVE) : r.form == K3F_VALU ? K3V_VALU : f16b ? K3V_BLOCK16 : K3V_MFMA;
+  int variant = wave ? (f16b ? K3V_WAVE16 : K3V_WAVE) : r.form == K3F_VALU ? K3V_VALU : f16b ? K3V_BLOCK16 : K3V_MFMA;
+  if (variant == K3V_WAVE16 && r.may_planes) {
+    bool planes = false;
+    { int rp = k3_planes(ctx, m, u, &planes); if (rp) return rp; }
+    if (planes) { variant = K3V_WAVE16P; a.xrec = reinterpret_cast<const _Float16*>(u->k3x_d); a.xrec_zero = (int32_t)u->N; u->k3x_used = true; }
+  }
   const int nwv = variant == K3V_BLOCK16 ? r.nwv16 : 4;
   const K3Kernel fn = k3_kernel(variant, m->KQ, variant == K3V_BLOCK16 ? r.NB16 : r.NB, nwv, post, f16a);
   const K3Kernel fin = wave ? k3_kernel(K3V_FINALIZE, m->KQ, r.NB, 4, false, false) : nullptr;
@@ -433,6 +475,7 @@
     HIPCHK(hipMemsetAsync(u->tid_count_d, 0, sizeof(unsigned long long) * ((size_t)tm->num_tids + 1), ctx->stream));
   }
   K3Args a = k3_args(ctx, m, tm, u, acc, weight, post, Neff);
+  if (!post) u->k3x_used = false;
   nparts = std::max(1, std::min(nparts, m->P));
   if (comm && nparts > 1) { rc = ctx_comm_stream(ctx); if (rc) return rc; }
   if (Neff > 0) {
diff --git a/kaldi_hmm_gmm_amd/csrc/khg_k3_accstats.hip.inc b/kaldi_hmm_gmm_amd/csrc/khg_k3_accstats.hip.inc
--- a/kaldi_hmm_gmm_amd/csrc/khg_k3_accstats.hip.inc
+++ b/kaldi_hmm_gmm_amd/csrc/khg_k3_accstats.hip.inc
@@ -29,6 +29,8 @@
   float pa_scale, pa_inv, pa_c1;
   float pb_gscale;
   int32_t pb_SG;
+  const _Float16* xrec;
+  int32_t xrec_zero;
   const int32_t* e_row;
   const float* e_w;
 };
@@ -883,6 +885,10 @@
 }
 
 typedef _Float16 k3_f16x8 __attribute__((ext_vector_type(8)));
+typedef _Float16 k3_f16x4 __attribute__((ext_vector_type(4)));
+typedef __fp16 k3_fp16x4 __attribute__((__vector_size__(4 * sizeof(__fp16))));
+typedef __attribute__((address_space(3))) k3_fp16x4 k3_lds_h4;
+__device__ __forceinline__ k3_f16x4 k3_read_tr16(k3_lds_h4* p) { return __builtin_bit_cast(k3_f16x4, __builtin_amdgcn_ds_read_tr16_b64_v4f16(p)); }
 #define K3_XH_ROW 104
 
 template <int NB>
@@ -1139,12 +1145,37 @@
   }
 }
 
-template <int NB>
+#define K3_X16_ROW 112
+#define K3_XREC 160
+__device__ __forceinline__ void k3_split_cell(float v, float sx, float sx2, _Float16& h1, _Float16& h2, _Float16& g1, _Float16& g2) {
+  const float s1 = v * sx, s2 = (v * v) * sx2;
+  h1 = (_Float16)s1; g1 = (_Float16)s2;
+  h2 = (_Float16)(s1 - (float)h1); g2 = (_Float16)(s2 - (float)g1);
+}
+__global__ __launch_bounds__(256) void k3_pack_x(const float* __restrict__ feats, int64_t N, int D, const int32_t* __restrict__ ex, _Float16* __restrict__ rec) {
+  const int64_t n = (N + 1) * 5;
+  for (int64_t i = (int64_t)blockIdx.x * 256 + threadIdx.x; i < n; i += (int64_t)gridDim.x * 256) {
+    const int64_t f = i / 5;
+    const int d0 = 8 * (int)(i - 5 * f);
+    k3_f16x8 h1, h2, g1, g2;
+#pragma unroll
+    for (int e = 0; e < 8; ++e) {
+      const int d = d0 + e, dc = min(d, D - 1);
+      const float v = (f < N && d < D) ? feats[f * D + dc] : 0.0f;
+      _Float16 a1, a2, b1, b2;
+      k3_split_cell(v, ldexpf(1.0f, ex[2 * dc]), ldexpf(1.0f, ex[2 * dc + 1]), a1, a2, b1, b2);
+      h1[e] = a1; h2[e] = a2; g1[e] = b1; g2[e] = b2;
+    }
+    _Float16* r = rec + f * K3_XREC + d0;
+    *reinterpret_cast<k3_f16x8*>(r) = h1; *reinterpret_cast<k3_f16x8*>(r + 40) = g1;
+    *reinterpret_cast<k3_f16x8*>(r + 80) = h2; *reinterpret_cast<k3_f16x8*>(r + 120) = g2;
+  }
+}
+template <int NB, bool PLANES = false>
 __global__ __launch_bounds__(256, 1) void k3_accumulate_wave16(K3Args a) {
   extern __shared__ __attribute__((aligned(16))) float k3s[];
-  constexpr int KQ = 10, XP = 4 * KQ, NDB = KQ / 2, TF = 16;
-  constexpr int XHH = 2 * TF * K3_XH_ROW;
-  constexpr int XTR = 36, XTH = 2 * 2 * XP * XTR;
+  constexpr int KQ = 10, XP = 4 * KQ, NDB = KQ / 2, TF = 16, ROW = K3_X16_ROW;
+  constexpr int XHH = 2 * TF * ROW;
   K3Item it;
   if (!k3_take_item(a, it)) return;
   const int pdf = it.pdf;
@@ -1156,12 +1187,11 @@
   const int tid = threadIdx.x, lane = tid & 63;
   const int wave = __builtin_amdgcn_readfirstlane(tid >> 6);
   const int j16 = lane & 15, q = lane >> 4;
-  _Float16* xh = reinterpret_cast<_Float16*>(k3s) + wave * (2 * XHH + XTH);
-  _Float16* xt = xh + 2 * XHH;
+  _Float16* xh = reinterpret_cast<_Float16*>(k3s) + wave * (2 * XHH);
   float gcv[NB];
 #pragma unroll
   for (int k = 0; k < NB; ++k) gcv[k] = ((16 * k + j16 < G) ? a.gconsts[g0 + 16 * k + j16] : -INFINITY) * a.pa_scale;
-  char* wl16 = reinterpret_cast<char*>(reinterpret_cast<_Float16*>(k3s) + 4 * (2 * XHH + XTH));
+  char* wl16 = reinterpret_cast<char*>(reinterpret_cast<_Float16*>(k3s) + 4 * (2 * XHH));
   for (int e0 = tid; e0 < NB * 3 * 64; e0 += 256) {
     const int l = e0 & 63, st = (e0 >> 6) % 3, k = e0 / (3 * 64), jl = l & 15, ql = l >> 4;
     k3_f16x8 p1, p2;
@@ -1180,9 +1210,9 @@
     *reinterpret_cast<k3_f16x8*>(wl16 + (((k * 3 + st) * 2 + 1) * 64 + l) * 16) = p2;
   }
   {
-    static_assert((2 * XHH + XTH) % 8 == 0, "the wave's planes are whole 16-byte words");
+    static_assert((2 * XHH) % 8 == 0 && ROW % 8 == 0, "the wave's planes and their rows are whole 16-byte words");
     const k3_f16x8 z = {0, 0, 0, 0, 0, 0, 0, 0};
-    for (int i = lane; i < (2 * XHH + XTH) / 8; i += 64) reinterpret_cast<k3_f16x8*>(xh)[i] = z;
+    for (int i = lane; i < (2 * XHH) / 8; i += 64) reinterpret_cast<k3_f16x8*>(xh)[i] = z;
   }
   __syncthreads();
 
@@ -1197,19 +1227,24 @@
   double tot_ll = 0.0;
   unsigned bad = 0;
   const int ntile = (nfr + TF - 1) / TF, npair = (ntile + 1) / 2;
-  constexpr int NM = 2 * TF * XP / (4 * 64);
+  constexpr int NM = 2 * TF * XP / (4 * 64), NR = 2 * TF * (K3_XREC / 8) / 64;
   static_assert(NM * 4 * 64 == 2 * TF * XP, "micro-tiles cover the pair exactly");
+  static_assert(NR * 64 == 2 * TF * (K3_XREC / 8) && (NR & 1) == 0, "record chunks cover the pair exactly, a tile per half of them");
   const int pstride = 4 * it.ny;
   float pre[NM][4];
   float sx[NM][2], sx2[NM][2];
+  k1b_u32x4 rec[NR];
   const bool even_d = (D & 1) == 0;
-#pragma unroll
-  for (int j = 0; j < NM; ++j)
-#pragma unroll
-    for (int c = 0; c < 2; ++c) {
-      const int d = min(2 * ((lane + 64 * j) % 20) + c, D - 1);
-      sx[j][c] = ldexpf(1.0f, a.pa_ex[2 * d]); sx2[j][c] = ldexpf(1.0f, a.pa_ex[2 * d + 1]);
-    }
+  if constexpr (!PLANES) {
+#pragma unroll
+    for (int j = 0; j < NM; ++j)
+#pragma unroll
+      for (int c = 0; c < 2; ++c) {
+        const int d = min(2 * ((lane + 64 * j) % 20) + c, D - 1);
+        sx[j][c] = ldexpf(1.0f, a.pa_ex[2 * d]); sx2[j][c] = ldexpf(1.0f, a.pa_ex[2 * d + 1]);
+      }
+  }
+  const int fid_none = PLANES ? a.xrec_zero : 0;
   const float gs = a.pb_gscale;
   const int rot = (int)(((unsigned)pdf * 2654435761u) % (unsigned)npair);
   auto pair_of = [&](int p) { const int x = p + rot; return x >= npair ? x - npair : x; };
@@ -1217,9 +1252,19 @@
   auto fid_of = [&](int pl, int tau) -> int {
     const int n = cf_of(pl, tau);
     const int t = pl < npair ? 2 * pair_of(pl) + tau : 0;
-    return lane < n ? a.frame_ids[beg + t * TF + lane] : 0;
+    return lane < n ? a.frame_ids[beg + t * TF + lane] : fid_none;
   };
   auto request = [&](int fid0, int fid1) {
+    if constexpr (PLANES) {
+      const k1b_u32x4* src = reinterpret_cast<const k1b_u32x4*>(a.xrec);
+#pragma unroll
+      for (int j = 0; j < NR; ++j) {
+        const int i = lane + 64 * j, fs = i / 20, kk = i - 20 * fs;
+        const int fid = __shfl(j < NR / 2 ? fid0 : fid1, fs & (TF - 1));
+        rec[j] = src[(int64_t)fid * (K3_XREC / 8) + kk];
+      }
+      return;
+    }
     int fa[NM], fb[NM];
 #pragma unroll
     for (int j = 0; j < NM; ++j) {
@@ -1251,35 +1296,33 @@
   if (p < npair) { request(fid_of(p, 0), fid_of(p, 1)); fidn0 = fid_of(p + pstride, 0); fidn1 = fid_of(p + pstride, 1); }
   for (; p < npair; p += pstride) {
     const int cf[2] = {cf_of(p, 0), cf_of(p, 1)};
-#pragma unroll
-    for (int j = 0; j < NM; ++j) {
-      typedef _Float16 h2v __attribute__((ext_vector_type(2)));
-      const int i = lane + 64 * j, tau = i / 160, r = i % 160, f0 = 2 * (r / 20), d0 = 2 * (r % 20);
-      const int cft = tau ? cf[1] : cf[0];
-      _Float16 h1[4], h2[4], g1[4], g2[4];
-#pragma unroll
-      for (int e = 0; e < 4; ++e) {
-        const int f = f0 + (e >> 1), d = d0 + (e & 1);
-        const float v = (f < cft && d < D) ? pre[j][e] : 0.0f;
-        const float s1 = v * sx[j][e & 1], s2 = (v * v) * sx2[j][e & 1];
-        h1[e] = (_Float16)s1; g1[e] = (_Float16)s2;
-        h2[e] = (_Float16)(s1 - (float)h1[e]); g2[e] = (_Float16)(s2 - (float)g1[e]);
-      }
-#pragma unroll
-      for (int ff = 0; ff < 2; ++ff) {
-        _Float16* r1 = xh + tau * XHH + (f0 + ff) * K3_XH_ROW + d0;
-        *reinterpret_cast<h2v*>(r1) = h2v{h1[2 * ff], h1[2 * ff + 1]};
-        *reinterpret_cast<h2v*>(r1 + TF * K3_XH_ROW) = h2v{h2[2 * ff], h2[2 * ff + 1]};
-        *reinterpret_cast<h2v*>(r1 + XP) = h2v{g1[2 * ff], g1[2 * ff + 1]};
-        *reinterpret_cast<h2v*>(r1 + TF * K3_XH_ROW + XP) = h2v{g2[2 * ff], g2[2 * ff + 1]};
-      }
-#pragma unroll
-      for (int dd = 0; dd < 2; ++dd) {
-        _Float16* c1 = xt + (d0 + dd) * XTR + tau * TF + f0;
-        *reinterpret_cast<h2v*>(c1) = h2v{h1[dd], h1[2 + dd]};
-        *reinterpret_cast<h2v*>(c1 + 2 * XP * XTR) = h2v{h2[dd], h2[2 + dd]};
-        *reinterpret_cast<h2v*>(c1 + XP * XTR) = h2v{g1[dd], g1[2 + dd]};
-        *reinterpret_cast<h2v*>(c1 + 2 * XP * XTR + XP * XTR) = h2v{g2[dd], g2[2 + dd]};
+    if constexpr (PLANES) {
+#pragma unroll
+      for (int j = 0; j < NR; ++j) {
+        const int i = lane + 64 * j, fs = i / 20, kk = i - 20 * fs, pc = kk >= K3_XREC / 16, tau = j >= NR / 2;
+        *reinterpret_cast<k1b_u32x4*>(xh + tau * XHH + (pc * TF + (fs & (TF - 1))) * ROW + 8 * (kk - pc * (K3_XREC / 16))) = rec[j];
+      }
+    } else {
+#pragma unroll
+      for (int j = 0; j < NM; ++j) {
+        typedef _Float16 h2v __attribute__((ext_vector_type(2)));
+        const int i = lane + 64 * j, tau = i / 160, r = i % 160, f0 = 2 * (r / 20), d0 = 2 * (r % 20);
+        const int cft = tau ? cf[1] : cf[0];
+        _Float16 h1[4], h2[4], g1[4], g2[4];
+#pragma unroll
+        for (int e = 0; e < 4; ++e) {
+          const int f = f0 + (e >> 1), d = d0 + (e & 1);
+          const float v = (f < cft && d < D) ? pre[j][e] : 0.0f;
+          k3_split_cell(v, sx[j][e & 1], sx2[j][e & 1], h1[e], h2[e], g1[e], g2[e]);
+        }
+#pragma unroll
+        for (int ff = 0; ff < 2; ++ff) {
+          _Float16* r1 = xh + tau * XHH + (f0 + ff) * ROW + d0;
+          *reinterpret_cast<h2v*>(r1) = h2v{h1[2 * ff], h1[2 * ff + 1]};
+          *reinterpret_cast<h2v*>(r1 + TF * ROW) = h2v{h2[2 * ff], h2[2 * ff + 1]};
+          *reinterpret_cast<h2v*>(r1 + XP) = h2v{g1[2 * ff], g1[2 * ff + 1]};
+          *reinterpret_cast<h2v*>(r1 + TF * ROW + XP) = h2v{g2[2 * ff], g2[2 * ff + 1]};
+        }
       }
     }
     if (p + pstride < npair) { request(fidn0, fidn1); fidn0 = fid_of(p + 2 * pstride, 0); fidn1 = fid_of(p + 2 * pstride, 1); }
@@ -1294,8 +1337,8 @@
       k3_f16x8 x1[2], x2[2];
 #pragma unroll
       for (int tau = 0; tau < 2; ++tau) {
-        x1[tau] = *reinterpret_cast<const k3_f16x8*>(xh + tau * XHH + j16 * K3_XH_ROW + 32 * st + 8 * q);
-        x2[tau] = *reinterpret_cast<const k3_f16x8*>(xh + tau * XHH + (TF + j16) * K3_XH_ROW + 32 * st + 8 * q);
+        x1[tau] = *reinterpret_cast<const k3_f16x8*>(xh + tau * XHH + j16 * ROW + 32 * st + 8 * q);
+        x2[tau] = *reinterpret_cast<const k3_f16x8*>(xh + tau * XHH + (TF + j16) * ROW + 32 * st + 8 * q);
       }
 #pragma unroll
       for (int k = 0; k < NB; ++k) {
@@ -1350,12 +1393,13 @@
     }
 #pragma unroll
     for (int db = 0; db < NDB; ++db) {
-      const _Float16* cb = xt + (16 * db + j16) * XTR + 4 * q;
+      k3_lds_h4* cb = (k3_lds_h4*)(xh + (4 * q + (j16 >> 2)) * ROW + 16 * db + 4 * (j16 & 3));
       k3_f16x8 xb1, xb2;
       {
-        typedef _Float16 h4 __attribute__((ext_vector_type(4)));
-        const h4 a0 = *reinterpret_cast<const h4*>(cb), a1 = *reinterpret_cast<const h4*>(cb + TF);
-        const h4 b0 = *reinterpret_cast<const h4*>(cb + 2 * XP * XTR), b1 = *reinterpret_cast<const h4*>(cb + 2 * XP * XTR + TF);
+        typedef k3_f16x4 h4;
+        constexpr int T1 = XHH / 4, P2 = TF * ROW / 4;
+        const h4 a0 = k3_read_tr16(cb), a1 = k3_read_tr16(cb + T1);
+        const h4 b0 = k3_read_tr16(cb + P2), b1 = k3_read_tr16(cb + T1 + P2);
 #pragma unroll
         for (int e = 0; e < 4; ++e) { xb1[e] = a0[e]; xb1[4 + e] = a1[e]; xb2[e] = b0[e]; xb2[4 + e] = b1[e]; }
       }
diff --git a/kaldi_hmm_gmm_amd/csrc/khg_pybind.cpp b/kaldi_hmm_gmm_amd/csrc/khg_pybind.cpp
--- a/kaldi_hmm_gmm_amd/csrc/khg_pybind.cpp
+++ b/kaldi_hmm_gmm_amd/csrc/khg_pybind.cpp
@@ -65,7 +65,7 @@
   static int opt_id(const py::object& o) {
     if (py::isinstance<py::int_>(o)) return o.cast<int>();
     static const char* names[KHG_OPT_COUNT] = {"k1_form", "k1_order", "k1_nf", "k1p_ts", "k1_interleave", "k1_dbg", "k2_inorder", "k2_ks", "k2_serial",
-                                               "k2_prof", "k3_bucket", "k3_form", "k3_phase_b", "k3_ny", "debug", "k3_phase_a", "k2_split", "k2s_hub", "lat_ops_lds", "k1_launch", "k1_pgrid", "k1_prof", "k2_ladder"};
+                                               "k2_prof", "k3_bucket", "k3_form", "k3_phase_b", "k3_ny", "debug", "k3_phase_a", "k2_split", "k2s_hub", "lat_ops_lds", "k1_launch", "k1_pgrid", "k1_prof", "k2_ladder", "k3_planes"};
     const std::string n = o.cast<std::string>();
     for (int i = 0; i < KHG_OPT_COUNT; ++i) if (n == names[i]) return i;
     if (n == "scratch_bytes") return KHG_INFO_SCRATCH_BYTES;
@@ -641,6 +641,13 @@
     d["nthr"] = o[5]; d["lds_bytes"] = o[6]; d["faithful_form"] = o[7];
     return d;
   }
+  py::dict k3_planes() {
+    int64_t bytes = 0, packs = 0; int32_t used = 0;
+    Check(khg_utts_k3_planes(h, &bytes, &packs, &used));
+    py::dict d;
+    d["bytes"] = bytes; d["packs"] = packs; d["used"] = used != 0;
+    return d;
+  }
   bool k2_ladder(py::object ctx_o) {
     int32_t o = 0;
     Check(khg_utts_k2_ladder(ctx_o.cast<KContext*>()->h, h, &o));
@@ -1071,7 +1078,7 @@
       .def_property_readonly("h", [](KUtts& x) { return reinterpret_cast<uintptr_t>(x.h); })
       .def_readonly("ctx", &KUtts::ctx_obj).def_readonly("frame_off", &KUtts::frame_off).def_readonly("n_utt", &KUtts::n_utt)
       .def_readonly("dim", &KUtts::dim)
-      .def("set_pdf_list", &KUtts::set_pdf_list).def("features_changed", &KUtts::features_changed).def("pdf_lists", &KUtts::pdf_lists).def("k2_plan", &KUtts::k2_plan, py::arg("ctx")).def("k2_ladder", &KUtts::k2_ladder, py::arg("ctx")).def("pdf_first_frames", &KUtts::pdf_first_frames)
+      .def("set_pdf_list", &KUtts::set_pdf_list).def("features_changed", &KUtts::features_changed).def("pdf_lists", &KUtts::pdf_lists).def("k2_plan", &KUtts::k2_plan, py::arg("ctx")).def("k2_ladder", &KUtts::k2_ladder, py::arg("ctx")).def("k3_planes", &KUtts::k3_planes).def("pdf_first_frames", &KUtts::pdf_first_frames)
       .def("pdf_last_frames", &KUtts::pdf_last_frames)
       .def("loglikes", &KUtts::loglikes, py::arg("model"), py::arg("reachable_only") = false, py::arg("band") = false)
       .def("loglikes_layout", &KUtts::loglikes_layout).def("download_loglikes", &KUtts::download_loglikes)
diff --git a/kaldi_hmm_gmm_amd/csrc/khg_utts.hip b/kaldi_hmm_gmm_amd/csrc/khg_utts.hip
--- a/kaldi_hmm_gmm_amd/csrc/khg_utts.hip
+++ b/kaldi_hmm_gmm_amd/csrc/khg_utts.hip
@@ -392,6 +392,7 @@
   u->xmax.clear();
   u->xs_ks = 0; u->xs_ex.clear();
   u->xh_ks = 0; u->xh_ex.clear();
+  u->k3x_key.clear();
   u->ll_valid = false;
   return KHG_OK;
 }
@@ -436,7 +437,7 @@
   DEVFREE(u->ali_d); DEVFREE(u->words_d); DEVFREE(u->num_words_d); DEVFREE(u->status_d); DEVFREE(u->like_d);
   DEVFREE(u->pdf_count_d); DEVFREE(u->pdf_cursor_d); DEVFREE(u->frame_ids_d); DEVFREE(u->pdf_start_d); DEVFREE(u->tid_count_d);
   DEVFREE(u->sort_keys_d); DEVFREE(u->sort_keys_out_d); DEVFREE(u->sort_vals_d); DEVFREE(u->sort_tmp_d); DEVFREE(u->cs_hist_d); DEVFREE(u->cs_tot_d);
-  DEVFREE(u->k3_part_d); DEVFREE(u->k3_llpart_d); DEVFREE(u->k3_items_d); DEVFREE(u->k3_item_off_d);
+  DEVFREE(u->k3x_d); DEVFREE(u->k3_part_d); DEVFREE(u->k3_llpart_d); DEVFREE(u->k3_items_d); DEVFREE(u->k3_item_off_d);
   DEVFREE(u->pe_row_d); DEVFREE(u->pe_tid_d); DEVFREE(u->pe_ids_d); DEVFREE(u->pe_w_d); DEVFREE(u->pe_keys_d); DEVFREE(u->pe_keys_out_d);
   DEVFREE(u->pe_vals_d); DEVFREE(u->pe_tmp_d); DEVFREE(u->pe_start_d);
   DEVFREE(u->rc_keys_d); DEVFREE(u->rc_keys_out_d); DEVFREE(u->rc_vals_d); DEVFREE(u->rc_vals_out_d); DEVFREE(u->rc_flag_d); DEVFREE(u->rc_inc_d);
```
